# Justin900429/autonomous_driving_with_diffusion_model

Hardware: AMD Instinct MI355X
Metric: denoising-steps/sec (higher is better)
Workload: dtype f32

## Files before the change

### autonomous_driving_with_diffusion_model_amd/_lib.py

```python
from __future__ import annotations

import ctypes as C
import os
from typing import Optional, Sequence

import torch

_HERE = os.path.dirname(os.path.abspath(__file__))
LIB_PATH = os.environ.get("ADX_LIB") or os.path.join(_HERE, "libadx.so")

c_f32p = C.POINTER(C.c_float)
i32, i64, f32, vp = C.c_int32, C.c_int64, C.c_float, C.c_void_p


class TConvDesc(C.Structure):
    _fields_ = [("kind", i32), ("taps", i32), ("stride", i32), ("pad", i32), ("c0", i32), ("c1", i32),
                ("cout", i32), ("lin", i32), ("lout", i32), ("groups", i32), ("eps", f32), ("w_layout", i32),
                ("w_flip", i32), ("exact", i32), ("lin_valid", i32), ("lout_valid", i32)]


class TConvIO(C.Structure):
    _fields_ = [("x0", vp), ("x0_sb", i64), ("x0_sc", i64), ("x0_sl", i64),
                ("x1", vp), ("x1_sb", i64), ("x1_sc", i64), ("x1_sl", i64),
                ("packed_w", vp), ("bias", vp), ("gamma", vp), ("beta", vp),
                ("tbias", vp), ("tbias_stride", i64),
                ("res", vp), ("res_sb", i64), ("res_sc", i64), ("res_sl", i64),
                ("y", vp), ("y_sb", i64), ("y_sc", i64), ("y_sl", i64), ("batch", i32), ("pre", vp), ("stats", vp),
                ("scratch", vp), ("scratch_floats", i64), ("tickets", vp)]


class EmbedWeights(C.Structure):
    _fields_ = [(n, vp) for n in ("freqs", "w1", "b1", "w3", "b3", "cw0", "cb0", "cw2", "cb2")]


class UnetConfig(C.Structure):
    _fields_ = [("horizon", i32), ("transition_dim", i32), ("dim", i32), ("n_mults", i32),
                ("dim_mults", i32 * 8), ("guidance", i32)]


class UnetIO(C.Structure):
    _fields_ = [("x", vp), ("img_feature", vp), ("feat_rows", i32), ("t", vp), ("t_rows", i32), ("cond", vp),
                ("rows", i32), ("out", vp), ("time_embed", vp), ("x_rows", i32), ("time_bias", vp)]


UNET_ATTENTION = 1


class Conv2dDesc(C.Structure):
    _fields_ = [("cin", i32), ("cout", i32), ("k", i32), ("stride", i32), ("pad", i32)]


class StepCoef(C.Structure):
    _fields_ = [("prediction_type", i32), ("clip", i32), ("clip_range", f32), ("sqrt_alpha_t", f32),
                ("sqrt_beta_t", f32), ("c_x0", f32), ("c_dir", f32), ("c_x", f32), ("c_noise", f32),
                ("add_noise", i32), ("use_clipped_model_output", i32), ("inpaint", i32), ("c_const", f32),
                ("c_known", f32), ("c_known_noise", f32), ("known_noise", i32), ("cfg_combine", i32),
                ("free_scale", f32), ("zero_first", i32)]


_SIGS = {
    "adx_version": (i32, []),
    "adx_last_error": (C.c_char_p, []),
    "adx_source_hash": (C.c_char_p, []),
    "adx_tconv_packed_bytes": (C.c_size_t, [C.POINTER(TConvDesc)]),
    "adx_tconv_pack": (i32, [C.POINTER(TConvDesc), vp, vp, vp]),
    "adx_tconv_forward": (i32, [C.POINTER(TConvDesc), C.POINTER(TConvIO), vp]),
    "adx_embed_forward": (i32, [C.POINTER(EmbedWeights), i32, vp, i32, vp, vp, i32, i32, vp, vp, vp]),
    "adx_unet_create": (i32, [C.POINTER(UnetConfig), C.POINTER(vp)]),
    "adx_unet_create_ex": (i32, [C.POINTER(UnetConfig), i32, C.POINTER(vp)]),
    "adx_unet_destroy": (None, [vp]),
    "adx_unet_num_params": (i32, [vp]),
    "adx_unet_packed_bytes": (C.c_size_t, [vp]),
    "adx_unet_pack": (i32, [vp, C.POINTER(vp), i32, vp, vp, vp]),
    "adx_unet_workspace_bytes": (C.c_size_t, [vp, i32]),
    "adx_unet_forward": (i32, [vp, vp, vp, C.POINTER(UnetIO), vp]),
    "adx_unet_time_bias_width": (i32, [vp]),
    "adx_unet_time_conditioning_workspace_bytes": (C.c_size_t, [vp, i32]),
    "adx_unet_time_conditioning": (i32, [vp, vp, vp, C.POINTER(UnetIO), vp, vp, vp]),
    "adx_unet_tape_create": (i32, [C.POINTER(vp)]),
    "adx_unet_tape_destroy": (None, [vp]),
    "adx_unet_train_workspace_bytes": (C.c_size_t, [vp, i32]),
    "adx_unet_forward_train": (i32, [vp, vp, vp, C.c_size_t, C.POINTER(UnetIO), vp, vp]),
    "adx_unet_backward": (i32, [vp, vp, vp, C.c_size_t, vp, vp, vp, vp, C.POINTER(vp), C.POINTER(vp), i32, vp]),
    "adx_gn_mish_backward": (i32, [vp, i64, i64, i64, vp, vp, vp, vp, vp, vp, vp, vp, vp, i64, i32, i32, i32, i32, vp]),
    "adx_tconv_wgrad": (i32, [C.POINTER(TConvDesc), C.POINTER(TConvIO), vp, vp, vp]),
    "adx_bias_grad": (i32, [vp, vp, i32, i32, i32, vp]),
    "adx_chan_layernorm_forward": (i32, [vp, i64, i64, i64, vp, vp, vp, vp, vp, i32, i32, i32, i32, vp]),
    "adx_chan_layernorm_backward": (i32, [vp, vp, i64, i64, i64, vp, vp, vp, vp, vp, vp, i32, i32, i32, i32, i32, vp]),
    "adx_linattn_forward": (i32, [vp, vp, i32, i32, i32, vp]),
    "adx_linattn_backward": (i32, [vp, vp, vp, i32, i32, i32, vp]),
    "adx_resnet_create": (i32, [i32, C.POINTER(vp)]),
    "adx_resnet_destroy": (None, [vp]),
    "adx_resnet_num_tensors": (i32, [vp]),
    "adx_resnet_packed_bytes": (C.c_size_t, [vp]),
    "adx_resnet_pack": (i32, [vp, C.POINTER(vp), i32, vp, vp]),
    "adx_resnet_workspace_bytes": (C.c_size_t, [vp, i32, i32, i32]),
    "adx_resnet_forward": (i32, [vp, vp, vp, vp, i32, i32, i32, vp, vp]),
    "adx_resnet_forward_u8": (i32, [vp, vp, vp, vp, C.POINTER(C.c_float), C.POINTER(C.c_float), i32, i32, i32, vp, vp]),
    "adx_resnet_tape_create": (i32, [C.POINTER(vp)]),
    "adx_resnet_tape_destroy": (None, [vp]),
    "adx_resnet_train_workspace_bytes": (C.c_size_t, [vp, i32, i32, i32]),
    "adx_resnet_forward_train": (i32, [vp, C.POINTER(vp), i32, vp, vp, C.c_size_t, vp, i32, i32, i32, vp, vp, i32, vp]),
    "adx_resnet_backward": (i32, [vp, C.POINTER(vp), C.POINTER(vp), i32, vp, C.c_size_t, vp, vp, vp]),
    "adx_resnet_backward_groups": (i32, [vp]),
    "adx_resnet_tensor_group": (i32, [vp, i32]),
    "adx_resnet_backward_events": (i32, [vp, C.POINTER(vp), C.POINTER(vp), i32, vp, C.c_size_t, vp, vp, C.POINTER(vp), i32, vp]),
    "adx_resnet_tape_describe": (i32, [vp, vp, i32, C.POINTER(i32), C.POINTER(i32), C.POINTER(i64)]),
    "adx_conv2d_packed_bytes": (C.c_size_t, [C.POINTER(Conv2dDesc)]),
    "adx_conv2d_pack": (i32, [C.POINTER(Conv2dDesc), vp, vp, vp]),
    "adx_conv2d_forward": (i32, [C.POINTER(Conv2dDesc), vp, vp, vp, vp, vp, vp, i32, i32, i32, i32, vp]),
    "adx_conv2d_cells_supported": (i32, [C.POINTER(Conv2dDesc), i32, i32, i32]),
    "adx_conv2d_forward_cells": (i32, [C.POINTER(Conv2dDesc), vp, vp, vp, vp, vp, vp, i32, i32, i32, i32, i32, vp]),
    "adx_conv2d_wgrad_scratch_bytes": (C.c_size_t, []),
    "adx_conv2d_wgrad": (i32, [C.POINTER(Conv2dDesc), vp, vp, vp, i32, i32, i32, vp, vp]),
    "adx_conv2d_wgrad_ex": (i32, [C.POINTER(Conv2dDesc), vp, vp, vp, i32, i32, i32, vp, i32, vp]),
    "adx_conv2d_wgrad_cells": (i32, [C.POINTER(Conv2dDesc), vp, vp, vp, vp, i32, i32, i32, vp, vp]),
    "adx_trajpred_create": (i32, [i32, C.POINTER(vp)]),
    "adx_trajpred_destroy": (None, [vp]),
    "adx_trajpred_num_params": (i32, [vp]),
    "adx_trajpred_packed_bytes": (C.c_size_t, [vp]),
    "adx_trajpred_scratch_bytes": (C.c_size_t, [vp, i32, i32]),
    "adx_trajpred_set_scratch": (i32, [vp, vp, C.c_size_t]),
    "adx_trajpred_pack": (i32, [vp, C.POINTER(vp), i32, vp, vp, vp]),
    "adx_trajpred_forward": (i32, [vp, vp, vp, i64, i64, vp, vp, i32, i32, vp]),
    "adx_trajpred_backward": (i32, [vp, vp, vp, i64, i64, vp, vp, vp, i32, i32, vp]),
    "adx_trajpred_backward_params": (i32, [vp, vp, vp, i64, i64, vp, vp, vp, vp, vp, i32, i32, C.c_float, C.c_uint64, vp]),
    "adx_trajpred_forward_train": (i32, [vp, vp, vp, i64, i64, vp, vp, i32, i32, C.c_float, C.c_uint64, vp]),
    "adx_trajpred_param_offsets": (i32, [vp, C.POINTER(i64), i32]),
    "adx_guided_output": (i32, [vp, vp, vp, vp, vp, f32, f32, vp, vp, i32, i32, vp]),
    "adx_optim_chunk": (i32, []),
    "adx_adamw_ema_step": (i32, [vp, vp, vp, i32, f32, f32, f32, f32, f32, i32, f32, i32, i32, vp]),
    "adx_adamw_ema_step_scaled": (i32, [vp, vp, vp, i32, f32, f32, f32, f32, f32, i32, f32, i32, i32, f32, vp]),
    "adx_image_normalize": (i32, [vp, vp, i32, i32, i32, C.POINTER(C.c_float), C.POINTER(C.c_float), vp]),
    "adx_probe_mfma_fp16": (i32, [vp, vp, i32, i32, C.POINTER(C.c_double), vp]),
    "adx_probe_mfma_fp16_16x16x32": (i32, [vp, vp, i32, i32, C.POINTER(C.c_double), vp]),
    "adx_image_augment": (i32, [vp, vp, i32, i32, i32, vp, vp, vp, vp, i32, vp]),
    "adx_ddim_step": (i32, [C.POINTER(StepCoef), vp, vp, vp, vp, vp, vp, vp, i32, i32, i32, vp]),
    "adx_ddpm_step": (i32, [C.POINTER(StepCoef), vp, vp, vp, vp, vp, vp, vp, i32, i32, i32, vp]),
    "adx_add_noise": (i32, [vp, vp, vp, vp, vp, i32, vp, i32, i32, i32, i32, vp]),
}

EXPORTED_SYMBOLS = tuple(_SIGS)

_lib: Optional[C.CDLL] = None


class AdxError(RuntimeError):
    pass


def lib() -> C.CDLL:
    global _lib
    if _lib is None:
        if not os.path.exists(LIB_PATH):
            raise AdxError(
                f"{LIB_PATH} not found: the HIP extension is not built. Run `python -c 'import __graft_entry__ as g; "
                f"g.build()'` (or autonomous_driving_with_diffusion_model_amd/csrc/build.sh). There is no CPU fallback.")
        handle = C.CDLL(LIB_PATH)
        for name, (res, args) in _SIGS.items():
            fn = getattr(handle, name)
            fn.restype = res
            fn.argtypes = args
        _lib = handle
    return _lib


class NativeTape:

    def __init__(self, create, destroy, what: str):
        import weakref
        h = vp()
        check(create(C.byref(h)), what)
        self.handle = h
        self._fin = weakref.finalize(self, destroy, h)

    @property
    def alive(self) -> bool:
        return self._fin.alive

    def release(self) -> None:
        self._fin()


def check(rc: int, what: str = "") -> None:
    if rc != 0:
        msg = lib().adx_last_error().decode(errors="replace")
        if rc == -1:
            raise ValueError(f"{what}: {msg}" if what else msg)
        raise AdxError(f"{what} failed (status {rc}): {msg}")


def ptr(t: Optional[torch.Tensor]) -> Optional[int]:
    return None if t is None else t.data_ptr()


def stream_ptr(device=None) -> int:
    return torch.cuda.current_stream(device).cuda_stream


def require_gpu_f32(t: torch.Tensor, name: str, dtype=torch.float32) -> torch.Tensor:
    if not t.is_cuda:
        raise AdxError(f"{name} lives on {t.device}; the adx kernels only run on an MI355X (no CPU path)")
    if t.dtype != dtype:
        raise TypeError(f"{name} must be {dtype}, got {t.dtype}")
    return t if t.is_contiguous() else t.contiguous()


def write_stamp(t: torch.Tensor) -> int:
    return 0 if t.is_inference() else t._version


def grad_buffer(p: torch.Tensor) -> torch.Tensor:
    v = getattr(p, "_adx_grad_view", None)
    if (v is not None and p.grad is None and not getattr(p, "_adx_grad_leased", False)
            and v.device == p.device and v.shape == p.shape):
        p._adx_grad_leased = True
        return v.detach()
    return torch.empty_like(p)


def ptr_array(tensors: Sequence[torch.Tensor]):
    arr = (vp * len(tensors))()
    for i, t in enumerate(tensors):
        arr[i] = t.data_ptr()
    return arr
```

### autonomous_driving_with_diffusion_model_amd/csrc/conv2d.hip

```cpp
#include <stdlib.h>

#include <vector>

#include "adx_common.h"
#include "conv2d_internal.h"

namespace adx {

constexpr int kCoutT = 64;
constexpr size_t kMaxLds = 96 * 1024;
constexpr int g_conv_cc = 16;
constexpr int g_conv_rows = 2;

template <int STRIDE, int K, int ROWS, int CCH = 16>
__global__ void __launch_bounds__(256) conv2d_kernel(const Conv2dArgs a) {
  constexpr int TH = 4 * ROWS;
  constexpr int CC = (K == 7) ? 4 : CCH;
  constexpr int PH = (TH - 1) * STRIDE + K;
  constexpr int PW = (kTileW - 1) * STRIDE + K;
  constexpr int PLANE = PH * PW;
  constexpr int NP = CC * PLANE;
  constexpr int PITEMS = (NP + 255) / 256;
  constexpr int NTAPS = K * K;
  constexpr int NW4 = NTAPS * CC * (kCoutT / 4);
// ... 177 lines not shown
  const int oy = blockIdx.y * 4 + wave;
  const int pl = blockIdx.x;
  if (oy >= OH) return;
  const float* src = x + (size_t)pl * H * W;
  float* dst = y + ((size_t)pl * OH + oy) * OW;
  if ((W & 1) == 0 && ((size_t)x & 7) == 0) {
    typedef float f32x2 __attribute__((ext_vector_type(2)));
    for (int ox0 = lane; ox0 - lane < OW; ox0 += 256) {
      float m[4] = {-INFINITY, -INFINITY, -INFINITY, -INFINITY};
#pragma unroll
      for (int dy = 0; dy < 3; ++dy) {
        const int iy = oy * 2 - 1 + dy;
        if (iy < 0 || iy >= H) continue;
        const float* row = src + (size_t)iy * W;
        f32x2 v[4];
        float left[4];
#pragma unroll
        for (int q = 0; q < 4; ++q) {
          const int ox = ox0 + 64 * q;
          const bool in = 2 * ox + 1 < W;
          v[q] = in ? *reinterpret_cast<const f32x2*>(row + 2 * ox) : f32x2{-INFINITY, -INFINITY};
          left[q] = (lane == 0 && ox > 0 && 2 * ox - 1 < W) ? row[2 * ox - 1] : -INFINITY;
        }
#pragma unroll
        for (int q = 0; q < 4; ++q) {
          const float nb = __shfl_up(v[q][1], 1, 64);
          const float l = lane == 0 ? left[q] : nb;
          m[q] = pool_max(pool_max(pool_max(m[q], l), v[q][0]), v[q][1]);
        }
      }
#pragma unroll
      for (int q = 0; q < 4; ++q)
        if (ox0 + 64 * q < OW) dst[ox0 + 64 * q] = m[q];
    }
    return;
  }
  for (int ox0 = lane; ox0 < OW; ox0 += 256) {
    float m[4] = {-INFINITY, -INFINITY, -INFINITY, -INFINITY};
#pragma unroll
    for (int dy = 0; dy < 3; ++dy) {
      const int iy = oy * 2 - 1 + dy;
      const bool rok = iy >= 0 && iy < H;
      const float* row = src + (size_t)(rok ? iy : 0) * W;
#pragma unroll
      for (int q = 0; q < 4; ++q)
#pragma unroll
        for (int dx = 0; dx < 3; ++dx) {
          const int ix = (ox0 + 64 * q) * 2 - 1 + dx;
          const bool ok = rok && ix >= 0 && ix < W;
          const float v = ok ? row[ix] : -INFINITY;
          m[q] = pool_max(m[q], v);
        }
    }
#pragma unroll
    for (int q = 0; q < 4; ++q)
      if (ox0 + 64 * q < OW) dst[ox0 + 64 * q] = m[q];
  }
}

__global__ void __launch_bounds__(1024) avgpool_fc_kernel(const float* __restrict__ x, const float* __restrict__ fw,
                                                           const float* __restrict__ fb, float* __restrict__ out,
                                                           int C, int HW, int out_dim) {
  __shared__ float pooled[512];
  const int n = blockIdx.x, tid = threadIdx.x, lane = tid & 63, wave = tid >> 6;
  const float* src = x + (size_t)n * C * HW;
  const float inv = 1.0f / (float)HW;
  for (int c0 = wave * 4; c0 < C; c0 += 64) {
    float s[4] = {0.f, 0.f, 0.f, 0.f};
    for (int i = lane; i < HW; i += 64) {
#pragma unroll
      for (int q = 0; q < 4; ++q) s[q] += (c0 + q < C) ? src[(size_t)(c0 + q) * HW + i] : 0.f;
    }
#pragma unroll
    for (int q = 0; q < 4; ++q) {
      const float t = wave_sum(s[q]);
      if (lane == 0 && c0 + q < C) pooled[c0 + q] = t * inv;
    }
  }
  __syncthreads();
  for (int j = wave; j < out_dim; j += 16) {
    float s = 0.f;
    for (int c = lane; c < C; c += 64) s += fw[(size_t)j * C + c] * pooled[c];
    s = wave_sum(s);
    if (lane == 0) out[(size_t)n * out_dim + j] = s + fb[j];
  }
}

int maxpool_launch(const float* x, float* y, int planes, int H, int W, int OH, int OW, hipStream_t s) {
  maxpool_kernel<<<dim3(planes, ceil_div(OH, 4)), dim3(256), 0, s>>>(x, y, planes, H, W, OH, OW);
  ADX_LAUNCH_CHECK();
  return ADX_OK;
}

__global__ void __launch_bounds__(1024) avgpool_fc_cells_kernel(const uint4* __restrict__ x, const float* __restrict__ fw,
                                                                 const float* __restrict__ fb, float* __restrict__ out,
                                                                 int C, int HW, int out_dim) {
  typedef _Float16 h8 __attribute__((ext_vector_type(8)));
  __shared__ float pooled[512];
  const int n = blockIdx.x, tid = threadIdx.x, lane = tid & 63, wave = tid >> 6;
  const uint4* src = x + (size_t)n * (C / 8) * 2 * HW;
  const float inv = 1.0f / (float)HW;
  for (int g = wave; g < C / 8; g += 16) {
    float s[8] = {0.f, 0.f, 0.f, 0.f, 0.f, 0.f, 0.f, 0.f};
    for (int i = lane; i < HW; i += 64) {
      const h8 hi = __builtin_bit_cast(h8, src[(size_t)(2 * g) * HW + i]);
      const h8 lo = __builtin_bit_cast(h8, src[(size_t)(2 * g + 1) * HW + i]);
#pragma unroll
      for (int q = 0; q < 8; ++q) s[q] += (float)hi[q] + (float)lo[q] * (1.f / 2048.f);
    }
#pragma unroll
    for (int q = 0; q < 8; ++q) {
      const float t = wave_sum(s[q]);
      if (lane == 0) pooled[8 * g + q] = t * inv;
    }
  }
  __syncthreads();
  for (int j = wave; j < out_dim; j += 16) {
    float s = 0.f;
    for (int c = lane; c < C; c += 64) s += fw[(size_t)j * C + c] * pooled[c];
    s = wave_sum(s);
    if (lane == 0) out[(size_t)n * out_dim + j] = s + fb[j];
  }
}

int avgpool_fc_launch(const float* x, const float* fw, const float* fb, float* out, int batch, int C, int HW, int out_dim,
                      hipStream_t s, int x_cells) {
  ADX_REQUIRE(C <= 512, "avgpool_fc: at most 512 channels");
  if (x_cells) {
    ADX_REQUIRE(C % 8 == 0, "avgpool_fc: the cell layout holds channels in groups of eight");
    avgpool_fc_cells_kernel<<<dim3(batch), dim3(1024), 0, s>>>(reinterpret_cast<const uint4*>(x), fw, fb, out, C, HW, out_dim);
    ADX_LAUNCH_CHECK();
    return ADX_OK;
  }
  avgpool_fc_kernel<<<dim3(batch), dim3(1024), 0, s>>>(x, fw, fb, out, C, HW, out_dim);
  ADX_LAUNCH_CHECK();
  return ADX_OK;
}

}

namespace adx {

static size_t align64f(size_t v) { return (v + 63) / 64 * 64; }

static int conv_out(int h, int k, int s, int p) { return conv_out_dim(h, k, s, p); }

static int conv2d_launch(const ConvSpec& L, const float* base, const float* x, const float* res, float* y, int N, int H,
                         int W, int relu, hipStream_t s, int fmt = 0) {
  return conv2d_launch_raw(L, x, base + L.o_w, base + L.o_scale, base + L.o_shift, res, y, N, H, W, relu, s, nullptr, 0, nullptr, 0,
                           nullptr, fmt);
}

static thread_local float* t_split_scratch = nullptr;
static thread_local size_t t_split_floats = 0;
void conv2d_set_split_scratch(float* p, size_t floats) { t_split_scratch = p; t_split_floats = p != nullptr ? floats : 0; }

int conv2d_launch_raw(const ConvSpec& L, const float* x, const float* w, const float* scale, const float* shift,
                      const float* res, float* y, int N, int H, int W, int relu, hipStream_t s, const uint32_t* x_amax,
                      int x_amax_n, float* stats_part, size_t stats_floats, int* stats_p, int fmt, const BnBwdStats* bst) {
  if (stats_p != nullptr) *stats_p = 0;
  Conv2dArgs a;
  a.x = x; a.w = w; a.scale = scale; a.shift = shift; a.res = res; a.y = y; a.x_amax = x_amax; a.x_amax_n = x_amax_n;
  a.w_ds = nullptr; a.scale_ds = nullptr; a.shift_ds = nullptr; a.y_ds = nullptr;
  a.N = N; a.Cin = L.cin; a.H = H; a.W = W; a.Cout = L.cout;
  a.OH = conv_out(H, L.k, L.stride, L.pad); a.OW = conv_out(W, L.k, L.stride, L.pad);
  a.KH = L.k; a.KW = L.k; a.stride = L.stride; a.pad = L.pad; a.relu = relu;
  a.cin_pad = L.cin_pad; a.cc = L.cc;
  a.x_u8 = nullptr;
  a.d2s_cin = 0; a.d2s_h = 0; a.d2s_w = 0; a.stem_seg_tiles = 0; a.stem_nseg = 1;
  a.ksplit = 1; a.cper = 0; a.part = t_split_scratch; a.part_stride = t_split_floats;
  a.stats_part = nullptr; a.stats_p = 0;
  a.bs_raw = a.bs_out = a.bs_mean = a.bs_rstd = a.bs_gamma = a.bs_beta = nullptr; a.bs_mask = 0; a.bs_bits = nullptr; a.res_bits = nullptr;
  if (bst != nullptr) {
    ADX_REQUIRE(bst->raw && bst->mean && bst->rstd && bst->gamma && bst->beta && (bst->mask == 2 || (bst->mask == 1 && (bst->out || bst->bits))),
                "conv2d: incomplete BatchNorm-backward statistics request");
    ADX_REQUIRE(scale == nullptr && relu == 0, "conv2d: BatchNorm-backward statistics belong to data-gradient launches");
    a.bs_raw = bst->raw; a.bs_out = bst->out; a.bs_mean = bst->mean; a.bs_rstd = bst->rstd; a.bs_gamma = bst->gamma;
    a.bs_beta = bst->beta; a.bs_mask = bst->mask; a.bs_bits = bst->mask == 1 ? bst->bits : nullptr;
    a.res_bits = bst->res_bits;
    ADX_REQUIRE(a.res_bits == nullptr || (res != nullptr && stats_part != nullptr &&
                                          conv2d_hs3x3_dgrad_stats(L, N, H, W, (fmt & kFmtXCells) != 0, stats_floats)),
                "conv2d: a masked residual belongs to a data-gradient launch with the statistics epilogue");
  }
  a.x_cells = (fmt & kFmtXCells) != 0; a.y_cells = (fmt & kFmtYCells) != 0; a.res_cells = (fmt & kFmtResCells) != 0 && res != nullptr;
  const bool train_cells = fmt == kFmtXCells && stats_part != nullptr && stats_p != nullptr && bst == nullptr && x_amax == nullptr &&
                           conv2d_hs3x3_train_cells(L, N, H, W, stats_floats);
  const bool dgrad_cells = fmt == (kFmtXCells | kFmtXScaled) && L.dgrad && x_amax != nullptr && x_amax_n < 0 &&
                           conv2d_hs3x3_dgrad_cells(L, N, H, W);
  if (dgrad_cells) fmt = kFmtXCells;
  ADX_REQUIRE(fmt == 0 || train_cells || dgrad_cells || (stats_part == nullptr && conv2d_hs3x3_plain(L, N, H, W)),
              "conv2d: the cell layout belongs to plain launches of the pipelined 3x3 kernel (%d -> %d, k%d s%d)", L.cin, L.cout, L.k, L.stride);
  if (conv2d_hs_eligible(L)) {
    if (stats_part != nullptr && stats_p != nullptr && conv2d_hs_stats_tiles(L, a) > 0 &&
        (size_t)conv2d_hs_stats_tiles(L, a) * (L.cout * 2 + L.cout / 64) <= stats_floats) {
      a.stats_part = stats_part;
      a.stats_p = conv2d_hs_stats_tiles(L, a);
      *stats_p = a.stats_p;
    }
    return conv2d_hs_launch(L, a, s);
  }
  const int rows = (L.stride == 1 && L.k == 3 && g_conv_rows == 2) ? 2 : 1;
  const int th = 4 * rows;
  a.tiles_x = ceil_div(a.OW, kTileW); a.tiles_y = ceil_div(a.OH, th); a.cout_tiles = L.cout / kCoutT;
  a.PH = (th - 1) * L.stride + L.k; a.PW = (kTileW - 1) * L.stride + L.k;
  a.PWp = a.PW;
  ADX_REQUIRE(L.cin % L.cc == 0 || L.cin < L.cc, "conv2d: cin %d must be < %d or a multiple of it", L.cin, L.cc);
  ADX_REQUIRE((size_t)L.cin * H * W < (1u << 31), "conv2d: image plane too large for 32-bit gather offsets");
  const int cch = (rows == 2 && g_conv_cc == 8) ? 8 : a.cc;
  const size_t np = (size_t)cch * a.PH * a.PW;
  const size_t lds = sizeof(float) * ((np + 255) / 256 * 256 + (size_t)L.k * L.k * cch * kCoutT + 2 * kCoutT);
  ADX_REQUIRE(lds <= kMaxLds, "conv2d: LDS %zu bytes too large", lds);
  const size_t grid = (size_t)a.cout_tiles * a.tiles_x * a.tiles_y * N;
  ADX_REQUIRE(grid < (1u << 31), "conv2d: grid too large");
  static std::atomic<uint64_t> attr_set{0};
  if (DeviceOnce once{attr_set}; once) {
    const void* fns[6] = {reinterpret_cast<const void*>(&conv2d_kernel<1, 3, 1>), reinterpret_cast<const void*>(&conv2d_kernel<2, 3, 1>),
                          reinterpret_cast<const void*>(&conv2d_kernel<2, 1, 1>), reinterpret_cast<const void*>(&conv2d_kernel<2, 7, 1>),
                          reinterpret_cast<const void*>(&conv2d_kernel<1, 1, 1>), reinterpret_cast<const void*>(&conv2d_kernel<1, 3, 2>)};
    ADX_CHECK_HIP(hipFuncSetAttribute(reinterpret_cast<const void*>(&conv2d_kernel<1, 3, 2, 8>),
                                      hipFuncAttributeMaxDynamicSharedMemorySize, (int)kMaxLds));
    for (const void* f : fns) ADX_CHECK_HIP(hipFuncSetAttribute(f, hipFuncAttributeMaxDynamicSharedMemorySize, (int)kMaxLds));
    once.commit();
  }
  const dim3 g((unsigned)grid), blk(256);
  if (L.stride == 1 && L.k == 3 && rows == 2 && cch == 8) conv2d_kernel<1, 3, 2, 8><<<g, blk, lds, s>>>(a);
  else if (L.stride == 1 && L.k == 3 && rows == 2) conv2d_kernel<1, 3, 2><<<g, blk, lds, s>>>(a);
  else if (L.stride == 1 && L.k == 3) conv2d_kernel<1, 3, 1><<<g, blk, lds, s>>>(a);
  else if (L.stride == 2 && L.k == 3) conv2d_kernel<2, 3, 1><<<g, blk, lds, s>>>(a);
  else if (L.stride == 2 && L.k == 1) conv2d_kernel<2, 1, 1><<<g, blk, lds, s>>>(a);
  else if (L.stride == 2 && L.k == 7) conv2d_kernel<2, 7, 1><<<g, blk, lds, s>>>(a);
  else if (L.stride == 1 && L.k == 1) conv2d_kernel<1, 1, 1><<<g, blk, lds, s>>>(a);
  else {
    set_error("conv2d: no kernel for k=%d stride=%d (ResNet-34 uses 3x3 s1, 3x3 s2, 1x1 s2, 7x7 s2)", L.k, L.stride);
    return ADX_ERR_INVALID;
  }
  ADX_LAUNCH_CHECK();
  return ADX_OK;
}

}

using namespace adx;

static int spec_from_desc(const adx_conv2d_desc* d, ConvSpec* L) {
  ADX_REQUIRE(d != nullptr, "conv2d: null descriptor");
  ADX_REQUIRE(d->cin >= 1 && d->cout >= 64 && d->cout % kCoutT == 0, "conv2d: cout %d must be a multiple of %d", d->cout,
              kCoutT);
  ADX_REQUIRE(d->k >= 1 && d->k <= 7 && (d->stride == 1 || d->stride == 2) && d->pad >= 0 && d->pad <= 3,
              "conv2d: unsupported k/stride/pad %d/%d/%d", d->k, d->stride, d->pad);
  memset(L, 0, sizeof(*L));
  L->cin = d->cin; L->cout = d->cout; L->k = d->k; L->stride = d->stride; L->pad = d->pad;
  L->cc = d->cin >= 16 ? 16 : 4;
  L->cin_pad = round_up(d->cin, L->cc);
  return ADX_OK;
}

extern "C" {

size_t adx_conv2d_packed_bytes(const adx_conv2d_desc* d) {
  ConvSpec L;
  if (spec_from_desc(d, &L) != ADX_OK) return 0;
  return sizeof(float) * (conv2d_hs_eligible(L) ? conv2d_packed_floats(L) : (size_t)L.k * L.k * L.cin_pad * L.cout);
}

int adx_conv2d_pack(const adx_conv2d_desc* d, const float* w, float* packed, adx_stream stream) {
  ConvSpec L;
  int rc = spec_from_desc(d, &L);
  if (rc != ADX_OK) return rc;
  ADX_REQUIRE(w && packed, "adx_conv2d_pack: null pointer");
  return conv2d_pack_spec(L, w, packed, 0, (hipStream_t)stream);
}

int adx_conv2d_forward(const adx_conv2d_desc* d, const float* x, const float* packed_w, const float* scale,
                       const float* shift, const float* res, float* y, int32_t n, int32_t h, int32_t w, int32_t relu,
                       adx_stream stream) {
  ConvSpec L;
  int rc = spec_from_desc(d, &L);
  if (rc != ADX_OK) return rc;
  ADX_REQUIRE(x && packed_w && y, "adx_conv2d_forward: null tensor");
  ADX_REQUIRE((scale == nullptr) == (shift == nullptr), "adx_conv2d_forward: scale and shift go together");
  ADX_REQUIRE(n >= 1 && h + 2 * d->pad >= d->k && w + 2 * d->pad >= d->k, "adx_conv2d_forward: input too small");
  return conv2d_launch_raw(L, x, packed_w, scale, shift, res, y, n, h, w, relu, (hipStream_t)stream);
}

int adx_conv2d_cells_supported(const adx_conv2d_desc* d, int32_t n, int32_t h, int32_t w) {
  ConvSpec L;
  if (d == nullptr || spec_from_desc(d, &L) != ADX_OK) return 0;
  return conv2d_hs3x3_plain(L, n, h, w) ? 1 : 0;
}

int adx_conv2d_forward_cells(const adx_conv2d_desc* d, const void* x, const float* packed_w, const float* scale,
                             const float* shift, const void* res, void* y, int32_t n, int32_t h, int32_t w, int32_t relu,
                             int32_t fmt, adx_stream stream) {
  ConvSpec L;
  int rc = spec_from_desc(d, &L);
  if (rc != ADX_OK) return rc;
  ADX_REQUIRE(x && packed_w && y, "adx_conv2d_forward_cells: null tensor");
  ADX_REQUIRE((scale == nullptr) == (shift == nullptr), "adx_conv2d_forward_cells: scale and shift go together");
  ADX_REQUIRE(fmt >= 0 && fmt <= 7 && (fmt & kFmtYCells), "adx_conv2d_forward_cells: fmt %d (the output is a cell tensor)", fmt);
  ADX_REQUIRE(conv2d_hs3x3_plain(L, n, h, w), "adx_conv2d_forward_cells: not a plain launch of the pipelined 3x3 kernel "
              "(adx_conv2d_cells_supported)");
  return conv2d_launch_raw(L, (const float*)x, packed_w, scale, shift, (const float*)res, (float*)y, n, h, w, relu,
                           (hipStream_t)stream, nullptr, 0, nullptr, 0, nullptr, fmt);
}

int adx_resnet_create(int32_t out_dim, adx_resnet** out) {
  ADX_REQUIRE(out != nullptr && out_dim >= 1 && out_dim <= 4096, "adx_resnet_create: bad argument");
  adx_resnet* r = new adx_resnet();
  r->out_dim = out_dim;
  int t = 0;
  size_t off = 0;
  auto add = [&](int cin, int cout, int k, int stride, int pad) {
    ConvSpec L{};
    L.cin = cin; L.cout = cout; L.k = k; L.stride = stride; L.pad = pad;
    L.t_w = t++; L.t_g = t++; L.t_b = t++; L.t_m = t++; L.t_v = t++;
    L.cc = cin >= 16 ? 16 : 4;
    L.cin_pad = round_up(cin, L.cc);
    L.fuse_with = -1;
    L.o_w = off; off = align64f(off + (conv2d_hs_eligible(L) ? conv2d_packed_floats(L) : (size_t)k * k * L.cin_pad * cout));
    L.o_scale = off; off = align64f(off + cout);
    L.o_shift = off; off = align64f(off + cout);
    r->convs.push_back(L);
  };
  add(3, 64, 7, 2, 3);
  const int planes[4] = {64, 128, 256, 512}, nblk[4] = {3, 4, 6, 3};
  int inpl = 64;
  for (int li = 0; li < 4; ++li)
    for (int bi = 0; bi < nblk[li]; ++bi) {
      const int stride = (li > 0 && bi == 0) ? 2 : 1;
      add(inpl, planes[li], 3, stride, 1);
      add(planes[li], planes[li], 3, 1, 1);
      const int ds = (stride != 1 || inpl != planes[li]) ? 1 : 0;
      if (ds) {
        add(inpl, planes[li], 1, stride, 0);
        r->convs.back().fuse_with = (int)r->convs.size() - 3;
      }
      r->block_has_ds.push_back(ds);
      inpl = planes[li];
    }
  r->t_fcw = t++; r->t_fcb = t++;
  r->n_tensors = t;
  r->o_fcw = off; off = align64f(off + (size_t)out_dim * 512);
  r->o_fcb = off; off = align64f(off + out_dim);
  r->packed_floats = off;
  *out = r;
  return ADX_OK;
}

void adx_resnet_destroy(adx_resnet* r) {
  if (r == nullptr) return;
  for (auto& st : r->side) if (st != nullptr) (void)hipStreamDestroy(st);
  if (r->ev_fork != nullptr) (void)hipEventDestroy(r->ev_fork);
  for (auto& ev : r->ev_join) if (ev != nullptr) (void)hipEventDestroy(ev);
  delete r;
}
int adx_resnet_num_tensors(const adx_resnet* r) { return r ? r->n_tensors : 0; }
size_t adx_resnet_packed_bytes(const adx_resnet* r) { return r ? r->packed_floats * sizeof(float) : 0; }

int adx_resnet_pack(adx_resnet* r, const float* const* T, int32_t n, void* packed, adx_stream stream) {
  ADX_REQUIRE(r && T && packed, "adx_resnet_pack: null argument");
  ADX_REQUIRE(n == r->n_tensors, "adx_resnet_pack: expected %d tensors, got %d", r->n_tensors, n);
  for (int i = 0; i < n; ++i) ADX_REQUIRE(T[i] != nullptr, "adx_resnet_pack: tensor %d is null", i);
  hipStream_t s = (hipStream_t)stream;
  float* base = (float*)packed;
  for (const ConvSpec& L : r->convs) {
    const bool fused = L.fuse_with >= 0 && resnet_fuses_ds(r->convs[L.fuse_with], L);
    int rc = fused ? conv2d_hs_pack(L, T[L.t_w], base + L.o_w, 0, s) : conv2d_pack_spec(L, T[L.t_w], base + L.o_w, 0, s);
    if (rc != ADX_OK) return rc;
    bn_fold_kernel<<<dim3(ceil_div(L.cout, 256)), dim3(256), 0, s>>>(T[L.t_g], T[L.t_b], T[L.t_m], T[L.t_v],
                                                                     base + L.o_scale, base + L.o_shift, L.cout);
    ADX_LAUNCH_CHECK();
  }
  ADX_CHECK_HIP(hipMemcpyAsync(base + r->o_fcw, T[r->t_fcw], (size_t)r->out_dim * 512 * sizeof(float),
                               hipMemcpyDeviceToDevice, s));
  ADX_CHECK_HIP(hipMemcpyAsync(base + r->o_fcb, T[r->t_fcb], (size_t)r->out_dim * sizeof(float),
                               hipMemcpyDeviceToDevice, s));
  r->packed_once = true;
  return ADX_OK;
}

static void resnet_dims(int h, int w, int* h1, int* w1, int* h2, int* w2) {
  *h1 = conv_out(h, 7, 2, 3); *w1 = conv_out(w, 7, 2, 3);
  *h2 = conv_out(*h1, 3, 2, 1); *w2 = conv_out(*w1, 3, 2, 1);
}

size_t adx_resnet_workspace_bytes(const adx_resnet* r, int32_t batch, int32_t h, int32_t w) {
  if (!r || batch < 1 || h < 32 || w < 32) return 0;
  int h1, w1, h2, w2;
  resnet_dims(h, w, &h1, &w1, &h2, &w2);
  const size_t stem = align64f((size_t)batch * 64 * h1 * w1);
  const size_t act = align64f((size_t)batch * 64 * h2 * w2);
  return (stem + 3 * act) * sizeof(float);
}

static int resnet_forward_impl(adx_resnet* r, const void* packed, void* workspace, const float* img,
                               const uint8_t* frames_u8, const float* mean, const float* stdv, int32_t batch, int32_t h,
                               int32_t w, float* feature, adx_stream stream);

int adx_resnet_forward(adx_resnet* r, const void* packed, void* workspace, const float* img, int32_t batch, int32_t h,
                       int32_t w, float* feature, adx_stream stream) {
  ADX_REQUIRE(img != nullptr, "adx_resnet_forward: null image");
  return resnet_forward_impl(r, packed, workspace, img, nullptr, nullptr, nullptr, batch, h, w, feature, stream);
}

int adx_resnet_forward_u8(adx_resnet* r, const void* packed, void* workspace, const uint8_t* frames_hwc, const float* mean,
                          const float* stdv, int32_t batch, int32_t h, int32_t w, float* feature, adx_stream stream) {
  ADX_REQUIRE(frames_hwc && mean && stdv, "adx_resnet_forward_u8: null frames / mean / std");
  ADX_REQUIRE(r != nullptr && !r->convs.empty() && conv2d_hs_eligible(r->convs[0]),
              "adx_resnet_forward_u8: the uint8 front-end lives in the split-fp16 stem kernel (unavailable with ADX_CONV_EXACT=1)");
  return resnet_forward_impl(r, packed, workspace, nullptr, frames_hwc, mean, stdv, batch, h, w, feature, stream);
}

__global__ void __launch_bounds__(256) range_scan_kernel(const uint32_t* __restrict__ v, size_t words, int cells, unsigned* flag) {
  bool bad = false;
  for (size_t i = (size_t)blockIdx.x * 256 + threadIdx.x; i < words; i += (size_t)gridDim.x * 256) {
    const uint32_t b = v[i];
    if (cells) bad |= ((b & 0x7C00u) == 0x7C00u) | ((b & 0x7C000000u) == 0x7C000000u);
    else bad |= (b & 0x7FFFFFFFu) >= 0x477FE000u;
  }
  if (bad) atomicOr(flag, 1u);
}

extern "C++" int adx::conv2d_range_check(const char* what, int index, const float* t, size_t floats, bool cells, hipStream_t s) {
  if (!debug_switches().check_range) return ADX_OK;
  static unsigned* flag = nullptr;
  if (flag == nullptr) ADX_CHECK_HIP(hipMalloc(&flag, sizeof(unsigned)));
  ADX_CHECK_HIP(hipMemsetAsync(flag, 0, sizeof(unsigned), s));
  range_scan_kernel<<<dim3(1024), dim3(256), 0, s>>>(reinterpret_cast<const uint32_t*>(t), floats, cells ? 1 : 0, flag);
  ADX_LAUNCH_CHECK();
  unsigned h = 0;
  ADX_CHECK_HIP(hipMemcpyAsync(&h, flag, sizeof(unsigned), hipMemcpyDeviceToHost, s));
  ADX_CHECK_HIP(hipStreamSynchronize(s));
  if (h != 0) {
    set_error("adx_resnet_forward: %s %d writes activations outside the fp16 range of the split kernels (|x| >= 65504 or "
              "non-finite); ADX_CONV_EXACT=1 runs the pass on the exact-fp32 kernels", what, index);
    return ADX_ERR_RANGE;
  }
  return ADX_OK;
}

static int resnet_forward_impl(adx_resnet* r, const void* packed, void* workspace, const float* img,
                               const uint8_t* frames_u8, const float* mean, const float* stdv, int32_t batch, int32_t h,
                               int32_t w, float* feature, adx_stream stream) {
  ADX_REQUIRE(r && packed && workspace && (img || frames_u8) && feature, "adx_resnet_forward: null argument");
  if (!r->packed_once) {
    set_error("adx_resnet_forward: weights were never packed (call adx_resnet_pack first)");
    return ADX_ERR_STATE;
  }
  ADX_REQUIRE(batch >= 1 && h >= 32 && w >= 32, "adx_resnet_forward: image %dx%d (batch %d) too small", h, w, batch);
  hipStream_t s = (hipStream_t)stream;
  const float* base = (const float*)packed;
  int h1, w1, h2, w2;
  resnet_dims(h, w, &h1, &w1, &h2, &w2);
  float* ws = (float*)workspace;
  float* stem = ws;
  const size_t act = align64f((size_t)batch * 64 * h2 * w2);
  float* buf[3];
  buf[0] = ws + align64f((size_t)batch * 64 * h1 * w1);
  buf[1] = buf[0] + act;
  buf[2] = buf[1] + act;

  struct ScratchScope {
    void set(float* p, size_t n) { conv2d_set_split_scratch(p, n); }
    ~ScratchScope() { conv2d_set_split_scratch(nullptr, 0); }
  } scratch_scope;
  const size_t nblocks = r->block_has_ds.size();

  struct Cursor { size_t ci; int cur, H, W; bool cells; };
  constexpr int fuse = 1;

  auto run_stem = [&](Cursor& st, int n0, int n, int nf, hipStream_t s) -> int {
    const ConvSpec& c0 = r->convs[0];
    const float* im = img != nullptr ? img + (size_t)n0 * 3 * h * w : nullptr;
    const uint8_t* fr = frames_u8 != nullptr ? frames_u8 + (size_t)n0 * 3 * h * w : nullptr;
    float* pooled = buf[0] + (size_t)n0 * 64 * h2 * w2;
    bool pooled_cells = false;
    int rc;
    if ((fuse || frames_u8 != nullptr) && conv2d_hs_eligible(c0)) {
      pooled_cells = nblocks > 0 && !r->block_has_ds[0] && r->convs[1].stride == 1 && conv2d_hs3x3_plain(r->convs[1], nf, h2, w2) &&
                     conv2d_hs3x3_plain(r->convs[2], nf, h2, w2);
      rc = conv2d_hs_stem_pool(c0, im, base + c0.o_w, base + c0.o_scale, base + c0.o_shift, pooled, n, h, w, s, fr, mean, stdv,
                               pooled_cells);
      if (rc != ADX_OK) return rc;
    } else {
      float* sm = stem + (size_t)n0 * 64 * h1 * w1;
      rc = conv2d_launch(c0, base, im, nullptr, sm, n, h, w, 1, s);
      if (rc != ADX_OK) return rc;
      rc = maxpool_launch(sm, pooled, n * 64, h1, w1, h2, w2, s);
      if (rc != ADX_OK) return rc;
    }
    st = Cursor{1, 0, h2, w2, pooled_cells};
    return conv2d_range_check("the stem (conv1 + bn1 + relu + maxpool), tensor", 0, pooled, (size_t)n * 64 * h2 * w2, pooled_cells, s);
  };

  auto run_block = [&](size_t b, Cursor& st, int n0, int n, int nf, hipStream_t s) -> int {
    size_t ci = st.ci;
    const int cur = st.cur, H = st.H, W = st.W;
    const bool cur_cells = st.cells;
    const ConvSpec& c1 = r->convs[ci++];
    const ConvSpec& c2 = r->convs[ci++];
    const int mid = (cur + 1) % 3, outb = (cur + 2) % 3;
    const int OH = conv_out(H, 3, c1.stride, 1), OW = conv_out(W, 3, c1.stride, 1);
    const size_t off_in = (size_t)n0 * 64 * h2 * w2, off_out = off_in;
    const float* xin = buf[cur] + off_in;
    const float* identity = xin;
    bool id_cells = cur_cells, mid_cells = false;
    const bool c2_plain = conv2d_hs3x3_plain(c2, nf, OH, OW);
    int rc;
    if (r->block_has_ds[b] && resnet_fuses_ds(c1, r->convs[ci + 0])) {
      const ConvSpec& ds = r->convs[ci++];
      mid_cells = c2_plain;
      rc = conv2d_hs_launch_block_s2(c1, ds, xin, base + c1.o_w, base + c1.o_scale, base + c1.o_shift, buf[mid] + off_out,
                                     base + ds.o_w, base + ds.o_scale, base + ds.o_shift, buf[outb] + off_out, n, H, W, s, cur_cells,
                                     mid_cells);
      if (rc != ADX_OK) return rc;
      identity = buf[outb] + off_out;
      id_cells = mid_cells;
    } else {
      const bool c1_plain = c1.stride == 1 && conv2d_hs3x3_plain(c1, nf, H, W);
      ADX_REQUIRE(!cur_cells || c1_plain, "adx_resnet_forward: internal error (cell-layout input of a launch that cannot read it)");
      mid_cells = c1_plain && c2_plain && !r->block_has_ds[b];
      rc = conv2d_launch(c1, base, xin, nullptr, buf[mid] + off_out, n, H, W, 1, s,
                         (cur_cells ? kFmtXCells : 0) | (mid_cells ? kFmtYCells : 0));
      if (rc != ADX_OK) return rc;
      if (r->block_has_ds[b]) {
        const ConvSpec& ds = r->convs[ci++];
        ADX_REQUIRE(!cur_cells, "adx_resnet_forward: internal error (cell-layout input of the downsample conv)");
        rc = conv2d_launch(ds, base, xin, nullptr, buf[outb] + off_out, n, H, W, 0, s);
        if (rc != ADX_OK) return rc;
        identity = buf[outb] + off_out;
        id_cells = false;
      }
    }
    float* dst = (r->block_has_ds[b] ? buf[cur] : buf[outb]) + off_out;
    bool out_cells = false;
    if (c2_plain) {
      if (b + 1 == nblocks) {
        out_cells = true;
      } else if (r->block_has_ds[b + 1]) {
        out_cells = resnet_fuses_ds(r->convs[ci], r->convs[ci + 2]);
      } else {
        out_cells = r->convs[ci].stride == 1 && conv2d_hs3x3_plain(r->convs[ci], nf, OH, OW) &&
                    conv2d_hs3x3_plain(r->convs[ci + 1], nf, OH, OW);
      }
    }
    ADX_REQUIRE(out_cells || !(mid_cells || id_cells),
                "adx_resnet_forward: internal error (a conv with cell-layout operands whose reader wants fp32)");
    rc = conv2d_range_check("conv1 + bn1 + relu of BasicBlock", (int)b, buf[mid] + off_out, (size_t)n * c1.cout * OH * OW, mid_cells, s);
    if (rc != ADX_OK) return rc;
    rc = conv2d_launch(c2, base, buf[mid] + off_out, identity, dst, n, OH, OW, 1, s,
                       (mid_cells ? kFmtXCells : 0) | (out_cells ? kFmtYCells : 0) | (id_cells ? kFmtResCells : 0));
    if (rc != ADX_OK) return rc;
    rc = conv2d_range_check("the output of BasicBlock", (int)b, dst, (size_t)n * c2.cout * OH * OW, out_cells, s);
    if (rc != ADX_OK) return rc;
    st = Cursor{ci, r->block_has_ds[b] ? cur : outb, OH, OW, out_cells};
    return ADX_OK;
  };

  constexpr int kMaxSub = adx_resnet::kMaxSub;
  int nsub = 1;
  if (batch >= 32 && !debug_switches().check_range && fuse && conv2d_hs_eligible(r->convs[0])) {
    nsub = std::min(debug_switches().resnet_streams, kMaxSub);
    while (nsub > 1 && batch / nsub < 16) --nsub;
  }
  if (nsub > 1) {
    hipStreamCaptureStatus cs = hipStreamCaptureStatusNone;
    if (hipStreamIsCapturing(s, &cs) != hipSuccess || cs != hipStreamCaptureStatusNone) nsub = 1;
  }
  if (nsub > 1) {
    int dev = 0;
    ADX_CHECK_HIP(hipGetDevice(&dev));
    if (r->side_device != dev || r->side[nsub - 2] == nullptr) {
      {
        if (r->side_device != dev) {
          for (auto& st : r->side) if (st != nullptr) { (void)hipStreamDestroy(st); st = nullptr; }
          if (r->ev_fork != nullptr) { (void)hipEventDestroy(r->ev_fork); r->ev_fork = nullptr; }
          for (auto& ev : r->ev_join) if (ev != nullptr) { (void)hipEventDestroy(ev); ev = nullptr; }
          r->side_device = dev;
        }
        if (r->ev_fork == nullptr) ADX_CHECK_HIP(hipEventCreateWithFlags(&r->ev_fork, hipEventDisableTiming));
        for (int k = 0; k < nsub - 1; ++k) {
          if (r->side[k] == nullptr) ADX_CHECK_HIP(hipStreamCreateWithFlags(&r->side[k], hipStreamNonBlocking));
          if (r->ev_join[k] == nullptr) ADX_CHECK_HIP(hipEventCreateWithFlags(&r->ev_join[k], hipEventDisableTiming));
        }
      }
    }
  }
  hipStream_t streams[kMaxSub];
  int n0s[kMaxSub], ns[kMaxSub];
  Cursor st[kMaxSub]{};
  for (int k = 0, at = 0; k < nsub; ++k) {
    streams[k] = k == 0 ? s : r->side[k - 1];
    n0s[k] = at;
    ns[k] = batch / nsub + (k < batch % nsub ? 1 : 0);
    at += ns[k];
  }
  const size_t scratch_per = ((size_t)batch * 64 * h1 * w1 / nsub) & ~(size_t)63;
  const bool stem_free = (fuse || frames_u8 != nullptr) && conv2d_hs_eligible(r->convs[0]);
  auto lend = [&](int k) { if (stem_free) scratch_scope.set(stem + (size_t)k * scratch_per, scratch_per); };
  int rc = ADX_OK;
  size_t first_split = 0;
  if (nsub > 1) {
    while (first_split < nblocks && !r->block_has_ds[first_split]) ++first_split;
    if (debug_switches().resnet_split_from >= 0) first_split = std::min((size_t)debug_switches().resnet_split_from, first_split);
  }
  if (first_split > 0) {
// ... 26 lines not shown
```

### autonomous_driving_with_diffusion_model_amd/csrc/conv2d_hs.hip

```cpp
#include <type_traits>
#include <stdlib.h>

#include "adx_common.h"
#include "conv2d_internal.h"
#include "conv2d_hs_common.h"

namespace adx {

template <bool AFFINE = true>
__device__ __forceinline__ void cells_store32(float (&v)[16], const float* sc, const float* sh, int cl0, const float (*res8)[8],
                                              bool relu, __amdgpu_buffer_rsrc_t yrsrc, uint32_t vcell, uint32_t so, uint32_t cplane) {
#pragma unroll
  for (int i = 0; i < 2; ++i)
#pragma unroll
    for (int j = 0; j < 4; ++j) {
      const auto sw = __builtin_amdgcn_permlane32_swap(f2u(v[8 * i + j]), f2u(v[8 * i + 4 + j]), false, false);
      v[8 * i + j] = u2f(sw[0]);
      v[8 * i + 4 + j] = u2f(sw[1]);
    }
#pragma unroll
  for (int i = 0; i < 2; ++i) {
    float o[8];
#pragma unroll
    for (int j = 0; j < 8; ++j) {
// ... 546 lines not shown
      const int s = 3 * cp + i;
      const int kh = i % 3, cpar = (i / 3) & 1;
      const u32x4* pb0 = patch + cpar * 4 * PLANE + pb_lane;
      const u32x4* wa0 = wl + (i & 1) * WST + wa_lane;
      load_w(s + 2 < nstages ? s + 2 : nstages - 1, i & 1);
      if ((i + 1) % 3 < PIT) load_p(s + 4 < nstages ? (s + 4) / 3 : nchunks - 1, (i + 1) % 3, i & 1);
      __builtin_amdgcn_sched_barrier(0);
#pragma unroll
      for (int kw = 0; kw < K; ++kw) {
        f16x8 A[2][2], B[2][2];
#pragma unroll
        for (int pl = 0; pl < 2; ++pl) {
#pragma unroll
          for (int m = 0; m < 2; ++m) A[pl][m] = __builtin_bit_cast(f16x8, wa0[(kw * 2 + pl) * 128 + m * 32]);
#pragma unroll
          for (int r = 0; r < 2; ++r) B[pl][r] = __builtin_bit_cast(f16x8, pb0[pl * PLANE + (r + kh) * PW + kw]);
        }
#pragma unroll
        for (int r = 0; r < 2; ++r)
#pragma unroll
          for (int m = 0; m < 2; ++m) {
            accm[r][m] = hs_mfma(A[0][m], B[0][r], accm[r][m]);
            accl[r][m] = hs_mfma(A[0][m], B[1][r], accl[r][m]);
            accl[r][m] = hs_mfma(A[1][m], B[0][r], accl[r][m]);
          }
        if (kw == 0) {
          store_w((i + 1) & 1, (i + 1) & 1);
          if (i % 3 < PIT) store_p((i + 1) & 1, i % 3, ((i + 3) / 3) & 1);
        }
      }
      __syncthreads();
    }
  }

  HS_TRACE(3);
  const int ox = VROW ? xl : ox0 + l31;
  const uint32_t plane_ob = (uint32_t)(a.OH * a.OW) * (uint32_t)sizeof(float);
  const size_t img = (size_t)n * a.Cout * a.OH * a.OW;
  const int img_bytes = (int)(uint32_t)((VROW ? (uint32_t)a.N : 1u) * (uint32_t)a.Cout * plane_ob);
  const uint32_t img_off = VROW ? (uint32_t)nl * (uint32_t)a.Cout * plane_ob : 0u;
  float* const ybase = a.ksplit > 1 ? a.part + (size_t)kpart * a.part_stride : a.y;
  const __amdgpu_buffer_rsrc_t yrsrc = __builtin_amdgcn_make_buffer_rsrc(ybase + img, 0, img_bytes, 0x00020000);
  const __amdgpu_buffer_rsrc_t rrsrc = __builtin_amdgcn_make_buffer_rsrc(
      const_cast<float*>(a.res != nullptr ? a.res + img : a.y), 0, a.res != nullptr ? img_bytes : 0, 0x00020000);
  const float* sst = ss + slab * 64;
  const uint32_t cbase_o = (uint32_t)cout0 * plane_ob;
  const uint32_t cplane = (uint32_t)(a.OH * a.OW) * 16u;
  const uint32_t cell0 = (uint32_t)(cout0 >> 3) * 2u * cplane;
  bool inside[2];
  uint32_t pix[2];
#pragma unroll
  for (int rr = 0; rr < 2; ++rr) {
    const int oy = oy0 + rowpair * 2 + rr;
    inside[rr] = lane_valid && oy < a.OH && ox < a.OW;
    pix[rr] = (uint32_t)(oy * a.OW + ox);
  }
  auto half4 = [](uint32_t h0, uint32_t h1, uint32_t l0, uint32_t l1, float* out) {
    const float inv = 1.f / kLoScale;
    asm("v_fma_mix_f32 %0, %1, %2, %3 op_sel:[0,0,0] op_sel_hi:[1,0,1]" : "=v"(out[0]) : "v"(l0), "s"(inv), "v"(h0));
    asm("v_fma_mix_f32 %0, %1, %2, %3 op_sel:[1,0,1] op_sel_hi:[1,0,1]" : "=v"(out[1]) : "v"(l0), "s"(inv), "v"(h0));
    asm("v_fma_mix_f32 %0, %1, %2, %3 op_sel:[0,0,0] op_sel_hi:[1,0,1]" : "=v"(out[2]) : "v"(l1), "s"(inv), "v"(h1));
    asm("v_fma_mix_f32 %0, %1, %2, %3 op_sel:[1,0,1] op_sel_hi:[1,0,1]" : "=v"(out[3]) : "v"(l1), "s"(inv), "v"(h1));
  };
  if constexpr (YCELLS) {
    const uint32_t khoff = (uint32_t)khalf * 2u * cplane;
    uint32_t vcell[2], vres[2];
#pragma unroll
    for (int rr = 0; rr < 2; ++rr) {
      vcell[rr] = inside[rr] ? img_off + pix[rr] * 16u + khoff : kOutside;
      vres[rr] = !inside[rr] ? kOutside : a.res_cells ? vcell[rr] : img_off + pix[rr] * 4u + (uint32_t)(8 * khalf) * plane_ob;
    }
    uint32_t rraw[2][2][2][8];
#pragma unroll
    for (int rr = 0; rr < 2; ++rr)
#pragma unroll
      for (int half = 0; half < 2; ++half)
#pragma unroll
        for (int i = 0; i < 2; ++i) {
          if (a.res_cells) {
            const uint32_t so = cell0 + (uint32_t)(half * 4 + 2 * i) * 2u * cplane;
            const u32x4 h4 = __builtin_amdgcn_raw_buffer_load_b128(rrsrc, vres[rr], so, 0);
            const u32x4 l4 = __builtin_amdgcn_raw_buffer_load_b128(rrsrc, vres[rr], so + cplane, 0);
#pragma unroll
            for (int j = 0; j < 4; ++j) { rraw[rr][half][i][j] = h4[j]; rraw[rr][half][i][4 + j] = l4[j]; }
          } else {
#pragma unroll
            for (int j = 0; j < 8; ++j)
              rraw[rr][half][i][j] = __builtin_amdgcn_raw_buffer_load_b32(rrsrc, vres[rr], cbase_o + (uint32_t)(half * 32 + 16 * i + j) * plane_ob, 0);
          }
        }
#ifdef ADX_HS_TRACE
    asm volatile("s_waitcnt vmcnt(0)" ::: "memory");
    HS_TRACE(6);
#endif
#pragma unroll
    for (int rr = 0; rr < 2; ++rr)
#pragma unroll
      for (int half = 0; half < 2; ++half) {
        float v[16];
#pragma unroll
        for (int r = 0; r < 16; ++r) v[r] = accm[rr][half][r] + accl[rr][half][r] * (1.f / kLoScale);
        float res8[2][8];
#pragma unroll
        for (int i = 0; i < 2; ++i) {
          if (a.res_cells) {
            half4(rraw[rr][half][i][0], rraw[rr][half][i][1], rraw[rr][half][i][4], rraw[rr][half][i][5], res8[i]);
            half4(rraw[rr][half][i][2], rraw[rr][half][i][3], rraw[rr][half][i][6], rraw[rr][half][i][7], res8[i] + 4);
          } else {
#pragma unroll
            for (int j = 0; j < 8; ++j) res8[i][j] = u2f(rraw[rr][half][i][j]);
          }
        }
        cells_store32(v, sst, sst + 64 * CT, half * 32 + 8 * khalf, res8, a.relu != 0, yrsrc, vcell[rr],
                      cell0 + (uint32_t)(half * 4) * 2u * cplane, cplane);
      }
  } else {
  uint32_t voff[2];
#pragma unroll
  for (int rr = 0; rr < 2; ++rr) voff[rr] = inside[rr] ? img_off + pix[rr] * 4u + (uint32_t)(4 * khalf) * plane_ob : kOutside;
  float rv[2][2][16];
  if constexpr (STATS != 2) {
#pragma unroll
  for (int rr = 0; rr < 2; ++rr)
#pragma unroll
    for (int half = 0; half < 2; ++half)
#pragma unroll
      for (int r = 0; r < 16; ++r) {
        const int cu = half * 32 + (r & 3) + 8 * (r >> 2);
        rv[rr][half][r] = __builtin_bit_cast(float, __builtin_amdgcn_raw_buffer_load_b32(rrsrc, voff[rr], cbase_o + cu * plane_ob, 0));
      }
  }
#ifdef ADX_HS_TRACE
  asm volatile("s_waitcnt vmcnt(0)" ::: "memory");
  HS_TRACE(6);
#endif
  if constexpr (STATS != 0) {
    float* red = reinterpret_cast<float*>(smem_raw);
    const bool val0 = voff[0] != kOutside, val1 = voff[1] != kOutside;
    auto park = [&](int half, int r, float sm, float sq) {
      sm += hs_dpp<0xB1>(sm);  sq += hs_dpp<0xB1>(sq);
      sm += hs_dpp<0x4E>(sm);  sq += hs_dpp<0x4E>(sq);
      sm += hs_dpp<0x141>(sm); sq += hs_dpp<0x141>(sq);
      sm += hs_dpp<0x140>(sm); sq += hs_dpp<0x140>(sq);
      if ((lane & 15) == 0) {
        float* d = red + (((wave * 4 + (lane >> 4)) * 32) + half * 16 + r) * 2;
        d[0] = sm;
        d[1] = sq;
      }
    };
    if constexpr (STATS == 1) {
#pragma unroll
      for (int half = 0; half < 2; ++half)
#pragma unroll
        for (int r = 0; r < 16; ++r) {
          const float v0 = val0 ? (accm[0][half][r] + accl[0][half][r] * (1.f / kLoScale)) * xs_inv : 0.f;
          const float v1 = val1 ? (accm[1][half][r] + accl[1][half][r] * (1.f / kLoScale)) * xs_inv : 0.f;
          park(half, r, v0 + v1, v0 * v0 + v1 * v1);
        }
    } else {
#pragma unroll
      for (int rr = 0; rr < 2; ++rr)
#pragma unroll
        for (int half = 0; half < 2; ++half)
#pragma unroll
          for (int r = 0; r < 16; ++r) accm[rr][half][r] = (accm[rr][half][r] + accl[rr][half][r] * (1.f / kLoScale)) * xs_inv;
      const __amdgpu_buffer_rsrc_t wrsrc = __builtin_amdgcn_make_buffer_rsrc(const_cast<float*>(a.bs_raw + img), 0, img_bytes, 0x00020000);
      const bool mask_bits = a.bs_mask == 1 && a.bs_bits != nullptr;
      const bool mask_out = a.bs_mask == 1 && !mask_bits;
      const __amdgpu_buffer_rsrc_t orsrc = __builtin_amdgcn_make_buffer_rsrc(
          const_cast<float*>(mask_out ? a.bs_out + img : a.y), 0, mask_out ? img_bytes : 0, 0x00020000);
      const uint32_t bplane = (uint32_t)(a.OH * a.OW);
      const __amdgpu_buffer_rsrc_t brsrc = __builtin_amdgcn_make_buffer_rsrc(
          const_cast<uint8_t*>(mask_bits ? a.bs_bits + (size_t)n * (a.Cout >> 3) * bplane : reinterpret_cast<const uint8_t*>(a.y)), 0,
          mask_bits ? (int)((VROW ? (uint32_t)a.N : 1u) * (uint32_t)(a.Cout >> 3) * bplane) : 0, 0x00020000);
      uint32_t boff[2];
#pragma unroll
      for (int rr = 0; rr < 2; ++rr)
        boff[rr] = inside[rr] ? (VROW ? (uint32_t)nl * (uint32_t)(a.Cout >> 3) * bplane : 0u) + pix[rr] : kOutside;
      const bool res_masked = a.res_bits != nullptr;
      const __amdgpu_buffer_rsrc_t qrsrc = __builtin_amdgcn_make_buffer_rsrc(
          const_cast<uint8_t*>(res_masked ? a.res_bits + (size_t)n * (a.Cout >> 3) * bplane : reinterpret_cast<const uint8_t*>(a.y)), 0,
          res_masked ? (int)((VROW ? (uint32_t)a.N : 1u) * (uint32_t)(a.Cout >> 3) * bplane) : 0, 0x00020000);
      const float* bsw = bsl + slab * 64;
      const uint32_t use_bit = mask_bits ? 1u : 0u, use_out = mask_out ? 1u : 0u, use_raw = 1u - use_bit - use_out;
      const uint32_t v0u = val0 ? 1u : 0u, v1u = val1 ? 1u : 0u;
      float dmx = 0.f;
#pragma unroll
      for (int half = 0; half < 2; ++half) {
        float rs_[2][16], rw_[2][16], ro_[2][16];
#pragma unroll
        for (int rr = 0; rr < 2; ++rr)
#pragma unroll
          for (int r = 0; r < 16; ++r) {
            const uint32_t so = cbase_o + (uint32_t)(half * 32 + (r & 3) + 8 * (r >> 2)) * plane_ob;
            rs_[rr][r] = __builtin_bit_cast(float, __builtin_amdgcn_raw_buffer_load_b32(rrsrc, voff[rr], so, 0));
            rw_[rr][r] = __builtin_bit_cast(float, __builtin_amdgcn_raw_buffer_load_b32(wrsrc, voff[rr], so, 0));
            ro_[rr][r] = 0.f;
          }
        if (mask_out) {
#pragma unroll
          for (int rr = 0; rr < 2; ++rr)
#pragma unroll
            for (int r = 0; r < 16; ++r) {
              const uint32_t so = cbase_o + (uint32_t)(half * 32 + (r & 3) + 8 * (r >> 2)) * plane_ob;
              ro_[rr][r] = __builtin_bit_cast(float, __builtin_amdgcn_raw_buffer_load_b32(orsrc, voff[rr], so, 0));
            }
        }
        if (res_masked) {
#pragma unroll
          for (int rr = 0; rr < 2; ++rr)
#pragma unroll
            for (int q = 0; q < 4; ++q) {
              const uint32_t m = (uint32_t)__builtin_amdgcn_raw_buffer_load_b8(qrsrc, boff[rr], ((uint32_t)(cout0 >> 3) + (uint32_t)(half * 4 + q)) * bplane, 0)
                                 >> (4 * khalf);
#pragma unroll
              for (int i = 0; i < 4; ++i)
                if (!((m >> i) & 1u)) rs_[rr][4 * q + i] = 0.f;
            }
        }
        uint32_t mb[2][4] = {{0u, 0u, 0u, 0u}, {0u, 0u, 0u, 0u}};
        if (mask_bits) {
#pragma unroll
          for (int rr = 0; rr < 2; ++rr)
#pragma unroll
            for (int q = 0; q < 4; ++q)
              mb[rr][q] = (uint32_t)__builtin_amdgcn_raw_buffer_load_b8(brsrc, boff[rr], ((uint32_t)(cout0 >> 3) + (uint32_t)(half * 4 + q)) * bplane, 0)
                          >> (4 * khalf);
        }
#pragma unroll
        for (int r = 0; r < 16; ++r) {
          const int cu = half * 32 + (r & 3) + 8 * (r >> 2);
          const int cl = cu + 4 * khalf;
          const float mu = bsw[cl], rsd = bsw[64 * CT + cl], msc = bsw[2 * 64 * CT + cl], msh = bsw[3 * 64 * CT + cl];
          float p[2], q[2];
#pragma unroll
          for (int rr = 0; rr < 2; ++rr) {
            const float y = accm[rr][half][r] + rs_[rr][r];
            __builtin_amdgcn_raw_buffer_store_b32(__builtin_bit_cast(uint32_t, y), yrsrc, voff[rr], cbase_o + cu * plane_ob, 0);
            const uint32_t on_bit = (mb[rr][r >> 2] >> (r & 3)) & 1u, on_out = ro_[rr][r] > 0.f ? 1u : 0u;
            const uint32_t on_raw = __builtin_fmaf(rw_[rr][r], msc, msh) > 0.f ? 1u : 0u;
            const bool keep = ((rr == 0 ? v0u : v1u) & ((on_bit & use_bit) | (on_out & use_out) | (on_raw & use_raw))) != 0u;
            p[rr] = keep ? y : 0.f;
            q[rr] = p[rr] * ((rw_[rr][r] - mu) * rsd);
            dmx = __builtin_fmaxf(dmx, __builtin_fabsf(p[rr]));
          }
          park(half, r, p[0] + p[1], q[0] + q[1]);
        }
      }
#pragma unroll
      for (int off = 32; off > 0; off >>= 1) dmx = __builtin_fmaxf(dmx, __shfl_xor(dmx, off, 64));
      if (lane == 0) red[4096 + wave] = dmx;
    }
    __syncthreads();
    if (STATS == 2 && tid >= 2 * 64 * CT && tid < 2 * 64 * CT + CT) {
      const int sl = tid - 2 * 64 * CT;
      constexpr int WPS = (NT / 64) / CT;
      float t = 0.f;
#pragma unroll
      for (int w = 0; w < WPS; ++w) t = __builtin_fmaxf(t, red[4096 + (MODE == 2 ? sl * WPS + w : w)]);
      const int p = (n * a.tiles_y + ty) * a.tiles_x + tx;
      a.stats_part[(size_t)a.Cout * 2 * a.stats_p + (size_t)(ct * CT + sl) * a.stats_p + p] = t;
    }
    if (tid < 2 * 64 * CT) {
      const int which = tid & 1, chs = tid >> 1, sl = chs >> 6, ch = chs & 63;
      const int c5 = ch & 31, kh2 = (c5 >> 2) & 1, r = (c5 & 3) + 4 * (c5 >> 3), idx32 = (ch >> 5) * 16 + r;
      constexpr int WPS = (NT / 64) / CT;
      float t = 0.f;
#pragma unroll
      for (int w = 0; w < WPS; ++w)
#pragma unroll
        for (int j = 0; j < 2; ++j) t += red[((((MODE == 2 ? sl * WPS + w : w) * 4 + kh2 * 2 + j) * 32) + idx32) * 2 + which];
      const int p = (n * a.tiles_y + ty) * a.tiles_x + tx;
      a.stats_part[((size_t)((ct * CT + sl) * kHsCout + ch) * 2 + which) * a.stats_p + p] = t;
    }
  }
  auto finish = [&](auto relu) {
#pragma unroll
    for (int rr = 0; rr < 2; ++rr)
#pragma unroll
      for (int half = 0; half < 2; ++half)
#pragma unroll
        for (int r = 0; r < 16; ++r) {
          const int cu = half * 32 + (r & 3) + 8 * (r >> 2);
          const int cl = cu + 4 * khalf;
          float v = (accm[rr][half][r] + accl[rr][half][r] * (1.f / kLoScale)) * xs_inv;
          v = v * sst[cl] + sst[64 * CT + cl];
          v += rv[rr][half][r];
          if (decltype(relu)::value) v = __builtin_fmaxf(v, 0.f);
          __builtin_amdgcn_raw_buffer_store_b32(__builtin_bit_cast(uint32_t, v), yrsrc, voff[rr], cbase_o + cu * plane_ob, 0);
        }
  };
  if constexpr (STATS != 2) {
    if (a.relu) finish(std::true_type{}); else finish(std::false_type{});
  }
  }
  HS_TRACE(4);
#ifdef ADX_HS_TRACE
  __builtin_amdgcn_s_waitcnt(0);
  asm volatile("s_waitcnt vmcnt(0)" ::: "memory");
  HS_TRACE(5);
#endif
}

__device__ __forceinline__ float pool_max3(float a, float b, float c) {
  float m = a;
  m = (b > m || b != b) ? b : m;
  m = (c > m || c != c) ? c : m;
  return m;
}

constexpr int kStemSteps = 11;
constexpr int kStemPP = 72;

template <bool POOL, bool U8>
__global__ void __launch_bounds__(256, 2) conv2d_hs_stem_kernel(const Conv2dArgs a) {
  constexpr int NT = 256;
  constexpr int PH = POOL ? 25 : 21;
  constexpr int PBUF = POOL ? 1 : 2;
  constexpr int CP = PH * kStemPP;
  constexpr int PLANEH = 3 * CP;
  constexpr int ITEMS = 3 * PH * 35;
  constexpr int PIT = (ITEMS + NT - 1) / NT;
  constexpr int NROW = POOL ? 3 : 1;
  extern __shared__ __attribute__((aligned(16))) unsigned char smem_raw[];
  u32x4* wl = reinterpret_cast<u32x4*>(smem_raw);
  uint32_t* patch = reinterpret_cast<uint32_t*>(wl + kStemSteps * 256);
  float* ss = reinterpret_cast<float*>(patch + PBUF * PLANEH);
  const int tid = threadIdx.x, lane = tid & 63;
  const int wave = __builtin_amdgcn_readfirstlane(tid >> 6);
  const int l31 = lane & 31, khalf = lane >> 5;
  int bid = blockIdx.x, seg = 0;
  if (a.stem_nseg > 1) { seg = bid % a.stem_nseg; bid /= a.stem_nseg; }
  const int n = bid / a.tiles_y, ty = bid - n * a.tiles_y;
  const int tx_own = a.stem_nseg > 1 ? seg * a.stem_seg_tiles : 0;
  const int tx_end = a.stem_nseg > 1 ? min(a.tiles_x, tx_own + a.stem_seg_tiles) : a.tiles_x;
  const int tx_begin = POOL && tx_own > 0 ? tx_own - 1 : tx_own;
  const int oy0 = POOL ? ty * 8 - 1 : ty * 8, iy0 = oy0 * 2 - 3;
  const size_t hw = (size_t)a.H * a.W;
  const float* xin = a.x + (size_t)n * 3 * hw;
  constexpr uint32_t kOutside = 0xC0000000u;
  const __amdgpu_buffer_rsrc_t xrsrc =
      U8 ? __builtin_amdgcn_make_buffer_rsrc(const_cast<uint8_t*>(a.x_u8 + (size_t)n * 3 * hw), 0, (int)(3 * hw), 0x00020000)
         : __builtin_amdgcn_make_buffer_rsrc(const_cast<float*>(xin), 0, (int)(3 * hw * sizeof(float)), 0x00020000);

  {
    const u32x4* wsrc = reinterpret_cast<const u32x4*>(a.w);
#pragma unroll
    for (int k = 0; k < kStemSteps; ++k) wl[tid + 256 * k] = wsrc[tid + 256 * k];
  }
  if (tid < 2 * kHsCout) {
    const int c = tid & (kHsCout - 1);
    ss[tid] = a.scale == nullptr ? (tid < kHsCout ? 1.f : 0.f) : (tid < kHsCout ? a.scale[c] : a.shift[c]);
  }
  float* cbuf = ss + 2 * kHsCout + wave * 64 + khalf;
  float* cpark = l31 == 31 ? cbuf : ss + 2 * kHsCout + 4 * 64 + (lane & 1);
  if (POOL && l31 == 0) {
#pragma unroll
    for (int i = 0; i < 32; ++i) cbuf[2 * i] = -INFINITY;
  }

  auto decode = [&](int k, int& c, int& py, int& pp) {
    int e = tid + NT * k;
    asm volatile("" : "+v"(e));
    c = e / (PH * 35);
    const int rem = e - c * (PH * 35);
    py = rem / 35;
    pp = rem - py * 35;
  };
  float pv[PIT][2];
  auto load_p = [&](int tx) {
    const int ix0 = tx * 64 - 3;
#pragma unroll
    for (int k = 0; k < PIT; ++k) {
      int c, py, pp;
      decode(k, c, py, pp);
      const int ix = ix0 + 2 * pp, iy = iy0 + py;
      const bool rok = tid + NT * k < ITEMS && iy >= 0 && iy < a.H;
      const bool ok0 = rok && ix >= 0 && ix < a.W, ok1 = rok && ix + 1 >= 0 && ix + 1 < a.W;
      if (U8) {
#pragma clang fp contract(off)
        const uint32_t brow = (uint32_t)(iy * a.W) * 3u + (uint32_t)c;
        const uint32_t b0 = __builtin_amdgcn_raw_buffer_load_b8(xrsrc, ok0 ? brow + (uint32_t)ix * 3u : kOutside, 0, 0);
        const uint32_t b1 = __builtin_amdgcn_raw_buffer_load_b8(xrsrc, ok1 ? brow + (uint32_t)(ix + 1) * 3u : kOutside, 0, 0);
        const float mean = c == 0 ? a.u8_mean[0] : (c == 1 ? a.u8_mean[1] : a.u8_mean[2]);
        const float stdv = c == 0 ? a.u8_std[0] : (c == 1 ? a.u8_std[1] : a.u8_std[2]);
        pv[k][0] = ok0 ? ((float)b0 / 255.0f - mean) / stdv : 0.f;
        pv[k][1] = ok1 ? ((float)b1 / 255.0f - mean) / stdv : 0.f;
      } else {
        const uint32_t grow = (uint32_t)(c * (int)hw + iy * a.W) * 4u;
        pv[k][0] = __builtin_bit_cast(float, __builtin_amdgcn_raw_buffer_load_b32(xrsrc, ok0 ? grow + (uint32_t)ix * 4u : kOutside, 0, 0));
        pv[k][1] = __builtin_bit_cast(float, __builtin_amdgcn_raw_buffer_load_b32(xrsrc, ok1 ? grow + (uint32_t)(ix + 1) * 4u : kOutside, 0, 0));
      }
    }
  };
  auto store_p = [&](int buf) {
    uint32_t* pd = patch + buf * PLANEH;
#pragma unroll
    for (int k = 0; k < PIT; ++k) {
      if (PIT * NT == ITEMS || tid + NT * k < ITEMS) {
        f16x2 h, l;
#pragma unroll
        for (int j = 0; j < 2; ++j) {
          const _Float16 hj = (_Float16)pv[k][j];
          h[j] = hj;
          l[j] = (_Float16)((pv[k][j] - (float)hj) * kLoScale);
        }
        int c, py, pp;
        decode(k, c, py, pp);
        const int dw = (c * CP + py * kStemPP) / 2 + pp;
        pd[dw] = __builtin_bit_cast(uint32_t, h);
        pd[PLANEH / 2 + dw] = __builtin_bit_cast(uint32_t, l);
      }
    }
  };

  const u32x4* wa0 = wl + khalf * 64 + l31;
  const int PHo = POOL ? (a.OH - 1) / 2 + 1 : a.OH, PWo = POOL ? (a.OW - 1) / 2 + 1 : a.OW;
  const size_t img = (size_t)n * a.Cout * PHo * PWo;
  const uint32_t plane_ob = (uint32_t)(PHo * PWo) * (uint32_t)sizeof(float);
  const __amdgpu_buffer_rsrc_t yrsrc = __builtin_amdgcn_make_buffer_rsrc(a.y + img, 0, (int)(a.Cout * plane_ob), 0x00020000);

#ifdef ADX_HS_TRACE
  long long tr_c = 0, tr_e = 0, tr_s = 0, tr_t = 0;
  unsigned long long* tr = g_hs_trace + (size_t)(8192 + (blockIdx.x & 8191)) * 8;
  if (threadIdx.x == 0) tr[0] = __builtin_readcyclecounter();
#endif
  load_p(tx_begin);
  store_p(PBUF == 2 ? tx_begin & 1 : 0);
  __syncthreads();
#ifdef ADX_HS_TRACE
  if (threadIdx.x == 0) tr[1] = __builtin_readcyclecounter();
#endif
  for (int tx = tx_begin; tx < tx_end; ++tx) {
#ifdef ADX_HS_TRACE
    tr_t = (long long)__builtin_readcyclecounter();
#endif
    if (tx + 1 < tx_end) load_p(tx + 1);
    const int ox = tx * kTileW + l31;
    float vm[2][16];
#pragma unroll 1
    for (int pass = 0; pass < NROW; ++pass) {
      const int prow = POOL ? (2 * wave + pass) * 2 : wave * 2 * 2;
      const uint32_t* pb0 = patch + (PBUF == 2 ? (tx & 1) * PLANEH : 0) + prow * (kStemPP / 2) + l31;
      constexpr int NR = POOL ? 1 : 2;
      f32x16 accm[NR][2], accl[NR][2];
#pragma unroll
      for (int r = 0; r < NR; ++r)
#pragma unroll
        for (int m = 0; m < 2; ++m)
#pragma unroll
          for (int i = 0; i < 16; ++i) { accm[r][m][i] = 0.f; accl[r][m][i] = 0.f; }
      struct Frags { f16x8 A[2][2], B[2][NR]; };
      auto fetch = [&](Frags& f, int step) {
        const int c0 = 2 * step, c1 = 2 * step + 1 > 20 ? 20 : 2 * step + 1;
        const int off0 = ((c0 / 7) * CP + (c0 % 7) * kStemPP) / 2, off1 = ((c1 / 7) * CP + (c1 % 7) * kStemPP) / 2;
        const uint32_t* pb = pb0 + (khalf ? off1 : off0);
#pragma unroll
        for (int pl = 0; pl < 2; ++pl) {
#pragma unroll
          for (int m = 0; m < 2; ++m) f.A[pl][m] = __builtin_bit_cast(f16x8, wa0[(step * 2 + pl) * 128 + m * 32]);
#pragma unroll
          for (int r = 0; r < NR; ++r) {
            const uint32_t* q = pb + pl * (PLANEH / 2) + r * 2 * (kStemPP / 2);
            u32x4 v;
            v[0] = q[0]; v[1] = q[1]; v[2] = q[2]; v[3] = q[3];
            f.B[pl][r] = __builtin_bit_cast(f16x8, v);
          }
        }
      };
      auto mfmas = [&](const Frags& f) {
#pragma unroll
        for (int r = 0; r < NR; ++r)
#pragma unroll
          for (int m = 0; m < 2; ++m) {
            accm[r][m] = hs_mfma(f.A[0][m], f.B[0][r], accm[r][m]);
            accl[r][m] = hs_mfma(f.A[0][m], f.B[1][r], accl[r][m]);
            accl[r][m] = hs_mfma(f.A[1][m], f.B[0][r], accl[r][m]);
          }
      };
      if (POOL) {
        Frags fr[2];
        fetch(fr[0], 0);
#pragma unroll
        for (int step = 0; step < kStemSteps; ++step) {
          if (step + 1 < kStemSteps) fetch(fr[(step + 1) & 1], step + 1);
          __builtin_amdgcn_sched_barrier(0);
          mfmas(fr[step & 1]);
          __builtin_amdgcn_sched_barrier(0);
        }
      } else {
#pragma unroll 1
        for (int step = 0; step < kStemSteps; ++step) {
          Frags f;
          fetch(f, step);
          mfmas(f);
        }
      }
      if (!POOL) {
#pragma unroll
        for (int rr = 0; rr < NR; ++rr) {
          const int oy = oy0 + wave * 2 + rr;
          const uint32_t voff = (oy < a.OH && ox < a.OW) ? (uint32_t)(oy * a.OW + ox) * 4u + (uint32_t)(4 * khalf) * plane_ob : kOutside;
#pragma unroll
          for (int half = 0; half < 2; ++half)
#pragma unroll
            for (int r = 0; r < 16; ++r) {
              const int cu = half * 32 + (r & 3) + 8 * (r >> 2);
              const int cl = cu + 4 * khalf;
              float v = accm[rr][half][r] + accl[rr][half][r] * (1.f / kLoScale);
              v = v * ss[cl] + ss[kHsCout + cl];
              if (a.relu) v = v > 0.f ? v : 0.f;
              __builtin_amdgcn_raw_buffer_store_b32(__builtin_bit_cast(uint32_t, v), yrsrc, voff, cu * plane_ob, 0);
            }
        }
      } else {
        const int oy = oy0 + 2 * wave + pass;
        const bool in = oy >= 0 && oy < a.OH && ox < a.OW;
#pragma unroll
        for (int half = 0; half < 2; ++half)
#pragma unroll
          for (int r = 0; r < 16; ++r) {
            const int cl = half * 32 + (r & 3) + 8 * (r >> 2) + 4 * khalf;
            float t = (accm[0][half][r] + accl[0][half][r] * (1.f / kLoScale)) * ss[cl] + ss[kHsCout + cl];
            if (a.relu) t = t > 0.f ? t : 0.f;
            t = in ? t : -INFINITY;
            vm[half][r] = pass == 0 ? t : pool_max3(vm[half][r], t, -INFINITY);
          }
      }
    }
#ifdef ADX_HS_TRACE
    { const long long t = (long long)__builtin_readcyclecounter(); tr_c += t - tr_t; tr_t = t; }
#endif
    if (POOL) {
      const int pr = ty * 4 + wave, pq = tx * 16 + (l31 >> 1);
      const bool st = pr < PHo && (l31 & 1) == 0 && pq < PWo && tx >= tx_own;
      const uint32_t voff = st ? (uint32_t)(pr * PWo + pq) * 4u + (uint32_t)(4 * khalf) * plane_ob : kOutside;
      float mm[2][16];
      float lf[2][16];
#pragma unroll
      for (int half = 0; half < 2; ++half)
#pragma unroll
        for (int r = 0; r < 16; ++r) lf[half][r] = cbuf[2 * (half * 16 + r)];
#pragma unroll
      for (int half = 0; half < 2; ++half)
#pragma unroll
        for (int r = 0; r < 16; ++r) {
          const int vi = __builtin_bit_cast(int, vm[half][r]);
          const float up = __builtin_bit_cast(float, __builtin_amdgcn_update_dpp(0, vi, 0x138 , 0xf, 0xf, false));
          const float dn = __builtin_bit_cast(float, __builtin_amdgcn_update_dpp(0, vi, 0x130 , 0xf, 0xf, false));
          const float left = l31 == 0 ? lf[half][r] : up;
          const float right = l31 == 31 ? -INFINITY : dn;
          const float m = pool_max3(left, vm[half][r], right);
          cpark[2 * (half * 16 + r)] = vm[half][r];
          mm[half][r] = m;
        }
      if (!a.y_cells) {
#pragma unroll
        for (int half = 0; half < 2; ++half)
#pragma unroll
          for (int r = 0; r < 16; ++r) {
            const int cu = half * 32 + (r & 3) + 8 * (r >> 2);
            __builtin_amdgcn_raw_buffer_store_b32(__builtin_bit_cast(uint32_t, mm[half][r]), yrsrc, voff, cu * plane_ob, 0);
          }
      } else {
        const uint32_t cplane = (uint32_t)(PHo * PWo) * 16u;
        const uint32_t vcell = st ? (uint32_t)(pr * PWo + pq) * 16u + (uint32_t)khalf * 2u * cplane : kOutside;
#pragma unroll
        for (int half = 0; half < 2; ++half)
          cells_store32<false>(mm[half], nullptr, nullptr, 0, nullptr, false, yrsrc, vcell, (uint32_t)(half * 4) * 2u * cplane, cplane);
      }
    }
#ifdef ADX_HS_TRACE
    { const long long t = (long long)__builtin_readcyclecounter(); tr_e += t - tr_t; tr_t = t; }
#endif
    if (tx + 1 < tx_end) {
      if (PBUF == 1) __syncthreads();
      store_p(PBUF == 2 ? (tx + 1) & 1 : 0);
    }
    __syncthreads();
#ifdef ADX_HS_TRACE
    { const long long t = (long long)__builtin_readcyclecounter(); tr_s += t - tr_t; tr_t = t; }
#endif
  }
#ifdef ADX_HS_TRACE
  if (threadIdx.x == 0) {
    tr[2] = (unsigned long long)tr_c;
    tr[3] = (unsigned long long)tr_e;
    tr[4] = (unsigned long long)tr_s;
    tr[5] = __builtin_readcyclecounter();
  }
#endif
}

__global__ void conv2d_hs_stem_pack_kernel(const float* __restrict__ w, _Float16* __restrict__ p) {
  const int idx = blockIdx.x * 256 + threadIdx.x;
  if (idx >= kStemSteps * 2 * 64 * 8) return;
  const int j = idx & 7, ml = (idx >> 3) & 63, h = (idx >> 9) & 1, step = idx >> 10;
  const int combo = 2 * step + h;
  float v = 0.f;
  if (combo < 21 && j < 7) v = w[((size_t)ml * 3 + combo / 7) * 49 + (combo % 7) * 7 + j];
  const _Float16 hi = (_Float16)v;
  const _Float16 lo = (_Float16)((v - (float)hi) * kLoScale);
  const size_t cell = ((size_t)(step * 2 + 0) * 2 + h) * 64 + ml;
  p[cell * 8 + j] = hi;
  p[(cell + 128) * 8 + j] = lo;
}

static bool hs_is_stem(const ConvSpec& L) { return L.k == 7 && L.stride == 2 && L.pad == 3 && L.cin == 3 && L.cout == 64; }

__global__ void conv2d_hs_pack_kernel(const float* __restrict__ w, _Float16* __restrict__ p, int M, int Kc, int Kreal,
                                      int taps, int dgrad, size_t total) {
  const size_t idx = (size_t)blockIdx.x * 256 + threadIdx.x;
  if (idx >= total) return;
  const int j = idx & 7;
  const int ml = (idx >> 3) & 63;
  const int h = (idx >> 9) & 1;
  size_t rest = idx >> 10;
  const int tap = rest % taps; rest /= taps;
  const int nchunks = Kc / kHsCC;
  const int chunk = rest % nchunks;
  const int ct = rest / nchunks;
  const int m = ct * 64 + ml, kc = chunk * kHsCC + h * 8 + j;
  float v = 0.f;
  if (kc < Kreal) v = dgrad ? w[((size_t)kc * M + m) * taps + (taps - 1 - tap)] : w[((size_t)m * Kreal + kc) * taps + tap];
  const _Float16 hi = (_Float16)v;
  const _Float16 lo = (_Float16)((v - (float)hi) * kLoScale);
  const size_t cell = ((((size_t)(ct * nchunks + chunk) * taps + tap) * 2 + 0) * 2 + h) * 64 + ml;
  p[cell * 8 + j] = hi;
  p[(cell + 128) * 8 + j] = lo;
}

constexpr int kHsPackJobs = 48;
struct HsPackTable {
  const float* w[kHsPackJobs];
  _Float16* p[kHsPackJobs];
  int M[kHsPackJobs], Kc[kHsPackJobs], Kreal[kHsPackJobs], taps[kHsPackJobs], dgrad[kHsPackJobs];
  unsigned first[kHsPackJobs + 1];
  int n;
};
__global__ void __launch_bounds__(256) conv2d_hs_pack_many_kernel(const HsPackTable t) {
  int j = 0, jend = t.n;
  while (jend - j > 1) {
    const int mid = (j + jend) >> 1;
    if (blockIdx.x >= t.first[mid]) j = mid; else jend = mid;
  }
  const int M = t.M[j], Kc = t.Kc[j], Kreal = t.Kreal[j], taps = t.taps[j], dgrad = t.dgrad[j];
  const float* __restrict__ w = t.w[j];
  _Float16* __restrict__ p = t.p[j];
  const size_t total = (size_t)M * Kc * taps;
  const size_t idx = (size_t)(blockIdx.x - t.first[j]) * 256 + threadIdx.x;
  if (idx >= total) return;
  const int e = idx & 7;
  const int ml = (idx >> 3) & 63;
  const int h = (idx >> 9) & 1;
  size_t rest = idx >> 10;
  const int tap = rest % taps; rest /= taps;
  const int nchunks = Kc / kHsCC;
  const int chunk = rest % nchunks;
  const int ct = rest / nchunks;
  const int m = ct * 64 + ml, kc = chunk * kHsCC + h * 8 + e;
  float v = 0.f;
  if (kc < Kreal) v = dgrad ? w[((size_t)kc * M + m) * taps + (taps - 1 - tap)] : w[((size_t)m * Kreal + kc) * taps + tap];
  const _Float16 hi = (_Float16)v;
  const _Float16 lo = (_Float16)((v - (float)hi) * kLoScale);
  const size_t cell = ((((size_t)(ct * nchunks + chunk) * taps + tap) * 2 + 0) * 2 + h) * 64 + ml;
  p[cell * 8 + e] = hi;
  p[(cell + 128) * 8 + e] = lo;
}

int conv2d_hs_pack_many(const HsPackJob* jobs, int n, hipStream_t s) {
  for (int j0 = 0; j0 < n; j0 += kHsPackJobs) {
    HsPackTable t;
    t.n = std::min(kHsPackJobs, n - j0);
    unsigned blocks = 0;
    for (int j = 0; j < t.n; ++j) {
      const HsPackJob& q = jobs[j0 + j];
      ADX_REQUIRE(q.w != nullptr && q.packed != nullptr && q.cin_pad % kHsCC == 0 && q.cout % kHsCout == 0,
                  "conv2d_hs_pack_many: job %d is not a split-fp16 weight image", j0 + j);
      t.w[j] = q.w; t.p[j] = (_Float16*)q.packed;
      t.M[j] = q.cout; t.Kc[j] = q.cin_pad; t.Kreal[j] = q.cin; t.taps[j] = q.taps; t.dgrad[j] = q.dgrad;
      t.first[j] = blocks;
      blocks += (unsigned)(((size_t)q.cout * q.cin_pad * q.taps + 255) / 256);
    }
    t.first[t.n] = blocks;
    conv2d_hs_pack_many_kernel<<<dim3(blocks), dim3(256), 0, s>>>(t);
    ADX_LAUNCH_CHECK();
  }
  return ADX_OK;
}

bool conv2d_hs_eligible(const ConvSpec& L) {
  if (debug_switches().conv_exact) return false;
  if (hs_is_stem(L) && !L.dgrad) return true;
  if (L.cin % kHsCC != 0 || L.cin_pad != L.cin || L.cout % kHsCout != 0) return false;
  return L.k == 3 && (L.stride == 1 || L.stride == 2);
}

size_t conv2d_packed_floats(const ConvSpec& L) {
  const size_t direct = (size_t)L.k * L.k * L.cin_pad * L.cout;
  return direct;
}

bool conv2d_hs_pack_batchable(const ConvSpec& c, int dgrad) { return conv2d_hs_eligible(c) && !(hs_is_stem(c) && !dgrad); }

int conv2d_hs_pack(const ConvSpec& c, const float* w, void* packed, int dgrad, hipStream_t s) {
  if (hs_is_stem(c) && !dgrad) {
    conv2d_hs_stem_pack_kernel<<<dim3(ceil_div(kStemSteps * 2 * 64 * 8, 256)), dim3(256), 0, s>>>(w, (_Float16*)packed);
    ADX_LAUNCH_CHECK();
    return ADX_OK;
  }
  const size_t total = (size_t)c.cout * c.cin_pad * c.k * c.k;
  conv2d_hs_pack_kernel<<<dim3((unsigned)((total + 255) / 256)), dim3(256), 0, s>>>(
      w, (_Float16*)packed, c.cout, c.cin_pad, c.cin, c.k * c.k, dgrad, total);
  ADX_LAUNCH_CHECK();
  return ADX_OK;
}

template <int STRIDE, int K, int ROWS, int PBUF, bool DS, bool XCELLS = false, bool YCELLS = false>
static int hs_launch_t(Conv2dArgs a, hipStream_t s) {
  constexpr int TH = 4 * ROWS;
  constexpr int PH = (TH - 1) * STRIDE + K, PW = (kTileW - 1) * STRIDE + K;
  constexpr size_t lds = (size_t)PBUF * 64 * PH * PW + (size_t)2 * K * 256 * 16 + (DS ? 256 * 16 : 0) +
                         (DS ? 4 : 2) * kHsCout * sizeof(float) + 16;
  static_assert(lds <= 80 * 1024, "two workgroups per CU need <= 80 KB each");
  static std::atomic<uint64_t> attr{0};
  if (DeviceOnce once{attr}; once) {
    ADX_CHECK_HIP(hipFuncSetAttribute(reinterpret_cast<const void*>(&conv2d_hs_kernel<STRIDE, K, ROWS, PBUF, DS, XCELLS, YCELLS>),
                                      hipFuncAttributeMaxDynamicSharedMemorySize, (int)lds));
    once.commit();
  }
  a.tiles_x = ceil_div(a.OW, kTileW); a.tiles_y = ceil_div(a.OH, TH); a.cout_tiles = a.Cout / kHsCout;
  const size_t grid = (size_t)a.cout_tiles * a.tiles_x * a.tiles_y * a.N;
  ADX_REQUIRE(grid < (1u << 31), "conv2d_hs: grid too large");
  ADX_REQUIRE((size_t)a.Cout * a.OH * a.OW * sizeof(float) < 0x7FFFFFFFu, "conv2d_hs: one image of the output exceeds the 32-bit byte offsets");
  conv2d_hs_kernel<STRIDE, K, ROWS, PBUF, DS, XCELLS, YCELLS><<<dim3((unsigned)grid), dim3(256), lds, s>>>(a);
  ADX_LAUNCH_CHECK();
  return ADX_OK;
}

template <bool POOL, bool U8 = false>
static int hs_stem_launch(Conv2dArgs a, hipStream_t s) {
  constexpr int PH = POOL ? 25 : 21, PBUF = POOL ? 1 : 2;
  constexpr size_t lds = (size_t)kStemSteps * 4096 + (size_t)PBUF * 4 * 3 * PH * kStemPP + 2 * kHsCout * sizeof(float) +
                         (POOL ? (4 * 64 + 2) * sizeof(float) : 0);
  static_assert(lds <= 80 * 1024, "two workgroups per CU need <= 80 KB each");
  static std::atomic<uint64_t> attr{0};
  if (DeviceOnce once{attr}; once) {
    ADX_CHECK_HIP(hipFuncSetAttribute(reinterpret_cast<const void*>(&conv2d_hs_stem_kernel<POOL, U8>),
                                      hipFuncAttributeMaxDynamicSharedMemorySize, (int)lds));
    once.commit();
  }
  a.tiles_x = ceil_div(a.OW, kTileW); a.cout_tiles = 1;
  a.tiles_y = POOL ? ceil_div((a.OH - 1) / 2 + 1, 4) : ceil_div(a.OH, 8);
  const int bands = a.tiles_y * a.N;
  a.stem_seg_tiles = 0; a.stem_nseg = 1;
  if (bands < 128 && a.tiles_x > 1) {
    const int want = std::min(a.tiles_x, std::max(1, 256 / bands));
    a.stem_seg_tiles = ceil_div(a.tiles_x, want);
    a.stem_nseg = ceil_div(a.tiles_x, a.stem_seg_tiles);
    if (a.stem_nseg <= 1) { a.stem_seg_tiles = 0; a.stem_nseg = 1; }
  }
  conv2d_hs_stem_kernel<POOL, U8><<<dim3((unsigned)(bands * a.stem_nseg)), dim3(256), lds, s>>>(a);
  ADX_LAUNCH_CHECK();
  return ADX_OK;
}

int conv2d_hs_stem_pool(const ConvSpec& L, const float* x, const float* w, const float* scale, const float* shift,
                        float* pooled, int N, int H, int W, hipStream_t s, const uint8_t* frames_u8, const float* mean,
                        const float* stdv, int y_cells) {
  ADX_REQUIRE((x || frames_u8) && w && scale && shift && pooled, "conv2d_hs_stem_pool: null pointer");
  ADX_REQUIRE((size_t)3 * H * W * sizeof(float) < 0xC0000000u, "conv2d_hs_stem_pool: image too large for 32-bit offsets");
  Conv2dArgs a{};
  a.x = x; a.w = w; a.scale = scale; a.shift = shift; a.y = pooled;
  if (frames_u8 != nullptr) {
    ADX_REQUIRE(mean && stdv, "conv2d_hs_stem_pool: uint8 frames need mean / std");
    a.x_u8 = frames_u8;
    for (int c = 0; c < 3; ++c) { a.u8_mean[c] = mean[c]; a.u8_std[c] = stdv[c]; }
  }
  a.N = N; a.Cin = 3; a.H = H; a.W = W; a.Cout = 64;
  a.OH = conv_out_dim(H, 7, 2, 3); a.OW = conv_out_dim(W, 7, 2, 3);
  a.KH = 7; a.KW = 7; a.stride = 2; a.pad = 3; a.relu = 1;
  a.cin_pad = L.cin_pad; a.cc = L.cc;
  a.y_cells = y_cells;
  return frames_u8 != nullptr ? hs_stem_launch<true, true>(a, s) : hs_stem_launch<true>(a, s);
}

int conv2d_hs_launch_block_s2(const ConvSpec& c1, const ConvSpec& ds, const float* x, const float* w1, const float* scale1,
                              const float* shift1, float* y1, const float* wd, const float* scaled, const float* shiftd,
                              float* yd, int N, int H, int W, hipStream_t s, int x_cells, int y_cells, int relu) {
  ADX_REQUIRE(x && w1 && y1 && wd && yd && (scale1 != nullptr) == (shift1 != nullptr) && (scaled != nullptr) == (shiftd != nullptr),
              "conv2d_hs block launch: null pointer");
  Conv2dArgs a{};
  a.x = x; a.w = w1; a.scale = scale1; a.shift = shift1; a.res = nullptr; a.y = y1; a.x_amax = nullptr; a.x_amax_n = 0;
  a.w_ds = wd; a.scale_ds = scaled; a.shift_ds = shiftd; a.y_ds = yd;
  a.N = N; a.Cin = c1.cin; a.H = H; a.W = W; a.Cout = c1.cout;
  a.OH = conv_out_dim(H, 3, 2, 1); a.OW = conv_out_dim(W, 3, 2, 1);
  a.KH = 3; a.KW = 3; a.stride = 2; a.pad = 1; a.relu = relu;
  a.cin_pad = c1.cin_pad; a.cc = c1.cc;
  a.x_cells = x_cells;
  a.y_cells = y_cells;
  (void)ds;
  return conv2d_hs_launch(c1, a, s);
}

__global__ void __launch_bounds__(256) conv2d_split_reduce_kernel(const float* __restrict__ part, size_t part_stride, int nparts,
                                                                  const float* __restrict__ scale, const float* __restrict__ shift,
                                                                  const float* __restrict__ res, float* __restrict__ y,
                                                                  int cout, int plane4, size_t total4, int relu) {
  const size_t i = (size_t)blockIdx.x * 256 + threadIdx.x;
  if (i >= total4) return;
  const int c = (int)((i / plane4) % cout);
  f32x4 v = reinterpret_cast<const f32x4*>(part)[i];
  for (int p0 = 1; p0 < nparts; p0 += 8) {
    f32x4 t[8];
#pragma unroll
    for (int j = 0; j < 8; ++j) t[j] = reinterpret_cast<const f32x4*>(part + (size_t)(p0 + j < nparts ? p0 + j : 0) * part_stride)[i];
#pragma unroll
    for (int j = 0; j < 8; ++j)
      if (p0 + j < nparts) v += t[j];
  }
  const float sc = scale != nullptr ? scale[c] : 1.f, sh = shift != nullptr ? shift[c] : 0.f;
  v = v * sc + sh;
  if (res != nullptr) v += reinterpret_cast<const f32x4*>(res)[i];
  if (relu) {
#pragma unroll
    for (int k = 0; k < 4; ++k) v[k] = __builtin_fmaxf(v[k], 0.f);
  }
  reinterpret_cast<f32x4*>(y)[i] = v;
}

static bool hs_vrow_ok(const Conv2dArgs& a) {
  return debug_switches().conv_vrow && a.N > 1 && (long)a.N * (a.OW + 1) < (1L << 21) &&
         (size_t)a.N * a.Cout * a.OH * a.OW * sizeof(float) < 0xC0000000u && (size_t)a.N * a.Cin * a.H * a.W * sizeof(float) < 0xC0000000u;
}
static int hs_vrow_tiles_x(const Conv2dArgs& a) { return ceil_div(a.N * (a.OW + 1) - 1, kTileW); }

template <int MODE>
static int hs3x3_launch(Conv2dArgs a, hipStream_t s) {
  constexpr int NT = MODE == 0 ? 256 : 512, TH = MODE == 1 ? 16 : 8, CT = MODE == 2 ? 2 : 1;
  constexpr size_t lds = (size_t)2 * 64 * (TH + 2) * 34 + (size_t)2 * 3 * 256 * CT * 16 + (2 * 64 * CT + 8) * sizeof(float) + 48;
  constexpr size_t lds_bs = lds + 4 * 64 * CT * sizeof(float);
  static_assert(lds_bs <= (MODE == 0 ? 80 : 160) * 1024, "LDS budget");
  static std::atomic<uint64_t> attr{0};
  if (DeviceOnce once{attr}; once) {
    ADX_CHECK_HIP(hipFuncSetAttribute(reinterpret_cast<const void*>(&conv2d_hs3x3_kernel<MODE, 0>),
                                      hipFuncAttributeMaxDynamicSharedMemorySize, (int)lds));
    ADX_CHECK_HIP(hipFuncSetAttribute(reinterpret_cast<const void*>(&conv2d_hs3x3_kernel<MODE, 1>),
                                      hipFuncAttributeMaxDynamicSharedMemorySize, (int)lds));
    ADX_CHECK_HIP(hipFuncSetAttribute(reinterpret_cast<const void*>(&conv2d_hs3x3_kernel<MODE, 2>),
                                      hipFuncAttributeMaxDynamicSharedMemorySize, (int)lds_bs));
    ADX_CHECK_HIP(hipFuncSetAttribute(reinterpret_cast<const void*>(&conv2d_hs3x3_kernel<MODE, 0, false, false, true>),
                                      hipFuncAttributeMaxDynamicSharedMemorySize, (int)lds));
    ADX_CHECK_HIP(hipFuncSetAttribute(reinterpret_cast<const void*>(&conv2d_hs3x3_kernel<MODE, 1, false, false, true>),
                                      hipFuncAttributeMaxDynamicSharedMemorySize, (int)lds));
    ADX_CHECK_HIP(hipFuncSetAttribute(reinterpret_cast<const void*>(&conv2d_hs3x3_kernel<MODE, 2, false, false, true>),
                                      hipFuncAttributeMaxDynamicSharedMemorySize, (int)lds_bs));
    once.commit();
  }
  a.tiles_x = ceil_div(a.OW, kTileW); a.tiles_y = ceil_div(a.OH, TH); a.cout_tiles = a.Cout / (kHsCout * CT);
  const size_t grid = (size_t)a.cout_tiles * a.tiles_x * a.tiles_y * a.N;
  ADX_REQUIRE(grid < (1u << 31), "conv2d_hs: grid too large");
  ADX_REQUIRE((size_t)a.Cout * a.OH * a.OW * sizeof(float) < 0x7FFFFFFFu, "conv2d_hs: one image of the output exceeds the 32-bit byte offsets");
  constexpr bool split_on = true;
  const size_t out_floats = (size_t)a.N * a.Cout * a.OH * a.OW;
  const size_t cap = a.part != nullptr ? a.part_stride : 0;
  const int nchunks = a.cin_pad / kHsCC;
  a.ksplit = 1; a.cper = nchunks; a.part_stride = 0;
  const bool fp32_layout = !(a.x_cells || a.y_cells || a.res_cells);
  const bool xscaled = a.x_amax != nullptr && a.x_amax_n < 0;
  const bool vrow = (fp32_layout || ((a.stats_part != nullptr || xscaled) && !a.y_cells && !a.res_cells)) && hs_vrow_ok(a);
  auto set_vrow = [&]() -> size_t {
    a.vw = a.OW + 1;
    a.inv_vw = 1.f / (float)a.vw;
    a.tiles_x = hs_vrow_tiles_x(a);
    return (size_t)a.cout_tiles * a.tiles_x * a.tiles_y;
  };
  if (a.stats_part != nullptr && a.x_cells && (conv2d_hs3x3q_train_eligible(a) || conv2d_hs3x3q_dgrad_eligible(a))) {
    a.part = nullptr;
    return conv2d_hs3x3q_launch(a, s);
  }
  if (a.stats_part != nullptr) {
    const size_t sgrid = vrow ? set_vrow() : grid;
    const int slots = vrow ? a.tiles_y * a.tiles_x : a.N * a.tiles_y * a.tiles_x;
    ADX_REQUIRE(a.stats_p == slots, "conv2d_hs: statistics buffer laid out for %d tiles, launch has %d", a.stats_p, slots);
    a.part = nullptr;
    if (a.x_cells) {
      ADX_REQUIRE((a.x_amax == nullptr || xscaled) && (a.bs_raw == nullptr) == (a.x_amax == nullptr) && !a.y_cells && !a.res_cells,
                  "conv2d_hs: a cell-layout input with statistics belongs to a training-forward launch or to a data gradient with its scale");
      ADX_REQUIRE((size_t)a.N * a.Cin * a.H * a.W * sizeof(float) < 0xC0000000u, "conv2d_hs: a cell-layout tensor exceeds the 32-bit byte offsets");
      static std::atomic<uint64_t> xattr{0};
      if (DeviceOnce once{xattr}; once) {
        ADX_CHECK_HIP(hipFuncSetAttribute(reinterpret_cast<const void*>(&conv2d_hs3x3_kernel<MODE, 1, true, false, true>),
                                          hipFuncAttributeMaxDynamicSharedMemorySize, (int)lds));
        ADX_CHECK_HIP(hipFuncSetAttribute(reinterpret_cast<const void*>(&conv2d_hs3x3_kernel<MODE, 1, true, false, false>),
                                          hipFuncAttributeMaxDynamicSharedMemorySize, (int)lds));
        ADX_CHECK_HIP(hipFuncSetAttribute(reinterpret_cast<const void*>(&conv2d_hs3x3_kernel<MODE, 2, true, false, true>),
                                          hipFuncAttributeMaxDynamicSharedMemorySize, (int)lds_bs));
        ADX_CHECK_HIP(hipFuncSetAttribute(reinterpret_cast<const void*>(&conv2d_hs3x3_kernel<MODE, 2, true, false, false>),
                                          hipFuncAttributeMaxDynamicSharedMemorySize, (int)lds_bs));
        once.commit();
      }
      if (a.bs_raw != nullptr) {
        if (vrow) conv2d_hs3x3_kernel<MODE, 2, true, false, true><<<dim3((unsigned)sgrid), dim3(NT), lds_bs, s>>>(a);
        else conv2d_hs3x3_kernel<MODE, 2, true, false, false><<<dim3((unsigned)sgrid), dim3(NT), lds_bs, s>>>(a);
      } else if (vrow) conv2d_hs3x3_kernel<MODE, 1, true, false, true><<<dim3((unsigned)sgrid), dim3(NT), lds, s>>>(a);
      else conv2d_hs3x3_kernel<MODE, 1, true, false, false><<<dim3((unsigned)sgrid), dim3(NT), lds, s>>>(a);
    } else if (vrow) {
      if (a.bs_raw != nullptr) conv2d_hs3x3_kernel<MODE, 2, false, false, true><<<dim3((unsigned)sgrid), dim3(NT), lds_bs, s>>>(a);
      else conv2d_hs3x3_kernel<MODE, 1, false, false, true><<<dim3((unsigned)sgrid), dim3(NT), lds, s>>>(a);
    } else {
      if (a.bs_raw != nullptr) conv2d_hs3x3_kernel<MODE, 2><<<dim3((unsigned)sgrid), dim3(NT), lds_bs, s>>>(a);
      else conv2d_hs3x3_kernel<MODE, 1><<<dim3((unsigned)sgrid), dim3(NT), lds, s>>>(a);
    }
    ADX_LAUNCH_CHECK();
    return ADX_OK;
  }
  if (MODE == 0 && split_on && cap > 0 && grid <= 64 && nchunks >= 8 && a.x_amax == nullptr && (a.OH * a.OW) % 4 == 0 &&
      (reinterpret_cast<uintptr_t>(a.y) & 15) == 0 && (a.res == nullptr || (reinterpret_cast<uintptr_t>(a.res) & 15) == 0)) {
    int S = 16;
    while (S > 1 && (nchunks % S != 0 || (nchunks / S) % 2 != 0 || grid * S > 256 || out_floats * S > cap)) S >>= 1;
    if (S > 1) {
      Conv2dArgs c = a;
      c.ksplit = S; c.cper = nchunks / S; c.part_stride = out_floats;
      c.scale = nullptr; c.shift = nullptr; c.res = nullptr; c.relu = 0;
      conv2d_hs3x3_kernel<MODE><<<dim3((unsigned)(grid * S)), dim3(NT), lds, s>>>(c);
      ADX_LAUNCH_CHECK();
      const size_t total4 = out_floats / 4;
      conv2d_split_reduce_kernel<<<dim3((unsigned)ceil_div((long)total4, 256L)), dim3(256), 0, s>>>(
          a.part, out_floats, S, a.scale, a.shift, a.res, a.y, a.Cout, a.OH * a.OW / 4, total4, a.relu);
      ADX_LAUNCH_CHECK();
      return ADX_OK;
    }
  }
  a.part = nullptr;
  if (a.x_cells && xscaled && !a.y_cells && !a.res_cells) {
    static std::atomic<uint64_t> dattr{0};
    if (DeviceOnce once{dattr}; once) {
      ADX_CHECK_HIP(hipFuncSetAttribute(reinterpret_cast<const void*>(&conv2d_hs3x3_kernel<MODE, 0, true, false, true>),
                                        hipFuncAttributeMaxDynamicSharedMemorySize, (int)lds));
      ADX_CHECK_HIP(hipFuncSetAttribute(reinterpret_cast<const void*>(&conv2d_hs3x3_kernel<MODE, 0, true, false, false>),
                                        hipFuncAttributeMaxDynamicSharedMemorySize, (int)lds));
      once.commit();
    }
    ADX_REQUIRE((size_t)a.N * a.Cin * a.H * a.W * sizeof(float) < 0xC0000000u, "conv2d_hs: a cell-layout tensor exceeds the 32-bit byte offsets");
    if (vrow) {
      const size_t vgrid = set_vrow();
      conv2d_hs3x3_kernel<MODE, 0, true, false, true><<<dim3((unsigned)vgrid), dim3(NT), lds, s>>>(a);
    } else {
      conv2d_hs3x3_kernel<MODE, 0, true, false, false><<<dim3((unsigned)grid), dim3(NT), lds, s>>>(a);
    }
    ADX_LAUNCH_CHECK();
    return ADX_OK;
  }
  if (a.x_cells || a.y_cells || a.res_cells) {
    ADX_REQUIRE(a.y_cells && a.x_amax == nullptr, "conv2d_hs: cell-layout operands come with a cell-layout output (and no dynamic range)");
    if (conv2d_hs3x3q_eligible(a)) return conv2d_hs3x3q_launch(a, s);
    constexpr size_t clds = lds;
    static std::atomic<uint64_t> cattr{0};
    if (DeviceOnce once{cattr}; once) {
      const void* fns[2] = {reinterpret_cast<const void*>(&conv2d_hs3x3_kernel<MODE, 0, true, true>),
                            reinterpret_cast<const void*>(&conv2d_hs3x3_kernel<MODE, 0, false, true>)};
      for (const void* f : fns) ADX_CHECK_HIP(hipFuncSetAttribute(f, hipFuncAttributeMaxDynamicSharedMemorySize, (int)clds));
      once.commit();
    }
    a.vw = a.N > 1 ? a.OW + 1 : a.OW;
    a.inv_vw = 1.f / (float)a.vw;
    ADX_REQUIRE((long)a.N * a.vw < (1L << 21), "conv2d_hs: batch x width exceeds the virtual-row arithmetic");
    a.tiles_x = ceil_div(a.N * a.vw - (a.N > 1 ? 1 : 0), kTileW);
    const size_t cgrid = (size_t)a.cout_tiles * a.tiles_x * a.tiles_y;
    ADX_REQUIRE((size_t)a.N * a.Cout * a.OH * a.OW * sizeof(float) < 0xC0000000u && (size_t)a.N * a.Cin * a.H * a.W * sizeof(float) < 0xC0000000u,
                "conv2d_hs: a cell-layout tensor exceeds the 32-bit byte offsets");
    if (a.x_cells) conv2d_hs3x3_kernel<MODE, 0, true, true><<<dim3((unsigned)cgrid), dim3(NT), clds, s>>>(a);
    else conv2d_hs3x3_kernel<MODE, 0, false, true><<<dim3((unsigned)cgrid), dim3(NT), clds, s>>>(a);
    ADX_LAUNCH_CHECK();
    return ADX_OK;
  }
  if (vrow) {
    const size_t vgrid = set_vrow();
    conv2d_hs3x3_kernel<MODE, 0, false, false, true><<<dim3((unsigned)vgrid), dim3(NT), lds, s>>>(a);
  } else {
    conv2d_hs3x3_kernel<MODE><<<dim3((unsigned)grid), dim3(NT), lds, s>>>(a);
  }
  ADX_LAUNCH_CHECK();
  return ADX_OK;
}

static int hs3x3_mode(const ConvSpec& L, const Conv2dArgs& a) {
  if (!(L.k == 3 && L.stride == 1 && a.w_ds == nullptr)) return -1;
  if (!((L.cin_pad / kHsCC) % 2 == 0 && L.pad == 1)) return -1;
  const int mode_env = debug_switches().hs_mode;
  int mode = a.Cin < 256 ? 0 : (a.OH > 8 ? 1 : (a.Cout % 128 == 0 ? 2 : 0));
  if ((long)a.N * ceil_div(a.OH, 8) * ceil_div(a.OW, kTileW) * (a.Cout / kHsCout) <= 256) mode = 0;
  if (mode_env >= 0 && !(mode_env == 2 && a.Cout % 128 != 0)) mode = mode_env;
  return mode;
}

bool conv2d_hs3x3_plain(const ConvSpec& L, int N, int H, int W) {
  if (!debug_switches().conv_cells || !conv2d_hs_eligible(L) || L.dgrad) return false;
  Conv2dArgs a{};
  a.N = N; a.Cin = L.cin; a.Cout = L.cout; a.H = H; a.W = W;
  a.OH = conv_out_dim(H, L.k, L.stride, L.pad); a.OW = conv_out_dim(W, L.k, L.stride, L.pad);
  const int mode = hs3x3_mode(L, a);
  if (mode < 0 || L.cin % 16 != 0 || L.cout % 64 != 0) return false;
  if ((size_t)N * L.cin * H * W * sizeof(float) >= 0xC0000000u || (size_t)N * L.cout * a.OH * a.OW * sizeof(float) >= 0xC0000000u) return false;
  const long grid0 = (long)a.N * ceil_div(a.OH, 8) * ceil_div(a.OW, kTileW) * (a.Cout / kHsCout);
  return mode != 0 || grid0 > 64 || L.cin_pad / kHsCC < 8;
}

bool conv2d_hs3x3_dgrad_cells(const ConvSpec& L, int N, int H, int W) {
  if (debug_switches().train_cells < 4 || !conv2d_hs_eligible(L) || !L.dgrad) return false;
  Conv2dArgs a{};
  a.N = N; a.Cin = L.cin; a.Cout = L.cout; a.H = H; a.W = W;
  a.OH = conv_out_dim(H, L.k, L.stride, L.pad); a.OW = conv_out_dim(W, L.k, L.stride, L.pad);
  return hs3x3_mode(L, a) >= 0 && L.cin % 16 == 0 && L.cin == L.cin_pad && L.cout % 64 == 0 &&
         (size_t)N * L.cin * H * W * sizeof(float) < 0xC0000000u;
}

bool conv2d_hs3x3_dgrad_stats(const ConvSpec& L, int N, int H, int W, bool x_cells, size_t stats_floats) {
  if (!conv2d_hs_eligible(L) || !L.dgrad) return false;
  Conv2dArgs a{};
  a.N = N; a.Cin = L.cin; a.Cout = L.cout; a.H = H; a.W = W;
  a.OH = conv_out_dim(H, L.k, L.stride, L.pad); a.OW = conv_out_dim(W, L.k, L.stride, L.pad);
  a.KH = L.k; a.KW = L.k; a.stride = L.stride; a.pad = L.pad; a.cin_pad = L.cin_pad;
  a.x_cells = x_cells ? 1 : 0;
  const int tiles = conv2d_hs_stats_tiles(L, a);
  return L.k == 3 && L.stride == 1 && tiles > 0 && (size_t)tiles * (L.cout * 2 + L.cout / 64) <= stats_floats;
}

bool conv2d_hs3x3_train_cells(const ConvSpec& L, int N, int H, int W, size_t stats_floats) {
  if (debug_switches().train_cells == 0 || !conv2d_hs_eligible(L) || L.dgrad) return false;
  Conv2dArgs a{};
  a.N = N; a.Cin = L.cin; a.Cout = L.cout; a.H = H; a.W = W;
  a.OH = conv_out_dim(H, L.k, L.stride, L.pad); a.OW = conv_out_dim(W, L.k, L.stride, L.pad);
  a.x_cells = 1;
  if (hs3x3_mode(L, a) < 0 || L.cin % 16 != 0 || L.cin != L.cin_pad || L.cout % 64 != 0) return false;
  if ((size_t)N * L.cin * H * W * sizeof(float) >= 0xC0000000u) return false;
  const int tiles = conv2d_hs_stats_tiles(L, a);
  return tiles > 0 && (size_t)tiles * L.cout * 2 <= stats_floats;
}

int conv2d_hs_stats_tiles(const ConvSpec& L, const Conv2dArgs& a) {
  const int mode = hs3x3_mode(L, a);
  if (mode < 0) return 0;
  if (a.x_cells && (conv2d_hs3x3q_train_eligible(a) || conv2d_hs3x3q_dgrad_eligible(a))) return conv2d_hs3x3q_train_tiles(a);
  if (!(a.y_cells || a.res_cells) && hs_vrow_ok(a)) return ceil_div(a.OH, mode == 1 ? 16 : 8) * hs_vrow_tiles_x(a);
  return a.N * ceil_div(a.OH, mode == 1 ? 16 : 8) * ceil_div(a.OW, kTileW);
}

__global__ void dgrad_s2_weights_kernel(const float* __restrict__ w, float* __restrict__ out, int cin, int cout) {
  const size_t idx = (size_t)blockIdx.x * 256 + threadIdx.x;
  if (idx >= (size_t)16 * cin * cout) return;
  const int c = idx & 1, r = (idx >> 1) & 1;
  size_t rest = idx >> 2;
  const int co = rest % cout; rest /= cout;
  const int ci = rest % cin;
  const int cls = (int)(rest / cin), py = cls >> 1, px = cls & 1;
  const int kh = py == 0 ? (r == 0 ? 1 : -1) : (r == 0 ? 2 : 0);
  const int kw = px == 0 ? (c == 0 ? 1 : -1) : (c == 0 ? 2 : 0);
  out[idx] = (kh >= 0 && kw >= 0) ? w[(((size_t)co * cin + ci) * 3 + kh) * 3 + kw] : 0.f;
}

bool conv2d_hs_dgrad_s2_eligible(int cin, int cout) {
  ConvSpec probe{};
  probe.cin = cout; probe.cin_pad = cout; probe.cout = 4 * cin; probe.k = 3; probe.stride = 1; probe.dgrad = 1;
  return cin % kHsCout == 0 && cout % kHsCC == 0 && conv2d_hs_eligible(probe);
}

int conv2d_hs_dgrad_s2(const float* w, const float* dy, float* dx, int accumulate, int N, int cin, int cout, int H, int W,
                       float* wbuild, float* wimg, const uint32_t* dy_amax, int dy_amax_n, hipStream_t s) {
  ADX_REQUIRE(w && dy && dx && wbuild && wimg, "conv2d_hs_dgrad_s2: null pointer");
  ADX_REQUIRE(conv2d_hs_dgrad_s2_eligible(cin, cout), "conv2d_hs_dgrad_s2: cin %d / cout %d outside the kernel's rules", cin, cout);
  const size_t nw = (size_t)16 * cin * cout;
  dgrad_s2_weights_kernel<<<dim3((unsigned)((nw + 255) / 256)), dim3(256), 0, s>>>(w, wbuild, cin, cout);
  ADX_LAUNCH_CHECK();
  ConvSpec g{};
  g.cin = cout; g.cin_pad = cout; g.cout = 4 * cin; g.k = 2; g.stride = 1; g.pad = 0; g.cc = kHsCC;
  int rc = conv2d_hs_pack(g, wbuild, wimg, 0, s);
  if (rc != ADX_OK) return rc;
  Conv2dArgs a{};
  a.x = dy; a.w = wimg; a.res = accumulate ? dx : nullptr; a.y = dx; a.x_amax = dy_amax; a.x_amax_n = dy_amax_n;
  a.N = N; a.Cin = cout; a.H = conv_out_dim(H, 3, 2, 1); a.W = conv_out_dim(W, 3, 2, 1); a.Cout = 4 * cin;
  a.OH = a.H; a.OW = a.W;
  a.KH = 2; a.KW = 2; a.stride = 1; a.pad = 0; a.relu = 0;
  a.cin_pad = cout; a.cc = kHsCC;
  a.d2s_cin = cin; a.d2s_h = H; a.d2s_w = W;
  ADX_REQUIRE((size_t)cin * H * W * sizeof(float) < 0x7FFFFFFFu, "conv2d_hs_dgrad_s2: one image of dx exceeds the 32-bit byte offsets");
  return hs_launch_t<1, 2, 2, 2, false>(a, s);
}

int conv2d_hs_launch(const ConvSpec& L, Conv2dArgs a, hipStream_t s) {
  ADX_REQUIRE((size_t)L.cin * a.H * a.W * sizeof(float) < 0xC0000000u, "conv2d_hs: one image of the input exceeds the 32-bit byte offsets");
  const bool ds = a.w_ds != nullptr;
  if (hs_is_stem(L) && !ds) {
    ADX_REQUIRE(a.x_amax == nullptr && a.res == nullptr, "conv2d_hs stem: no residual / dynamic range");
    return hs_stem_launch<false>(a, s);
  }
  if (L.k == 3 && L.stride == 1 && !ds) {
    const int mode = hs3x3_mode(L, a);
    if (mode >= 0) return mode == 1 ? hs3x3_launch<1>(a, s) : (mode == 2 ? hs3x3_launch<2>(a, s) : hs3x3_launch<0>(a, s));
    ADX_REQUIRE(a.stats_part == nullptr, "conv2d_hs: statistics requested from a launch the pipelined kernel does not serve");
    return hs_launch_t<1, 3, 2, 2, false>(a, s);
  }
  if (L.k == 3 && L.stride == 2 && L.pad == 1) {
    if (a.x_cells || a.y_cells) {
      ADX_REQUIRE(ds && a.x_amax == nullptr && a.res == nullptr && a.d2s_cin == 0,
                  "conv2d_hs: cell-layout operands of the stride-2 conv need the fused downsample launch (no residual, no dynamic range)");
      if (a.x_cells && a.y_cells) return hs_launch_t<2, 3, 1, 1, true, true, true>(a, s);
      return a.x_cells ? hs_launch_t<2, 3, 1, 1, true, true, false>(a, s) : hs_launch_t<2, 3, 1, 1, true, false, true>(a, s);
    }
    return ds ? hs_launch_t<2, 3, 1, 1, true>(a, s) : hs_launch_t<2, 3, 1, 1, false>(a, s);
  }
  set_error("conv2d_hs: no kernel for k=%d stride=%d pad=%d%s", L.k, L.stride, L.pad, ds ? " with a fused downsample" : "");
  return ADX_ERR_INVALID;
}

}

#ifdef ADX_HS_TRACE
extern "C" int adx_hs_trace_read(unsigned long long* host, int nwords) {
  return (int)hipMemcpyFromSymbol(host, HIP_SYMBOL(adx::g_hs_trace), (size_t)nwords * 8);
}
#endif
```

### autonomous_driving_with_diffusion_model_amd/ops.py

```python
from __future__ import annotations

import ctypes as C
import math
import os
from typing import Optional

import torch

from . import _lib as L


def _strides3(t: torch.Tensor):
    return t.stride(0), t.stride(1), t.stride(2)


def tconv(x0: torch.Tensor, weight: torch.Tensor, bias: Optional[torch.Tensor] = None, *, x1: Optional[torch.Tensor] = None,
          kind: int = 0, stride: int = 1, pad: int = 0, gn_weight: Optional[torch.Tensor] = None,
          gn_bias: Optional[torch.Tensor] = None, groups: int = 0, eps: float = 1e-5,
          tbias: Optional[torch.Tensor] = None, res: Optional[torch.Tensor] = None,
          out: Optional[torch.Tensor] = None, scratch: Optional[torch.Tensor] = None,
          tickets: Optional[torch.Tensor] = None) -> torch.Tensor:
    assert x0.is_cuda and x0.dtype == torch.float32 and x0.dim() == 3
    B, c0, lin = x0.shape
    c1 = 0 if x1 is None else x1.shape[1]
    taps = weight.shape[2]
    cout = weight.shape[0] if kind == 0 else weight.shape[1]
    lout = (lin + 2 * pad - taps) // stride + 1 if kind == 0 else (lin - 1) * stride - 2 * pad + taps
    d = L.TConvDesc(kind, taps, stride, pad, c0, c1, cout, lin, lout, groups, eps)
    nbytes = L.lib().adx_tconv_packed_bytes(C.byref(d))
    if nbytes == 0:
        L.check(-1, "adx_tconv_packed_bytes")
    packed = torch.empty(nbytes // 4, dtype=torch.float32, device=x0.device)
    s = L.stream_ptr(x0.device)
    w = weight.detach().contiguous()
    L.check(L.lib().adx_tconv_pack(C.byref(d), w.data_ptr(), packed.data_ptr(), s), "adx_tconv_pack")
    y = out if out is not None else torch.empty((B, cout, lout), dtype=torch.float32, device=x0.device)
    io = L.TConvIO()
    io.x0 = x0.data_ptr()
    io.x0_sb, io.x0_sc, io.x0_sl = _strides3(x0)
    if x1 is not None:
        io.x1 = x1.data_ptr()
        io.x1_sb, io.x1_sc, io.x1_sl = _strides3(x1)
    io.packed_w = packed.data_ptr()
    keep = [w, packed]
    for name, t in (("bias", bias), ("gamma", gn_weight), ("beta", gn_bias)):
        if t is not None:
            tc = t.detach().contiguous()
            keep.append(tc)
            setattr(io, name, tc.data_ptr())
    if tbias is not None:
        assert tbias.dim() == 2 and tbias.stride(1) == 1
        io.tbias, io.tbias_stride = tbias.data_ptr(), tbias.stride(0)
    if res is not None:
        io.res = res.data_ptr()
        io.res_sb, io.res_sc, io.res_sl = _strides3(res)
    io.y = y.data_ptr()
    io.y_sb, io.y_sc, io.y_sl = _strides3(y)
    io.batch = B
    if scratch is not None:
        assert scratch.is_cuda and scratch.dtype == torch.float32 and scratch.is_contiguous()
        io.scratch, io.scratch_floats = scratch.data_ptr(), scratch.numel()
        if tickets is not None:
            assert tickets.is_cuda and tickets.dtype == torch.int32 and tickets.numel() >= 256 and tickets.is_contiguous()
            io.tickets = tickets.data_ptr()
    L.check(L.lib().adx_tconv_forward(C.byref(d), C.byref(io), s), "adx_tconv_forward")
    return y


def embed(freqs, w1, b1, w3, b3, t, img_feature, rows, cond=None, cond_mlp=None):
    dim = w3.shape[0]
    ew = L.EmbedWeights()
    keep = []
    for name, v in (("freqs", freqs), ("w1", w1), ("b1", b1), ("w3", w3), ("b3", b3)):
        v = v.detach().contiguous()
        keep.append(v)
        setattr(ew, name, v.data_ptr())
    if cond_mlp is not None:
        for name, v in zip(("cw0", "cb0", "cw2", "cb2"), cond_mlp):
            v = v.detach().contiguous()
            keep.append(v)
            setattr(ew, name, v.data_ptr())
    te = torch.empty((rows, dim), dtype=torch.float32, device=t.device)
    mc = torch.empty((rows, 2 * dim), dtype=torch.float32, device=t.device)
    t = t.contiguous()
    img_feature = img_feature.contiguous()
    if cond is not None:
        cond = cond.contiguous()
    L.check(L.lib().adx_embed_forward(C.byref(ew), dim, t.data_ptr(), t.shape[0], L.ptr(cond), img_feature.data_ptr(),
                                      img_feature.shape[0], rows, te.data_ptr(), mc.data_ptr(),
                                      L.stream_ptr(t.device)), "adx_embed_forward")
    return te, mc


def conv2d(x: torch.Tensor, weight: torch.Tensor, *, stride: int = 1, pad: int = 0, scale=None, shift=None, res=None,
           relu: bool = False, packed: Optional[torch.Tensor] = None, out: Optional[torch.Tensor] = None):
    assert x.is_cuda and x.dtype == torch.float32 and x.dim() == 4 and x.is_contiguous()
    n, cin, h, w = x.shape
    cout, _, k, _ = weight.shape
    d = L.Conv2dDesc(cin, cout, k, stride, pad)
    s = L.stream_ptr(x.device)
    if packed is None:
        nbytes = L.lib().adx_conv2d_packed_bytes(C.byref(d))
        if nbytes == 0:
            L.check(-1, "adx_conv2d_packed_bytes")
        packed = torch.empty(nbytes // 4, dtype=torch.float32, device=x.device)
        wc = weight.detach().contiguous()
        L.check(L.lib().adx_conv2d_pack(C.byref(d), wc.data_ptr(), packed.data_ptr(), s), "adx_conv2d_pack")
    oh, ow = (h + 2 * pad - k) // stride + 1, (w + 2 * pad - k) // stride + 1
    y = out if out is not None else torch.empty((n, cout, oh, ow), dtype=torch.float32, device=x.device)
    L.check(L.lib().adx_conv2d_forward(C.byref(d), x.data_ptr(), packed.data_ptr(), L.ptr(scale), L.ptr(shift),
                                       L.ptr(res), y.data_ptr(), n, h, w, int(relu), s), "adx_conv2d_forward")
    return y, packed


def to_cells(x: torch.Tensor) -> torch.Tensor:
    n, c, h, w = x.shape
    hi = x.to(torch.float16)
    lo = ((x - hi.float()) * 2048.0).to(torch.float16)
    cells = torch.stack([hi.view(n, c // 8, 8, h, w), lo.view(n, c // 8, 8, h, w)], dim=2)
    return cells.permute(0, 1, 2, 4, 5, 3).contiguous().view(torch.uint8).reshape(-1)


def from_cells(cells: torch.Tensor, shape) -> torch.Tensor:
    n, c, h, w = shape
    v = cells.view(torch.float16).view(n, c // 8, 2, h, w, 8).float()
    return (v[:, :, 0] + v[:, :, 1] / 2048.0).permute(0, 1, 4, 2, 3).reshape(n, c, h, w).contiguous()


def conv2d_cells(x: torch.Tensor, packed: torch.Tensor, cin: int, cout: int, n: int, h: int, w: int, *, x_cells: bool,
                 scale=None, shift=None, res=None, res_cells: bool = False, relu: bool = False,
                 out: Optional[torch.Tensor] = None) -> torch.Tensor:
    d = L.Conv2dDesc(cin, cout, 3, 1, 1)
    if not L.lib().adx_conv2d_cells_supported(C.byref(d), n, h, w):
        raise ValueError(f"conv2d_cells: {cin}->{cout} at {n}x{h}x{w} is not a plain launch of the pipelined 3x3 kernel")
    y = out if out is not None else torch.empty(n * cout * h * w * 4, dtype=torch.uint8, device=x.device)
    fmt = (1 if x_cells else 0) | 2 | (4 if (res is not None and res_cells) else 0)
    L.check(L.lib().adx_conv2d_forward_cells(C.byref(d), x.data_ptr(), packed.data_ptr(), L.ptr(scale), L.ptr(shift), L.ptr(res),
                                             y.data_ptr(), n, h, w, int(relu), fmt, L.stream_ptr(x.device)),
            "adx_conv2d_forward_cells")
    return y


def conv2d_weight_grad(x: torch.Tensor, dy: torch.Tensor, k: int, *, stride: int = 1, pad: int = 0,
                       estimate_range: bool = True) -> torch.Tensor:
    assert x.is_cuda and dy.is_cuda and x.dtype == dy.dtype == torch.float32 and x.is_contiguous() and dy.is_contiguous()
    n, cin, h, w = x.shape
    cout = dy.shape[1]
    d = L.Conv2dDesc(cin, cout, k, stride, pad)
    dw = torch.empty((cout, cin, k, k), dtype=torch.float32, device=x.device)
    scratch = torch.empty(L.lib().adx_conv2d_wgrad_scratch_bytes(), dtype=torch.uint8, device=x.device)
    L.check(L.lib().adx_conv2d_wgrad_ex(C.byref(d), x.data_ptr(), dy.data_ptr(), dw.data_ptr(), n, h, w, scratch.data_ptr(),
                                        int(bool(estimate_range)), L.stream_ptr(x.device)), "adx_conv2d_wgrad_ex")
    return dw


def conv2d_weight_grad_cells(x: torch.Tensor, dy: torch.Tensor) -> torch.Tensor:
    assert x.is_cuda and dy.is_cuda and x.dtype == dy.dtype == torch.float32
    n, cin, h, w = x.shape
    cout = dy.shape[1]
    amax = float(dy.abs().max())
    s = 2.0 ** (14 - math.floor(math.log2(amax))) if amax > 0 else 1.0
    scale = torch.tensor([s, 1.0 / s], dtype=torch.float32, device=x.device)
    d = L.Conv2dDesc(cin, cout, 3, 1, 1)
    dw = torch.empty((cout, cin, 3, 3), dtype=torch.float32, device=x.device)
    scratch = torch.empty(L.lib().adx_conv2d_wgrad_scratch_bytes(), dtype=torch.uint8, device=x.device)
    xc, dc = to_cells(x.contiguous()), to_cells((dy * s).contiguous())
    L.check(L.lib().adx_conv2d_wgrad_cells(C.byref(d), xc.data_ptr(), dc.data_ptr(), scale.data_ptr(), dw.data_ptr(), n, h, w,
                                           scratch.data_ptr(), L.stream_ptr(x.device)), "adx_conv2d_wgrad_cells")
    return dw


IMAGENET_MEAN, IMAGENET_STD = (0.485, 0.456, 0.406), (0.229, 0.224, 0.225)


def image_transform(frames_u8: torch.Tensor, mean=IMAGENET_MEAN, std=IMAGENET_STD) -> torch.Tensor:
    if frames_u8.dim() == 3:
        frames_u8 = frames_u8[None]
    if not frames_u8.is_cuda or frames_u8.dtype != torch.uint8 or frames_u8.shape[-1] != 3:
        raise L.AdxError("image_transform expects a uint8 [N, H, W, 3] tensor on the GPU")
    f = frames_u8.contiguous()
    n, h, w, _ = f.shape
    out = torch.empty((n, 3, h, w), dtype=torch.float32, device=f.device)
    m, s = (C.c_float * 3)(*mean), (C.c_float * 3)(*std)
    L.check(L.lib().adx_image_normalize(f.data_ptr(), out.data_ptr(), n, h, w, m, s, L.stream_ptr(f.device)),
            "adx_image_normalize")
    return out
```

### include/adx.h

```cpp
#ifndef ADX_H
#define ADX_H

#include <stddef.h>
#include <stdint.h>

#ifdef __cplusplus
extern "C" {
#endif

#define ADX_OK 0
#define ADX_ERR_INVALID (-1)
#define ADX_ERR_HIP (-2)
#define ADX_ERR_STATE (-3)
#define ADX_ERR_RANGE (-4)

typedef void* adx_stream;

int adx_version(void);
const char* adx_source_hash(void);
const char* adx_last_error(void);


typedef struct adx_tconv_desc {
  int32_t kind, taps, stride, pad;
  int32_t c0, c1, cout;
  int32_t lin, lout;
  int32_t groups;
  float eps;
  int32_t w_layout, w_flip;
  int32_t exact;
  int32_t lin_valid, lout_valid;
} adx_tconv_desc;

size_t adx_tconv_packed_bytes(const adx_tconv_desc* d);

int adx_tconv_pack(const adx_tconv_desc* d, const float* w, float* packed, adx_stream s);

typedef struct adx_tconv_io {
  const float* x0; int64_t x0_sb, x0_sc, x0_sl;
  const float* x1; int64_t x1_sb, x1_sc, x1_sl;
  const float* packed_w;
  const float* bias;
  const float* gamma; const float* beta;
  const float* tbias; int64_t tbias_stride;
  const float* res; int64_t res_sb, res_sc, res_sl;
  float* y; int64_t y_sb, y_sc, y_sl;
  int32_t batch;
  float* pre; float* stats;
  float* scratch; int64_t scratch_floats;
  uint32_t* tickets;
} adx_tconv_io;

int adx_tconv_forward(const adx_tconv_desc* d, const adx_tconv_io* io, adx_stream s);

typedef struct adx_embed_weights {
  const float* freqs;
  const float* w1; const float* b1;
  const float* w3; const float* b3;
  const float* cw0; const float* cb0;
  const float* cw2; const float* cb2;
} adx_embed_weights;
int adx_embed_forward(const adx_embed_weights* w, int32_t dim, const int64_t* t, int32_t t_rows,
                      const float* cond ,
                      const float* img_feature, int32_t feat_rows, int32_t rows,
                      float* time_embed, float* mish_cond, adx_stream s);

typedef struct adx_unet adx_unet;

typedef struct adx_unet_config {
  int32_t horizon, transition_dim, dim;
  int32_t n_mults; int32_t dim_mults[8];
  int32_t guidance;
} adx_unet_config;

int adx_unet_create(const adx_unet_config* cfg, adx_unet** out);
#define ADX_UNET_ATTENTION 1
int adx_unet_create_ex(const adx_unet_config* cfg, int32_t flags, adx_unet** out);
void adx_unet_destroy(adx_unet* u);
int adx_unet_num_params(const adx_unet* u);
size_t adx_unet_packed_bytes(const adx_unet* u);
int adx_unet_pack(adx_unet* u, const float* const* params, int32_t n_params, const float* freqs,
                  void* packed, adx_stream s);
size_t adx_unet_workspace_bytes(const adx_unet* u, int32_t rows);

typedef struct adx_unet_io {
  const float* x;
  const float* img_feature; int32_t feat_rows;
  const int64_t* t; int32_t t_rows;
  const float* cond;
  int32_t rows;
  float* out;
  float* time_embed;
  int32_t x_rows;
  const float* time_bias;
} adx_unet_io;
int adx_unet_forward(adx_unet* u, const void* packed, void* workspace, const adx_unet_io* io, adx_stream s);
int32_t adx_unet_time_bias_width(const adx_unet* u);
size_t adx_unet_time_conditioning_workspace_bytes(const adx_unet* u, int32_t rows);
int adx_unet_time_conditioning(adx_unet* u, const void* packed, void* workspace, const adx_unet_io* io, float* time_embed,
                               float* time_bias, adx_stream s);

typedef struct adx_unet_tape adx_unet_tape;
int adx_unet_tape_create(adx_unet_tape** out);
void adx_unet_tape_destroy(adx_unet_tape* t);
size_t adx_unet_train_workspace_bytes(const adx_unet* u, int32_t rows);
int adx_unet_forward_train(adx_unet* u, const void* packed, void* workspace, size_t workspace_bytes,
                           const adx_unet_io* io, adx_unet_tape* tape, adx_stream s);
int adx_unet_backward(adx_unet* u, const void* packed, void* workspace, size_t workspace_bytes, adx_unet_tape* tape,
                      const float* d_out, const float* d_time_embed ,
                      float* d_img_feature, const float* const* params, float* const* grads, int32_t n_grads,
                      adx_stream s);
int adx_gn_mish_backward(const float* dy, int64_t dy_sb, int64_t dy_sc, int64_t dy_sl, const float* pre,
                         const float* stats, const float* gamma, const float* beta, float* dc, float* dgamma,
                         float* dbeta, float* dbias, float* dtb, int64_t dtb_stride, int32_t B, int32_t C, int32_t L,
                         int32_t groups, adx_stream s);
int adx_tconv_wgrad(const adx_tconv_desc* d, const adx_tconv_io* io, const float* dc, float* dw, adx_stream s);
int adx_bias_grad(const float* dc, float* db, int32_t B, int32_t C, int32_t L, adx_stream s);
int adx_chan_layernorm_forward(const float* x, int64_t sb, int64_t sc, int64_t sl, const float* g, const float* b, float* xn,
                               float* mean, float* rstd, int32_t B, int32_t C, int32_t L, int32_t L_valid, adx_stream s);
int adx_chan_layernorm_backward(const float* dy, const float* x, int64_t sb, int64_t sc, int64_t sl, const float* mean,
                                const float* rstd, const float* g, float* dx, float* dg, float* db, int32_t B, int32_t C,
                                int32_t L, int32_t L_valid, int32_t accumulate, adx_stream s);
int adx_linattn_forward(const float* qkv, float* o, int32_t B, int32_t L, int32_t L_valid, adx_stream s);
int adx_linattn_backward(const float* qkv, const float* dout, float* dqkv, int32_t B, int32_t L, int32_t L_valid, adx_stream s);

typedef struct adx_resnet adx_resnet;
int adx_resnet_create(int32_t out_dim, adx_resnet** out);
void adx_resnet_destroy(adx_resnet* r);
int adx_resnet_num_tensors(const adx_resnet* r);
size_t adx_resnet_packed_bytes(const adx_resnet* r);
int adx_resnet_pack(adx_resnet* r, const float* const* tensors, int32_t n, void* packed, adx_stream s);
size_t adx_resnet_workspace_bytes(const adx_resnet* r, int32_t batch, int32_t h, int32_t w);
int adx_resnet_forward(adx_resnet* r, const void* packed, void* workspace, const float* img ,
                       int32_t batch, int32_t h, int32_t w, float* feature , adx_stream s);
int adx_resnet_forward_u8(adx_resnet* r, const void* packed, void* workspace, const uint8_t* frames_hwc,
                          const float* mean , const float* stdv , int32_t batch, int32_t h, int32_t w,
                          float* feature , adx_stream s);

typedef struct adx_conv2d_desc { int32_t cin, cout, k, stride, pad; } adx_conv2d_desc;
size_t adx_conv2d_packed_bytes(const adx_conv2d_desc* d);
int adx_conv2d_pack(const adx_conv2d_desc* d, const float* w , float* packed, adx_stream s);
int adx_conv2d_forward(const adx_conv2d_desc* d, const float* x, const float* packed_w, const float* scale,
                       const float* shift, const float* res, float* y, int32_t n, int32_t h, int32_t w,
                       int32_t relu, adx_stream s);
int adx_conv2d_cells_supported(const adx_conv2d_desc* d, int32_t n, int32_t h, int32_t w);
int adx_conv2d_forward_cells(const adx_conv2d_desc* d, const void* x, const float* packed_w, const float* scale,
                             const float* shift, const void* res, void* y, int32_t n, int32_t h, int32_t w, int32_t relu,
                             int32_t fmt, adx_stream s);
size_t adx_conv2d_wgrad_scratch_bytes(void);
int adx_conv2d_wgrad(const adx_conv2d_desc* d, const float* x, const float* dy, float* dw, int32_t n, int32_t h,
                     int32_t w, void* scratch, adx_stream s);
int adx_conv2d_wgrad_ex(const adx_conv2d_desc* d, const float* x, const float* dy, float* dw, int32_t n, int32_t h,
                        int32_t w, void* scratch, int32_t estimate_range, adx_stream s);
int adx_conv2d_wgrad_cells(const adx_conv2d_desc* d, const void* x_cells, const void* dy_cells, const float* dy_scale, float* dw,
                           int32_t n, int32_t h, int32_t w, void* scratch, adx_stream s);

typedef struct adx_resnet_tape adx_resnet_tape;
int adx_resnet_tape_create(adx_resnet_tape** out);
void adx_resnet_tape_destroy(adx_resnet_tape* t);
size_t adx_resnet_train_workspace_bytes(const adx_resnet* r, int32_t batch, int32_t h, int32_t w);
int adx_resnet_forward_train(adx_resnet* r, const float* const* tensors, int32_t n_tensors, void* packed,
                             void* workspace, size_t workspace_bytes, const float* img, int32_t batch, int32_t h,
                             int32_t w, float* feature, adx_resnet_tape* tape, int32_t update_running, adx_stream s);
int adx_resnet_backward(adx_resnet* r, const float* const* tensors, float* const* grads, int32_t n_tensors,
                        void* workspace, size_t workspace_bytes, adx_resnet_tape* tape, const float* d_feature,
                        adx_stream s);
int32_t adx_resnet_backward_groups(const adx_resnet* r);
int32_t adx_resnet_tensor_group(const adx_resnet* r, int32_t tensor);
int adx_resnet_backward_events(adx_resnet* r, const float* const* tensors, float* const* grads, int32_t n_tensors,
                               void* workspace, size_t workspace_bytes, adx_resnet_tape* tape, const float* d_feature,
                               void* const* events, int32_t n_events, adx_stream s);
int adx_resnet_tape_describe(const adx_resnet_tape* tape, const void* workspace, int32_t index, int32_t* n_records,
                             int32_t* ints, int64_t* offs);

typedef struct adx_trajpred adx_trajpred;
int adx_trajpred_create(int32_t out_dim, adx_trajpred** out);
void adx_trajpred_destroy(adx_trajpred* t);
int adx_trajpred_num_params(const adx_trajpred* t);
size_t adx_trajpred_packed_bytes(const adx_trajpred* t);
size_t adx_trajpred_scratch_bytes(const adx_trajpred* t, int32_t batch, int32_t T);
int adx_trajpred_set_scratch(adx_trajpred* t, void* scratch, size_t bytes);
int adx_trajpred_pack(adx_trajpred* t, const float* const* params, int32_t n, const float* freqs, void* packed,
                      adx_stream s);
int adx_trajpred_forward(adx_trajpred* t, const void* packed, const float* action, int64_t act_sb, int64_t act_st,
                         const float* time_embed, float* out, int32_t batch, int32_t T, adx_stream s);
int adx_trajpred_backward(adx_trajpred* t, const void* packed, const float* action, int64_t act_sb, int64_t act_st,
                          const float* time_embed, const float* grad_out, float* grad_action, int32_t batch,
                          int32_t T, adx_stream s);
int adx_trajpred_backward_params(adx_trajpred* t, const void* packed, const float* action, int64_t act_sb,
                                 int64_t act_st, const float* time_embed, const float* grad_out, float* grad_action,
                                 void* grad_image, float* d_time_embed, int32_t batch, int32_t T, float dropout_p,
                                 uint64_t seed, adx_stream s);
int adx_trajpred_forward_train(adx_trajpred* t, const void* packed, const float* action, int64_t act_sb, int64_t act_st,
                               const float* time_embed, float* out, int32_t batch, int32_t T, float dropout_p,
                               uint64_t seed, adx_stream s);
int adx_trajpred_param_offsets(const adx_trajpred* t, int64_t* offsets, int32_t n);
int adx_guided_output(adx_trajpred* t, const void* packed, const float* action ,
                      const float* time_embed, const float* target , float model_std, float scale,
                      float* x_guided , float* loss , int32_t batch,
                      int32_t T, adx_stream s);

int adx_optim_chunk(void);
int adx_adamw_ema_step(const void* table, const int32_t* block_tensor, const int32_t* block_chunk, int32_t n_blocks,
                       float lr, float beta1, float beta2, float eps, float weight_decay, int32_t step,
                       float ema_decay, int32_t use_ema, int32_t sanitize, adx_stream s);
int adx_adamw_ema_step_scaled(const void* table, const int32_t* block_tensor, const int32_t* block_chunk, int32_t n_blocks,
                       float lr, float beta1, float beta2, float eps, float weight_decay, int32_t step,
                       float ema_decay, int32_t use_ema, int32_t sanitize, float grad_scale, adx_stream s);

#define ADX_PRED_EPSILON 0
#define ADX_PRED_SAMPLE 1
#define ADX_PRED_V 2

typedef struct adx_step_coef {
  int32_t prediction_type;
  int32_t clip;
  float clip_range;
  float sqrt_alpha_t, sqrt_beta_t;
  float c_x0;
  float c_dir;
  float c_x;
  float c_noise;
  int32_t add_noise;
  int32_t use_clipped_model_output;
  int32_t inpaint;
  float c_const;
  float c_known, c_known_noise;
  int32_t known_noise;
  int32_t cfg_combine; float free_scale;
  int32_t zero_first;
} adx_step_coef;

int adx_ddim_step(const adx_step_coef* c, const float* model_output, const float* sample, const float* noise,
                  const float* target, const float* mask, float* prev, float* x0,
                  int32_t batch, int32_t horizon, int32_t dim, adx_stream s);
int adx_ddpm_step(const adx_step_coef* c, const float* model_output, const float* sample, const float* noise,
                  const float* target, const float* mask, float* prev, float* x0,
                  int32_t batch, int32_t horizon, int32_t dim, adx_stream s);
int adx_add_noise(const float* x, const float* noise, const int64_t* t, const float* sqrt_ab, const float* sqrt_1mab,
                  int32_t n_train, float* out, int32_t batch, int32_t horizon, int32_t dim, int32_t zero_first,
                  adx_stream s);

int adx_image_normalize(const uint8_t* frame_hwc, float* out_nchw, int32_t n, int32_t h, int32_t w, const float* mean,
                        const float* stdv, adx_stream s);

int adx_image_augment(uint8_t* frames_hwc, uint8_t* scratch, int32_t n, int32_t h, int32_t w, const float* plan,
                      const uint64_t* seeds, const int32_t* ranges, const float* blur_sigma, int32_t any_blur, adx_stream s);

int adx_probe_mfma_fp16(const void* operands, float* out, int32_t workgroups, int32_t iters, double* flops, adx_stream s);
int adx_probe_mfma_fp16_16x16x32(const void* operands, float* out, int32_t workgroups, int32_t iters, double* flops, adx_stream s);

#ifdef __cplusplus
}
#endif
#endif
```

Measured before the change: 167.8.

## Split stem conv+maxpool into dedicated column-strip kernel with cross-wave pool exchange

```diff
diff --git a/autonomous_driving_with_diffusion_model_amd/_lib.py b/autonomous_driving_with_diffusion_model_amd/_lib.py
--- a/autonomous_driving_with_diffusion_model_amd/_lib.py
+++ b/autonomous_driving_with_diffusion_model_amd/_lib.py
@@ -111,6 +111,7 @@
     "adx_conv2d_forward": (i32, [C.POINTER(Conv2dDesc), vp, vp, vp, vp, vp, vp, i32, i32, i32, i32, vp]),
     "adx_conv2d_cells_supported": (i32, [C.POINTER(Conv2dDesc), i32, i32, i32]),
     "adx_conv2d_forward_cells": (i32, [C.POINTER(Conv2dDesc), vp, vp, vp, vp, vp, vp, i32, i32, i32, i32, i32, vp]),
+    "adx_conv2d_stem_pool": (i32, [vp, i32, vp, vp, vp, vp, vp, vp, i32, i32, i32, i32, vp]),
     "adx_conv2d_wgrad_scratch_bytes": (C.c_size_t, []),
     "adx_conv2d_wgrad": (i32, [C.POINTER(Conv2dDesc), vp, vp, vp, i32, i32, i32, vp, vp]),
     "adx_conv2d_wgrad_ex": (i32, [C.POINTER(Conv2dDesc), vp, vp, vp, i32, i32, i32, vp, i32, vp]),
diff --git a/autonomous_driving_with_diffusion_model_amd/csrc/conv2d.hip b/autonomous_driving_with_diffusion_model_amd/csrc/conv2d.hip
--- a/autonomous_driving_with_diffusion_model_amd/csrc/conv2d.hip
+++ b/autonomous_driving_with_diffusion_model_amd/csrc/conv2d.hip
@@ -503,6 +503,19 @@
               "(adx_conv2d_cells_supported)");
   return conv2d_launch_raw(L, (const float*)x, packed_w, scale, shift, (const float*)res, (float*)y, n, h, w, relu,
                            (hipStream_t)stream, nullptr, 0, nullptr, 0, nullptr, fmt);
+}
+
+int adx_conv2d_stem_pool(const void* x, int32_t x_u8, const float* packed_w, const float* scale, const float* shift,
+                         const float* mean, const float* stdv, void* y, int32_t n, int32_t h, int32_t w, int32_t y_cells,
+                         adx_stream stream) {
+  ConvSpec L{};
+  L.cin = 3; L.cout = 64; L.k = 7; L.stride = 2; L.pad = 3; L.cc = 4; L.cin_pad = 4;
+  ADX_REQUIRE(x && packed_w && scale && shift && y, "adx_conv2d_stem_pool: null tensor");
+  ADX_REQUIRE(n >= 1 && h >= 1 && w >= 1, "adx_conv2d_stem_pool: bad shape %d x %d x %d", n, h, w);
+  ADX_REQUIRE(conv2d_hs_eligible(L), "adx_conv2d_stem_pool: the fused stem + pool is a split-fp16 kernel (unavailable with ADX_CONV_EXACT=1)");
+  ADX_REQUIRE(!x_u8 || (mean && stdv), "adx_conv2d_stem_pool: uint8 frames need mean / std");
+  return conv2d_hs_stem_pool(L, x_u8 ? nullptr : (const float*)x, packed_w, scale, shift, (float*)y, n, h, w, (hipStream_t)stream,
+                             x_u8 ? (const uint8_t*)x : nullptr, mean, stdv, y_cells ? 1 : 0);
 }
 
 int adx_resnet_create(int32_t out_dim, adx_resnet** out) {
diff --git a/autonomous_driving_with_diffusion_model_amd/csrc/conv2d_hs.hip b/autonomous_driving_with_diffusion_model_amd/csrc/conv2d_hs.hip
--- a/autonomous_driving_with_diffusion_model_amd/csrc/conv2d_hs.hip
+++ b/autonomous_driving_with_diffusion_model_amd/csrc/conv2d_hs.hip
@@ -872,46 +872,117 @@
 #endif
 }
 
-__device__ __forceinline__ float pool_max3(float a, float b, float c) {
-  float m = a;
-  m = (b > m || b != b) ? b : m;
-  m = (c > m || c != c) ? c : m;
-  return m;
-}
-
 constexpr int kStemSteps = 11;
 constexpr int kStemPP = 72;
-
-template <bool POOL, bool U8>
+constexpr int kStemPH = 21;
+
+struct StemFrags { f16x8 A[2][2], B[2]; };
+__device__ __forceinline__ void stem_tile(const u32x4* wa0, const uint32_t* pb0, int khalf, f32x16 (&accm)[2], f32x16 (&accl)[2]) {
+  constexpr int CP = kStemPH * kStemPP, PLANEH = 3 * CP;
+#pragma unroll
+  for (int m = 0; m < 2; ++m)
+#pragma unroll
+    for (int i = 0; i < 16; ++i) { accm[m][i] = 0.f; accl[m][i] = 0.f; }
+  auto fetch = [&](StemFrags& f, int step) {
+    const int c0 = 2 * step, c1 = 2 * step + 1 > 20 ? 20 : 2 * step + 1;
+    const int off0 = ((c0 / 7) * CP + (c0 % 7) * kStemPP) / 2, off1 = ((c1 / 7) * CP + (c1 % 7) * kStemPP) / 2;
+    const uint32_t* pb = pb0 + (khalf ? off1 : off0);
+#pragma unroll
+    for (int pl = 0; pl < 2; ++pl) {
+#pragma unroll
+      for (int m = 0; m < 2; ++m) f.A[pl][m] = __builtin_bit_cast(f16x8, wa0[(step * 2 + pl) * 128 + m * 32]);
+      const uint32_t* q = pb + pl * (PLANEH / 2);
+      u32x4 v;
+      v[0] = q[0]; v[1] = q[1]; v[2] = q[2]; v[3] = q[3];
+      f.B[pl] = __builtin_bit_cast(f16x8, v);
+    }
+  };
+  StemFrags fr[2];
+  fetch(fr[0], 0);
+#pragma unroll
+  for (int step = 0; step < kStemSteps; ++step) {
+    if (step + 1 < kStemSteps) fetch(fr[(step + 1) & 1], step + 1);
+    __builtin_amdgcn_sched_barrier(0);
+    const StemFrags& f = fr[step & 1];
+#pragma unroll
+    for (int m = 0; m < 2; ++m) {
+      accm[m] = hs_mfma(f.A[0][m], f.B[0], accm[m]);
+      accl[m] = hs_mfma(f.A[0][m], f.B[1], accl[m]);
+      accl[m] = hs_mfma(f.A[1][m], f.B[0], accl[m]);
+    }
+    __builtin_amdgcn_sched_barrier(0);
+  }
+}
+
+constexpr int kStemStageItems = 3 * kStemPH / 7;
+template <bool U8>
+struct StemStager {
+  float pv[kStemStageItems][2];
+  __device__ __forceinline__ void load(const Conv2dArgs& a, __amdgpu_buffer_rsrc_t xrsrc, int r0, int ix, int iy0) {
+    constexpr uint32_t kOutside = 0xC0000000u;
+    const bool act = r0 < 7;
+    const bool ok0 = act && ix >= 0 && ix < a.W, ok1 = act && ix + 1 >= 0 && ix + 1 < a.W;
+    const size_t hw = (size_t)a.H * a.W;
+#pragma unroll
+    for (int k = 0; k < kStemStageItems; ++k) {
+      const int rc = r0 + 7 * k;
+      const int c = (rc >= kStemPH) + (rc >= 2 * kStemPH), iy = iy0 + rc - kStemPH * c;
+      const bool rok = iy >= 0 && iy < a.H;
+      const bool v0 = rok && ok0, v1 = rok && ok1;
+      if (U8) {
+#pragma clang fp contract(off)
+        const uint32_t brow = (uint32_t)(iy * a.W) * 3u + (uint32_t)c;
+        const uint32_t b0 = __builtin_amdgcn_raw_buffer_load_b8(xrsrc, v0 ? brow + (uint32_t)ix * 3u : kOutside, 0, 0);
+        const uint32_t b1 = __builtin_amdgcn_raw_buffer_load_b8(xrsrc, v1 ? brow + (uint32_t)(ix + 1) * 3u : kOutside, 0, 0);
+        const float mean = c == 0 ? a.u8_mean[0] : (c == 1 ? a.u8_mean[1] : a.u8_mean[2]);
+        const float stdv = c == 0 ? a.u8_std[0] : (c == 1 ? a.u8_std[1] : a.u8_std[2]);
+        pv[k][0] = v0 ? ((float)b0 / 255.0f - mean) / stdv : 0.f;
+        pv[k][1] = v1 ? ((float)b1 / 255.0f - mean) / stdv : 0.f;
+      } else {
+        const uint32_t grow = (uint32_t)(c * (int)hw + iy * a.W) * 4u;
+        pv[k][0] = __builtin_bit_cast(float, __builtin_amdgcn_raw_buffer_load_b32(xrsrc, v0 ? grow + (uint32_t)ix * 4u : kOutside, 0, 0));
+        pv[k][1] = __builtin_bit_cast(float, __builtin_amdgcn_raw_buffer_load_b32(xrsrc, v1 ? grow + (uint32_t)(ix + 1) * 4u : kOutside, 0, 0));
+      }
+    }
+  }
+  __device__ __forceinline__ void store(uint32_t* pd, int r0, int pp) const {
+    constexpr int PLANEH = 3 * kStemPH * kStemPP;
+    if (r0 >= 7) return;
+#pragma unroll
+    for (int k = 0; k < kStemStageItems; ++k) {
+      f16x2 h, l;
+#pragma unroll
+      for (int j = 0; j < 2; ++j) {
+        const _Float16 hj = (_Float16)pv[k][j];
+        h[j] = hj;
+        l[j] = (_Float16)((pv[k][j] - (float)hj) * kLoScale);
+      }
+      const int dw = ((r0 + 7 * k) * kStemPP) / 2 + pp;
+      pd[dw] = __builtin_bit_cast(uint32_t, h);
+      pd[PLANEH / 2 + dw] = __builtin_bit_cast(uint32_t, l);
+    }
+  }
+};
+
 __global__ void __launch_bounds__(256, 2) conv2d_hs_stem_kernel(const Conv2dArgs a) {
-  constexpr int NT = 256;
-  constexpr int PH = POOL ? 25 : 21;
-  constexpr int PBUF = POOL ? 1 : 2;
-  constexpr int CP = PH * kStemPP;
+  constexpr int CP = kStemPH * kStemPP;
   constexpr int PLANEH = 3 * CP;
-  constexpr int ITEMS = 3 * PH * 35;
-  constexpr int PIT = (ITEMS + NT - 1) / NT;
-  constexpr int NROW = POOL ? 3 : 1;
   extern __shared__ __attribute__((aligned(16))) unsigned char smem_raw[];
   u32x4* wl = reinterpret_cast<u32x4*>(smem_raw);
   uint32_t* patch = reinterpret_cast<uint32_t*>(wl + kStemSteps * 256);
-  float* ss = reinterpret_cast<float*>(patch + PBUF * PLANEH);
+  float* ss = reinterpret_cast<float*>(patch + 2 * PLANEH);
   const int tid = threadIdx.x, lane = tid & 63;
   const int wave = __builtin_amdgcn_readfirstlane(tid >> 6);
   const int l31 = lane & 31, khalf = lane >> 5;
   int bid = blockIdx.x, seg = 0;
   if (a.stem_nseg > 1) { seg = bid % a.stem_nseg; bid /= a.stem_nseg; }
   const int n = bid / a.tiles_y, ty = bid - n * a.tiles_y;
-  const int tx_own = a.stem_nseg > 1 ? seg * a.stem_seg_tiles : 0;
-  const int tx_end = a.stem_nseg > 1 ? min(a.tiles_x, tx_own + a.stem_seg_tiles) : a.tiles_x;
-  const int tx_begin = POOL && tx_own > 0 ? tx_own - 1 : tx_own;
-  const int oy0 = POOL ? ty * 8 - 1 : ty * 8, iy0 = oy0 * 2 - 3;
+  const int tx_begin = a.stem_nseg > 1 ? seg * a.stem_seg_tiles : 0;
+  const int tx_end = a.stem_nseg > 1 ? min(a.tiles_x, tx_begin + a.stem_seg_tiles) : a.tiles_x;
+  const int oy0 = ty * 8, iy0 = oy0 * 2 - 3;
   const size_t hw = (size_t)a.H * a.W;
-  const float* xin = a.x + (size_t)n * 3 * hw;
-  constexpr uint32_t kOutside = 0xC0000000u;
   const __amdgpu_buffer_rsrc_t xrsrc =
-      U8 ? __builtin_amdgcn_make_buffer_rsrc(const_cast<uint8_t*>(a.x_u8 + (size_t)n * 3 * hw), 0, (int)(3 * hw), 0x00020000)
-         : __builtin_amdgcn_make_buffer_rsrc(const_cast<float*>(xin), 0, (int)(3 * hw * sizeof(float)), 0x00020000);
+      __builtin_amdgcn_make_buffer_rsrc(const_cast<float*>(a.x + (size_t)n * 3 * hw), 0, (int)(3 * hw * sizeof(float)), 0x00020000);
 
   {
     const u32x4* wsrc = reinterpret_cast<const u32x4*>(a.w);
@@ -922,231 +993,219 @@
     const int c = tid & (kHsCout - 1);
     ss[tid] = a.scale == nullptr ? (tid < kHsCout ? 1.f : 0.f) : (tid < kHsCout ? a.scale[c] : a.shift[c]);
   }
-  float* cbuf = ss + 2 * kHsCout + wave * 64 + khalf;
-  float* cpark = l31 == 31 ? cbuf : ss + 2 * kHsCout + 4 * 64 + (lane & 1);
-  if (POOL && l31 == 0) {
-#pragma unroll
-    for (int i = 0; i < 32; ++i) cbuf[2 * i] = -INFINITY;
-  }
-
-  auto decode = [&](int k, int& c, int& py, int& pp) {
-    int e = tid + NT * k;
-    asm volatile("" : "+v"(e));
-    c = e / (PH * 35);
-    const int rem = e - c * (PH * 35);
-    py = rem / 35;
-    pp = rem - py * 35;
-  };
-  float pv[PIT][2];
-  auto load_p = [&](int tx) {
-    const int ix0 = tx * 64 - 3;
-#pragma unroll
-    for (int k = 0; k < PIT; ++k) {
-      int c, py, pp;
-      decode(k, c, py, pp);
-      const int ix = ix0 + 2 * pp, iy = iy0 + py;
-      const bool rok = tid + NT * k < ITEMS && iy >= 0 && iy < a.H;
-      const bool ok0 = rok && ix >= 0 && ix < a.W, ok1 = rok && ix + 1 >= 0 && ix + 1 < a.W;
-      if (U8) {
-#pragma clang fp contract(off)
-        const uint32_t brow = (uint32_t)(iy * a.W) * 3u + (uint32_t)c;
-        const uint32_t b0 = __builtin_amdgcn_raw_buffer_load_b8(xrsrc, ok0 ? brow + (uint32_t)ix * 3u : kOutside, 0, 0);
-        const uint32_t b1 = __builtin_amdgcn_raw_buffer_load_b8(xrsrc, ok1 ? brow + (uint32_t)(ix + 1) * 3u : kOutside, 0, 0);
-        const float mean = c == 0 ? a.u8_mean[0] : (c == 1 ? a.u8_mean[1] : a.u8_mean[2]);
-        const float stdv = c == 0 ? a.u8_std[0] : (c == 1 ? a.u8_std[1] : a.u8_std[2]);
-        pv[k][0] = ok0 ? ((float)b0 / 255.0f - mean) / stdv : 0.f;
-        pv[k][1] = ok1 ? ((float)b1 / 255.0f - mean) / stdv : 0.f;
-      } else {
-        const uint32_t grow = (uint32_t)(c * (int)hw + iy * a.W) * 4u;
-        pv[k][0] = __builtin_bit_cast(float, __builtin_amdgcn_raw_buffer_load_b32(xrsrc, ok0 ? grow + (uint32_t)ix * 4u : kOutside, 0, 0));
-        pv[k][1] = __builtin_bit_cast(float, __builtin_amdgcn_raw_buffer_load_b32(xrsrc, ok1 ? grow + (uint32_t)(ix + 1) * 4u : kOutside, 0, 0));
-      }
-    }
-  };
-  auto store_p = [&](int buf) {
-    uint32_t* pd = patch + buf * PLANEH;
-#pragma unroll
-    for (int k = 0; k < PIT; ++k) {
-      if (PIT * NT == ITEMS || tid + NT * k < ITEMS) {
-        f16x2 h, l;
-#pragma unroll
-        for (int j = 0; j < 2; ++j) {
-          const _Float16 hj = (_Float16)pv[k][j];
-          h[j] = hj;
-          l[j] = (_Float16)((pv[k][j] - (float)hj) * kLoScale);
-        }
-        int c, py, pp;
-        decode(k, c, py, pp);
-        const int dw = (c * CP + py * kStemPP) / 2 + pp;
-        pd[dw] = __builtin_bit_cast(uint32_t, h);
-        pd[PLANEH / 2 + dw] = __builtin_bit_cast(uint32_t, l);
-      }
-    }
-  };
-
+  const int r0 = tid / 35, pp = tid - r0 * 35;
+  StemStager<false> sg;
   const u32x4* wa0 = wl + khalf * 64 + l31;
-  const int PHo = POOL ? (a.OH - 1) / 2 + 1 : a.OH, PWo = POOL ? (a.OW - 1) / 2 + 1 : a.OW;
+  const size_t img = (size_t)n * a.Cout * a.OH * a.OW;
+  const uint32_t plane_ob = (uint32_t)(a.OH * a.OW) * (uint32_t)sizeof(float);
+  const __amdgpu_buffer_rsrc_t yrsrc = __builtin_amdgcn_make_buffer_rsrc(a.y + img, 0, (int)(a.Cout * plane_ob), 0x00020000);
+  constexpr uint32_t kOutside = 0xC0000000u;
+
+  sg.load(a, xrsrc, r0, tx_begin * 64 - 3 + 2 * pp, iy0);
+  sg.store(patch + (tx_begin & 1) * PLANEH, r0, pp);
+  __syncthreads();
+  for (int tx = tx_begin; tx < tx_end; ++tx) {
+    if (tx + 1 < tx_end) sg.load(a, xrsrc, r0, (tx + 1) * 64 - 3 + 2 * pp, iy0);
+    const int ox = tx * kTileW + l31;
+    const uint32_t* pb0 = patch + (tx & 1) * PLANEH + wave * 4 * (kStemPP / 2) + l31;
+    f32x16 accm[2][2], accl[2][2];
+#pragma unroll
+    for (int r = 0; r < 2; ++r)
+#pragma unroll
+      for (int m = 0; m < 2; ++m)
+#pragma unroll
+        for (int i = 0; i < 16; ++i) { accm[r][m][i] = 0.f; accl[r][m][i] = 0.f; }
+#pragma unroll 1
+    for (int step = 0; step < kStemSteps; ++step) {
+      const int c0 = 2 * step, c1 = 2 * step + 1 > 20 ? 20 : 2 * step + 1;
+      const int off0 = ((c0 / 7) * CP + (c0 % 7) * kStemPP) / 2, off1 = ((c1 / 7) * CP + (c1 % 7) * kStemPP) / 2;
+      const uint32_t* pb = pb0 + (khalf ? off1 : off0);
+      f16x8 A[2][2], B[2][2];
+#pragma unroll
+      for (int pl = 0; pl < 2; ++pl) {
+#pragma unroll
+        for (int m = 0; m < 2; ++m) A[pl][m] = __builtin_bit_cast(f16x8, wa0[(step * 2 + pl) * 128 + m * 32]);
+#pragma unroll
+        for (int r = 0; r < 2; ++r) {
+          const uint32_t* q = pb + pl * (PLANEH / 2) + r * 2 * (kStemPP / 2);
+          u32x4 v;
+          v[0] = q[0]; v[1] = q[1]; v[2] = q[2]; v[3] = q[3];
+          B[pl][r] = __builtin_bit_cast(f16x8, v);
+        }
+      }
+#pragma unroll
+      for (int r = 0; r < 2; ++r)
+#pragma unroll
+        for (int m = 0; m < 2; ++m) {
+          accm[r][m] = hs_mfma(A[0][m], B[0][r], accm[r][m]);
+          accl[r][m] = hs_mfma(A[0][m], B[1][r], accl[r][m]);
+          accl[r][m] = hs_mfma(A[1][m], B[0][r], accl[r][m]);
+        }
+    }
+#pragma unroll
+    for (int rr = 0; rr < 2; ++rr) {
+      const int oy = oy0 + wave * 2 + rr;
+      const uint32_t voff = (oy < a.OH && ox < a.OW) ? (uint32_t)(oy * a.OW + ox) * 4u + (uint32_t)(4 * khalf) * plane_ob : kOutside;
+#pragma unroll
+      for (int half = 0; half < 2; ++half)
+#pragma unroll
+        for (int r = 0; r < 16; ++r) {
+          const int cu = half * 32 + (r & 3) + 8 * (r >> 2);
+          const int cl = cu + 4 * khalf;
+          float v = accm[rr][half][r] + accl[rr][half][r] * (1.f / kLoScale);
+          v = v * ss[cl] + ss[kHsCout + cl];
+          if (a.relu) v = v > 0.f ? v : 0.f;
+          __builtin_amdgcn_raw_buffer_store_b32(__builtin_bit_cast(uint32_t, v), yrsrc, voff, cu * plane_ob, 0);
+        }
+    }
+    if (tx + 1 < tx_end) sg.store(patch + ((tx + 1) & 1) * PLANEH, r0, pp);
+    __syncthreads();
+  }
+}
+
+constexpr int kStemPoolCols = 15;
+template <bool U8>
+__global__ void __launch_bounds__(256, 2) conv2d_hs_stem_pool_kernel(const Conv2dArgs a) {
+  constexpr int PLANEH = 3 * kStemPH * kStemPP;
+  extern __shared__ __attribute__((aligned(16))) unsigned char smem_raw[];
+  u32x4* wl = reinterpret_cast<u32x4*>(smem_raw);
+  uint32_t* patch = reinterpret_cast<uint32_t*>(wl + kStemSteps * 256);
+  float* ss = reinterpret_cast<float*>(patch + PLANEH);
+  float* xch = ss + 2 * kHsCout;
+  const int tid = threadIdx.x, lane = tid & 63;
+  const int wave = __builtin_amdgcn_readfirstlane(tid >> 6);
+  const int l31 = lane & 31, khalf = lane >> 5;
+  int bid = blockIdx.x, seg = 0;
+  if (a.stem_nseg > 1) { seg = bid % a.stem_nseg; bid /= a.stem_nseg; }
+  const int n = bid / a.tiles_x, tx = bid - n * a.tiles_x;
+  const int b_own = a.stem_nseg > 1 ? seg * a.stem_seg_tiles : 0;
+  const int b_end = a.stem_nseg > 1 ? min(a.tiles_y, b_own + a.stem_seg_tiles) : a.tiles_y;
+  const int b_begin = b_own > 0 ? b_own - 1 : 0;
+  const int sx0 = tx * 2 * kStemPoolCols - 1;
+  const size_t hw = (size_t)a.H * a.W;
+  const __amdgpu_buffer_rsrc_t xrsrc =
+      U8 ? __builtin_amdgcn_make_buffer_rsrc(const_cast<uint8_t*>(a.x_u8 + (size_t)n * 3 * hw), 0, (int)(3 * hw), 0x00020000)
+         : __builtin_amdgcn_make_buffer_rsrc(const_cast<float*>(a.x + (size_t)n * 3 * hw), 0, (int)(3 * hw * sizeof(float)), 0x00020000);
+
+  {
+    const u32x4* wsrc = reinterpret_cast<const u32x4*>(a.w);
+#pragma unroll
+    for (int k = 0; k < kStemSteps; ++k) wl[tid + 256 * k] = wsrc[tid + 256 * k];
+  }
+  if (tid < 2 * kHsCout) {
+    const int c = tid & (kHsCout - 1);
+    ss[tid] = a.scale == nullptr ? (tid < kHsCout ? 1.f : 0.f) : (tid < kHsCout ? a.scale[c] : a.shift[c]);
+  }
+  const int r0 = tid / 35, pp = tid - r0 * 35;
+  const int ix = 2 * sx0 - 3 + 2 * pp;
+  StemStager<U8> sg;
+  const u32x4* wa0 = wl + khalf * 64 + l31;
+  const uint32_t* pb0 = patch + wave * 4 * (kStemPP / 2) + l31;
+
+  const int PHo = (a.OH - 1) / 2 + 1, PWo = (a.OW - 1) / 2 + 1;
   const size_t img = (size_t)n * a.Cout * PHo * PWo;
   const uint32_t plane_ob = (uint32_t)(PHo * PWo) * (uint32_t)sizeof(float);
   const __amdgpu_buffer_rsrc_t yrsrc = __builtin_amdgcn_make_buffer_rsrc(a.y + img, 0, (int)(a.Cout * plane_ob), 0x00020000);
+  constexpr uint32_t kOutside = 0xC0000000u;
+  const int sx = sx0 + l31, pq = tx * kStemPoolCols + (l31 >> 1);
+  const bool col_in = sx >= 0 && sx < a.OW;
+  const bool col_st = (l31 & 1) != 0 && l31 < 2 * kStemPoolCols && pq < PWo;
+  float* xl = xch + khalf * 16 + (l31 >> 1);
 
 #ifdef ADX_HS_TRACE
   long long tr_c = 0, tr_e = 0, tr_s = 0, tr_t = 0;
   unsigned long long* tr = g_hs_trace + (size_t)(8192 + (blockIdx.x & 8191)) * 8;
   if (threadIdx.x == 0) tr[0] = __builtin_readcyclecounter();
 #endif
-  load_p(tx_begin);
-  store_p(PBUF == 2 ? tx_begin & 1 : 0);
+  sg.load(a, xrsrc, r0, ix, b_begin * 16 - 3);
+  sg.store(patch, r0, pp);
   __syncthreads();
 #ifdef ADX_HS_TRACE
   if (threadIdx.x == 0) tr[1] = __builtin_readcyclecounter();
 #endif
-  for (int tx = tx_begin; tx < tx_end; ++tx) {
+  float vm[32];
+#pragma unroll
+  for (int j = 0; j < 32; ++j) vm[j] = -INFINITY;
+  for (int b = b_begin; b < b_end; ++b) {
 #ifdef ADX_HS_TRACE
     tr_t = (long long)__builtin_readcyclecounter();
 #endif
-    if (tx + 1 < tx_end) load_p(tx + 1);
-    const int ox = tx * kTileW + l31;
-    float vm[2][16];
-#pragma unroll 1
-    for (int pass = 0; pass < NROW; ++pass) {
-      const int prow = POOL ? (2 * wave + pass) * 2 : wave * 2 * 2;
-      const uint32_t* pb0 = patch + (PBUF == 2 ? (tx & 1) * PLANEH : 0) + prow * (kStemPP / 2) + l31;
-      constexpr int NR = POOL ? 1 : 2;
-      f32x16 accm[NR][2], accl[NR][2];
-#pragma unroll
-      for (int r = 0; r < NR; ++r)
-#pragma unroll
-        for (int m = 0; m < 2; ++m)
-#pragma unroll
-          for (int i = 0; i < 16; ++i) { accm[r][m][i] = 0.f; accl[r][m][i] = 0.f; }
-      struct Frags { f16x8 A[2][2], B[2][NR]; };
-      auto fetch = [&](Frags& f, int step) {
-        const int c0 = 2 * step, c1 = 2 * step + 1 > 20 ? 20 : 2 * step + 1;
-        const int off0 = ((c0 / 7) * CP + (c0 % 7) * kStemPP) / 2, off1 = ((c1 / 7) * CP + (c1 % 7) * kStemPP) / 2;
-        const uint32_t* pb = pb0 + (khalf ? off1 : off0);
-#pragma unroll
-        for (int pl = 0; pl < 2; ++pl) {
-#pragma unroll
-          for (int m = 0; m < 2; ++m) f.A[pl][m] = __builtin_bit_cast(f16x8, wa0[(step * 2 + pl) * 128 + m * 32]);
-#pragma unroll
-          for (int r = 0; r < NR; ++r) {
-            const uint32_t* q = pb + pl * (PLANEH / 2) + r * 2 * (kStemPP / 2);
-            u32x4 v;
-            v[0] = q[0]; v[1] = q[1]; v[2] = q[2]; v[3] = q[3];
-            f.B[pl][r] = __builtin_bit_cast(f16x8, v);
-          }
-        }
-      };
-      auto mfmas = [&](const Frags& f) {
-#pragma unroll
-        for (int r = 0; r < NR; ++r)
-#pragma unroll
-          for (int m = 0; m < 2; ++m) {
-            accm[r][m] = hs_mfma(f.A[0][m], f.B[0][r], accm[r][m]);
-            accl[r][m] = hs_mfma(f.A[0][m], f.B[1][r], accl[r][m]);
-            accl[r][m] = hs_mfma(f.A[1][m], f.B[0][r], accl[r][m]);
-          }
-      };
-      if (POOL) {
-        Frags fr[2];
-        fetch(fr[0], 0);
-#pragma unroll
-        for (int step = 0; step < kStemSteps; ++step) {
-          if (step + 1 < kStemSteps) fetch(fr[(step + 1) & 1], step + 1);
-          __builtin_amdgcn_sched_barrier(0);
-          mfmas(fr[step & 1]);
-          __builtin_amdgcn_sched_barrier(0);
-        }
-      } else {
-#pragma unroll 1
-        for (int step = 0; step < kStemSteps; ++step) {
-          Frags f;
-          fetch(f, step);
-          mfmas(f);
-        }
-      }
-      if (!POOL) {
-#pragma unroll
-        for (int rr = 0; rr < NR; ++rr) {
-          const int oy = oy0 + wave * 2 + rr;
-          const uint32_t voff = (oy < a.OH && ox < a.OW) ? (uint32_t)(oy * a.OW + ox) * 4u + (uint32_t)(4 * khalf) * plane_ob : kOutside;
-#pragma unroll
-          for (int half = 0; half < 2; ++half)
-#pragma unroll
-            for (int r = 0; r < 16; ++r) {
-              const int cu = half * 32 + (r & 3) + 8 * (r >> 2);
-              const int cl = cu + 4 * khalf;
-              float v = accm[rr][half][r] + accl[rr][half][r] * (1.f / kLoScale);
-              v = v * ss[cl] + ss[kHsCout + cl];
-              if (a.relu) v = v > 0.f ? v : 0.f;
-              __builtin_amdgcn_raw_buffer_store_b32(__builtin_bit_cast(uint32_t, v), yrsrc, voff, cu * plane_ob, 0);
-            }
-        }
-      } else {
-        const int oy = oy0 + 2 * wave + pass;
-        const bool in = oy >= 0 && oy < a.OH && ox < a.OW;
-#pragma unroll
-        for (int half = 0; half < 2; ++half)
-#pragma unroll
-          for (int r = 0; r < 16; ++r) {
-            const int cl = half * 32 + (r & 3) + 8 * (r >> 2) + 4 * khalf;
-            float t = (accm[0][half][r] + accl[0][half][r] * (1.f / kLoScale)) * ss[cl] + ss[kHsCout + cl];
-            if (a.relu) t = t > 0.f ? t : 0.f;
-            t = in ? t : -INFINITY;
-            vm[half][r] = pass == 0 ? t : pool_max3(vm[half][r], t, -INFINITY);
-          }
-      }
-    }
+    const bool pre = b < b_own;
+    if (b + 1 < b_end) sg.load(a, xrsrc, r0, ix, (b + 1) * 16 - 3);
+    auto stem_row = [&](auto odd) {
+      constexpr int rr = decltype(odd)::value ? 1 : 0;
+      f32x16 accm[2], accl[2];
+      stem_tile(wa0, pb0 + rr * 2 * (kStemPP / 2), khalf, accm, accl);
+      const int oy = b * 8 + 2 * wave + rr;
+      const float hi = oy < a.OH && col_in ? INFINITY : -INFINITY;
+      float hv[32];
+#pragma unroll
+      for (int half = 0; half < 2; ++half)
+#pragma unroll
+        for (int r = 0; r < 16; ++r) {
+          const int cl = half * 32 + (r & 3) + 8 * (r >> 2) + 4 * khalf;
+          float t = (accm[half][r] + accl[half][r] * (1.f / kLoScale)) * ss[cl] + ss[kHsCout + cl];
+          t = __builtin_fminf(__builtin_fmaxf(t, 0.f), hi);
+          const int ti = __builtin_bit_cast(int, t);
+          const float left = __builtin_bit_cast(float, __builtin_amdgcn_mov_dpp(ti, 0x138 , 0xf, 0xf, true));
+          const float right = __builtin_bit_cast(float, __builtin_amdgcn_mov_dpp(ti, 0x130 , 0xf, 0xf, true));
+          const int j = half * 16 + r;
+          hv[j] = __builtin_fmaxf(__builtin_fmaxf(left, t), right);
+          vm[j] = __builtin_fmaxf(vm[j], hv[j]);
+        }
+      if constexpr (rr == 1) {
+        if (l31 & 1) {
+#pragma unroll
+          for (int j = 0; j < 32; ++j) xl[wave * 1024 + 32 * j] = hv[j];
+        }
+      }
+    };
+    if (!pre) stem_row(std::false_type{});
+    stem_row(std::true_type{});
 #ifdef ADX_HS_TRACE
     { const long long t = (long long)__builtin_readcyclecounter(); tr_c += t - tr_t; tr_t = t; }
 #endif
-    if (POOL) {
-      const int pr = ty * 4 + wave, pq = tx * 16 + (l31 >> 1);
-      const bool st = pr < PHo && (l31 & 1) == 0 && pq < PWo && tx >= tx_own;
-      const uint32_t voff = st ? (uint32_t)(pr * PWo + pq) * 4u + (uint32_t)(4 * khalf) * plane_ob : kOutside;
-      float mm[2][16];
-      float lf[2][16];
-#pragma unroll
-      for (int half = 0; half < 2; ++half)
-#pragma unroll
-        for (int r = 0; r < 16; ++r) lf[half][r] = cbuf[2 * (half * 16 + r)];
-#pragma unroll
-      for (int half = 0; half < 2; ++half)
-#pragma unroll
-        for (int r = 0; r < 16; ++r) {
-          const int vi = __builtin_bit_cast(int, vm[half][r]);
-          const float up = __builtin_bit_cast(float, __builtin_amdgcn_update_dpp(0, vi, 0x138 , 0xf, 0xf, false));
-          const float dn = __builtin_bit_cast(float, __builtin_amdgcn_update_dpp(0, vi, 0x130 , 0xf, 0xf, false));
-          const float left = l31 == 0 ? lf[half][r] : up;
-          const float right = l31 == 31 ? -INFINITY : dn;
-          const float m = pool_max3(left, vm[half][r], right);
-          cpark[2 * (half * 16 + r)] = vm[half][r];
-          mm[half][r] = m;
-        }
-      if (!a.y_cells) {
-#pragma unroll
-        for (int half = 0; half < 2; ++half)
-#pragma unroll
-          for (int r = 0; r < 16; ++r) {
-            const int cu = half * 32 + (r & 3) + 8 * (r >> 2);
-            __builtin_amdgcn_raw_buffer_store_b32(__builtin_bit_cast(uint32_t, mm[half][r]), yrsrc, voff, cu * plane_ob, 0);
+    __syncthreads();
+    {
+      const float* src = xl + ((wave + 3) & 3) * 1024;
+      float up[32];
+#pragma unroll
+      for (int j = 0; j < 32; ++j) up[j] = src[32 * j];
+      if (wave != 0) {
+#pragma unroll
+        for (int j = 0; j < 32; ++j) vm[j] = __builtin_fmaxf(up[j], vm[j]);
+      }
+      const int pr = b * 4 + wave;
+      if (!pre && pr < PHo) {
+        const bool st = col_st;
+        if (!a.y_cells) {
+          const uint32_t voff = st ? (uint32_t)(pr * PWo + pq) * 4u + (uint32_t)(4 * khalf) * plane_ob : kOutside;
+#pragma unroll
+          for (int half = 0; half < 2; ++half)
+#pragma unroll
+            for (int r = 0; r < 16; ++r) {
+              const int cu = half * 32 + (r & 3) + 8 * (r >> 2);
+              __builtin_amdgcn_raw_buffer_store_b32(__builtin_bit_cast(uint32_t, vm[half * 16 + r]), yrsrc, voff, cu * plane_ob, 0);
+            }
+        } else {
+          const uint32_t cplane = (uint32_t)(PHo * PWo) * 16u;
+          const uint32_t vcell = st ? (uint32_t)(pr * PWo + pq) * 16u + (uint32_t)khalf * 2u * cplane : kOutside;
+#pragma unroll
+          for (int half = 0; half < 2; ++half) {
+            float mm[16];
+#pragma unroll
+            for (int r = 0; r < 16; ++r) mm[r] = vm[half * 16 + r];
+            cells_store32<false>(mm, nullptr, nullptr, 0, nullptr, false, yrsrc, vcell, (uint32_t)(half * 4) * 2u * cplane, cplane);
           }
-      } else {
-        const uint32_t cplane = (uint32_t)(PHo * PWo) * 16u;
-        const uint32_t vcell = st ? (uint32_t)(pr * PWo + pq) * 16u + (uint32_t)khalf * 2u * cplane : kOutside;
-#pragma unroll
-        for (int half = 0; half < 2; ++half)
-          cells_store32<false>(mm[half], nullptr, nullptr, 0, nullptr, false, yrsrc, vcell, (uint32_t)(half * 4) * 2u * cplane, cplane);
-      }
+        }
+      }
+#pragma unroll
+      for (int j = 0; j < 32; ++j) vm[j] = wave == 0 ? up[j] : -INFINITY;
     }
 #ifdef ADX_HS_TRACE
     { const long long t = (long long)__builtin_readcyclecounter(); tr_e += t - tr_t; tr_t = t; }
 #endif
-    if (tx + 1 < tx_end) {
-      if (PBUF == 1) __syncthreads();
-      store_p(PBUF == 2 ? (tx + 1) & 1 : 0);
-    }
+    if (b + 1 < b_end) sg.store(patch, r0, pp);
     __syncthreads();
 #ifdef ADX_HS_TRACE
     { const long long t = (long long)__builtin_readcyclecounter(); tr_s += t - tr_t; tr_t = t; }
@@ -1308,20 +1367,17 @@
   return ADX_OK;
 }
 
-template <bool POOL, bool U8 = false>
 static int hs_stem_launch(Conv2dArgs a, hipStream_t s) {
-  constexpr int PH = POOL ? 25 : 21, PBUF = POOL ? 1 : 2;
-  constexpr size_t lds = (size_t)kStemSteps * 4096 + (size_t)PBUF * 4 * 3 * PH * kStemPP + 2 * kHsCout * sizeof(float) +
-                         (POOL ? (4 * 64 + 2) * sizeof(float) : 0);
+  constexpr size_t lds = (size_t)kStemSteps * 4096 + (size_t)2 * 4 * 3 * kStemPH * kStemPP + 2 * kHsCout * sizeof(float);
   static_assert(lds <= 80 * 1024, "two workgroups per CU need <= 80 KB each");
   static std::atomic<uint64_t> attr{0};
   if (DeviceOnce once{attr}; once) {
-    ADX_CHECK_HIP(hipFuncSetAttribute(reinterpret_cast<const void*>(&conv2d_hs_stem_kernel<POOL, U8>),
-                                      hipFuncAttributeMaxDynamicSharedMemorySize, (int)lds));
+    ADX_CHECK_HIP(hipFuncSetAttribute(reinterpret_cast<const void*>(&conv2d_hs_stem_kernel), hipFuncAttributeMaxDynamicSharedMemorySize,
+                                      (int)lds));
     once.commit();
   }
   a.tiles_x = ceil_div(a.OW, kTileW); a.cout_tiles = 1;
-  a.tiles_y = POOL ? ceil_div((a.OH - 1) / 2 + 1, 4) : ceil_div(a.OH, 8);
+  a.tiles_y = ceil_div(a.OH, 8);
   const int bands = a.tiles_y * a.N;
   a.stem_seg_tiles = 0; a.stem_nseg = 1;
   if (bands < 128 && a.tiles_x > 1) {
@@ -1330,7 +1386,33 @@
     a.stem_nseg = ceil_div(a.tiles_x, a.stem_seg_tiles);
     if (a.stem_nseg <= 1) { a.stem_seg_tiles = 0; a.stem_nseg = 1; }
   }
-  conv2d_hs_stem_kernel<POOL, U8><<<dim3((unsigned)(bands * a.stem_nseg)), dim3(256), lds, s>>>(a);
+  conv2d_hs_stem_kernel<<<dim3((unsigned)(bands * a.stem_nseg)), dim3(256), lds, s>>>(a);
+  ADX_LAUNCH_CHECK();
+  return ADX_OK;
+}
+
+template <bool U8>
+static int hs_stem_pool_launch(Conv2dArgs a, hipStream_t s) {
+  constexpr size_t lds = (size_t)kStemSteps * 4096 + (size_t)4 * 3 * kStemPH * kStemPP + 2 * kHsCout * sizeof(float) +
+                         (size_t)4 * 1024 * sizeof(float);
+  static_assert(lds <= 80 * 1024, "two workgroups per CU need <= 80 KB each");
+  static std::atomic<uint64_t> attr{0};
+  if (DeviceOnce once{attr}; once) {
+    ADX_CHECK_HIP(hipFuncSetAttribute(reinterpret_cast<const void*>(&conv2d_hs_stem_pool_kernel<U8>),
+                                      hipFuncAttributeMaxDynamicSharedMemorySize, (int)lds));
+    once.commit();
+  }
+  a.tiles_x = ceil_div((a.OW - 1) / 2 + 1, kStemPoolCols); a.cout_tiles = 1;
+  a.tiles_y = ceil_div((a.OH - 1) / 2 + 1, 4);
+  const int strips = a.tiles_x * a.N;
+  a.stem_seg_tiles = 0; a.stem_nseg = 1;
+  if (strips < 256 && a.tiles_y > 1) {
+    const int want = std::min(a.tiles_y, std::max(1, 512 / strips));
+    a.stem_seg_tiles = ceil_div(a.tiles_y, want);
+    a.stem_nseg = ceil_div(a.tiles_y, a.stem_seg_tiles);
+    if (a.stem_nseg <= 1) { a.stem_seg_tiles = 0; a.stem_nseg = 1; }
+  }
+  conv2d_hs_stem_pool_kernel<U8><<<dim3((unsigned)(strips * a.stem_nseg)), dim3(256), lds, s>>>(a);
   ADX_LAUNCH_CHECK();
   return ADX_OK;
 }
@@ -1352,7 +1434,7 @@
   a.KH = 7; a.KW = 7; a.stride = 2; a.pad = 3; a.relu = 1;
   a.cin_pad = L.cin_pad; a.cc = L.cc;
   a.y_cells = y_cells;
-  return frames_u8 != nullptr ? hs_stem_launch<true, true>(a, s) : hs_stem_launch<true>(a, s);
+  return frames_u8 != nullptr ? hs_stem_pool_launch<true>(a, s) : hs_stem_pool_launch<false>(a, s);
 }
 
 int conv2d_hs_launch_block_s2(const ConvSpec& c1, const ConvSpec& ds, const float* x, const float* w1, const float* scale1,
@@ -1663,7 +1745,7 @@
   const bool ds = a.w_ds != nullptr;
   if (hs_is_stem(L) && !ds) {
     ADX_REQUIRE(a.x_amax == nullptr && a.res == nullptr, "conv2d_hs stem: no residual / dynamic range");
-    return hs_stem_launch<false>(a, s);
+    return hs_stem_launch(a, s);
   }
   if (L.k == 3 && L.stride == 1 && !ds) {
     const int mode = hs3x3_mode(L, a);
diff --git a/autonomous_driving_with_diffusion_model_amd/ops.py b/autonomous_driving_with_diffusion_model_amd/ops.py
--- a/autonomous_driving_with_diffusion_model_amd/ops.py
+++ b/autonomous_driving_with_diffusion_model_amd/ops.py
@@ -185,3 +185,19 @@
     L.check(L.lib().adx_image_normalize(f.data_ptr(), out.data_ptr(), n, h, w, m, s, L.stream_ptr(f.device)),
             "adx_image_normalize")
     return out
+
+
+def stem_pool(x: torch.Tensor, packed: torch.Tensor, scale: torch.Tensor, shift: torch.Tensor, *, cells: bool = False,
+              mean=IMAGENET_MEAN, std=IMAGENET_STD, out: Optional[torch.Tensor] = None) -> torch.Tensor:
+    u8 = x.dtype == torch.uint8
+    assert x.is_cuda and x.is_contiguous() and x.dim() == 4 and (x.shape[3] == 3 if u8 else (x.dtype == torch.float32 and x.shape[1] == 3))
+    n, h, w = (x.shape[0], x.shape[1], x.shape[2]) if u8 else (x.shape[0], x.shape[2], x.shape[3])
+    oh, ow = (h - 1) // 2 + 1, (w - 1) // 2 + 1
+    ph, pw = (oh - 1) // 2 + 1, (ow - 1) // 2 + 1
+    if out is None:
+        out = (torch.empty(n * 64 * ph * pw * 4, dtype=torch.uint8, device=x.device) if cells else
+               torch.empty((n, 64, ph, pw), dtype=torch.float32, device=x.device))
+    m, s = (C.c_float * 3)(*mean), (C.c_float * 3)(*std)
+    L.check(L.lib().adx_conv2d_stem_pool(x.data_ptr(), int(u8), packed.data_ptr(), scale.data_ptr(), shift.data_ptr(), m, s,
+                                         out.data_ptr(), n, h, w, int(cells), L.stream_ptr(x.device)), "adx_conv2d_stem_pool")
+    return out
diff --git a/include/adx.h b/include/adx.h
--- a/include/adx.h
+++ b/include/adx.h
@@ -147,6 +147,9 @@
 int adx_conv2d_forward_cells(const adx_conv2d_desc* d, const void* x, const float* packed_w, const float* scale,
                              const float* shift, const void* res, void* y, int32_t n, int32_t h, int32_t w, int32_t relu,
                              int32_t fmt, adx_stream s);
+int adx_conv2d_stem_pool(const void* x, int32_t x_u8, const float* packed_w, const float* scale, const float* shift,
+                         const float* mean, const float* stdv, void* y, int32_t n, int32_t h, int32_t w, int32_t y_cells,
+                         adx_stream s);
 size_t adx_conv2d_wgrad_scratch_bytes(void);
 int adx_conv2d_wgrad(const adx_conv2d_desc* d, const float* x, const float* dy, float* dw, int32_t n, int32_t h,
                      int32_t w, void* scratch, adx_stream s);
```

New measurement: 173.4, median of 6. +3.3%, better.
